# StanfordASL/pmpc

Measured on AMD Instinct MI355X. Metric: SCP iterations/sec (M particles x N horizon), higher is better.
Workload: dtype f64; 1 GPU; quadrotor x12 u4 M=4096 N=50 Nc=1 box-u, full SCP iteration (on-device linearise + c_lqp_solve-equivalent + residual), BASELINE config D; timed window = SCP iterations 6..2477 from the cold start X_prev = x0, U_prev = U_ref (the active-set round count falls as the SCP loop converges, so the rate depends on the window); particles_per_gpu=4096, parallelism=particle-shard x1, scp_loop=library (pmpc_scp_loop_device), ipm_warm_start=True

## Files before the change

include/pmpc_abi.h:

```cpp
#ifndef PMPC_ABI_H
#define PMPC_ABI_H

#include <stddef.h>

#ifdef __cplusplus
extern "C" {
#endif


void c_lqp_solve(double *X_out, double *U_out, size_t xdim, size_t udim, size_t N, size_t M, long long Nc,
                 double *x0, double *f, double *fx, double *fu, double *X_prev, double *U_prev, double *Q,
                 double *R, double *X_ref, double *U_ref, double *lx, double *ux, double *lu, double *uu,
                 double reg_x, double reg_u, double *slew_reg, double *slew_reg0, double *slew_um1,
                 long long verbose);

void c_lcone_solve(double *X_out, double *U_out, size_t xdim, size_t udim, size_t N, size_t M, long long Nc,
                   double *x0, double *f, double *fx, double *fu, double *X_prev, double *U_prev, double *Q,
                   double *R, double *X_ref, double *U_ref, double *lx, double *ux, double *lu, double *uu,
                   double reg_x, double reg_u, double *slew_reg, double *slew_reg0, double *slew_um1,
                   long long verbose, double smooth_alpha, char *solver);

void pmpc_lqp_solve_host(double *X_out, double *U_out, size_t xdim, size_t udim, size_t N, size_t M, long long Nc,
                         double *x0, double *f, double *fx, double *fu, double *X_prev, double *U_prev, double *Q,
                         double *R, double *X_ref, double *U_ref, double *lx, double *ux, double *lu, double *uu,
                         double reg_x, double reg_u, double *slew_reg, double *slew_reg0, double *slew_um1,
                         long long verbose, unsigned rowmajor);
void pmpc_lcone_solve_host(double *X_out, double *U_out, size_t xdim, size_t udim, size_t N, size_t M, long long Nc,
                           double *x0, double *f, double *fx, double *fu, double *X_prev, double *U_prev, double *Q,
                           double *R, double *X_ref, double *U_ref, double *lx, double *ux, double *lu, double *uu,
                           double reg_x, double reg_u, double *slew_reg, double *slew_reg0, double *slew_um1,
                           long long verbose, double smooth_alpha, unsigned rowmajor, long long cone_k);
void pmpc_lcone_solve_host_ex(double *X_out, double *U_out, size_t xdim, size_t udim, size_t N, size_t M, long long Nc, double *x0, double *f,
                              double *fx, double *fu, double *X_prev, double *U_prev, double *Q, double *R, double *X_ref, double *U_ref, double *lx,
                              double *ux, double *lu, double *uu, double reg_x, double reg_u, double *slew_reg, double *slew_reg0, double *slew_um1,
                              long long verbose, double smooth_alpha, unsigned rowmajor, long long cone_k, int smooth_cstr, double smooth_beta);


#define PMPC_HAS_XBOUNDS 1u
#define PMPC_HAS_UBOUNDS 2u
#define PMPC_HAS_SLEW 4u
#define PMPC_HAS_SLEW0 8u
#define PMPC_FORCE_GENERIC 16u
#define PMPC_SYMMETRIC_COST 32u

#define PMPC_COLD_START 64u
#define PMPC_STATIC_CONS_BOUNDS 128u
#define PMPC_PREV_IS_LAST_SOLUTION 256u

#define PMPC_CONE_OBJECTIVE 1024u
#define PMPC_F32_MATRICES 512u

typedef struct pmpc_problem {
  size_t xdim, udim, N, M;
  long long Nc;
  unsigned flags;
  double reg_x, reg_u;
  const double *x0, *f, *fx, *fu, *X_prev, *U_prev, *Q, *R, *X_ref, *U_ref;
  const double *lx, *ux, *lu, *uu;
  const double *slew_reg, *slew_reg0, *slew_um1;
  double *X_out, *U_out;
  const double *weights;
  double barrier_mu;
  size_t soc_q;
  const double *soc_W, *soc_w0, *soc_v;
  double soc_v0;
  const double *soc_u_interior;
  size_t cone_count;
  const int *cone_sizes;
  const double *cone_A, *cone_c;
  int cone_per_stage;
  long long cone_k;
  int smooth_cstr;
  double smooth_beta;
} pmpc_problem;

typedef struct pmpc_info {
  int status;
  int ipm_iters;
  int structured_solves;
  int fast_path;
  double mu;
  double slack_res;
  double max_violation;
  int outer_solves;
  int active_set_rounds;
} pmpc_info;

typedef struct pmpc_ctx pmpc_ctx;

int pmpc_create(pmpc_ctx **ctx, int device);
void pmpc_destroy(pmpc_ctx *ctx);
int pmpc_set_option(pmpc_ctx *ctx, const char *key, double value);
int pmpc_get_option(pmpc_ctx *ctx, const char *key, double *value);
void *pmpc_stream(pmpc_ctx *ctx);
void pmpc_sync(pmpc_ctx *ctx);

int pmpc_lqp_solve_device(pmpc_ctx *ctx, const pmpc_problem *prob, pmpc_info *info, int verbose);

int pmpc_lcone_solve_device(pmpc_ctx *ctx, const pmpc_problem *prob, double smooth_alpha, pmpc_info *info, int verbose);

int pmpc_lsoc_solve_device(pmpc_ctx *ctx, const pmpc_problem *prob, pmpc_info *info, int verbose);

int pmpc_particle_costs_device(pmpc_ctx *ctx, const pmpc_problem *prob, const double *X, const double *U, double *J_out);

int pmpc_comm_unique_id(void *unique_id_128);
int pmpc_comm_init(pmpc_ctx *ctx, int rank, int world, const void *unique_id_128);
int pmpc_comm_init_mock(pmpc_ctx *ctx, int rank, int world, int group);
int pmpc_comm_rank(pmpc_ctx *ctx);
int pmpc_comm_world(pmpc_ctx *ctx);

int pmpc_linearize_device(pmpc_ctx *ctx, int model, size_t N, size_t M, const double *x0, const double *X_prev,
                          const double *U_prev, const double *params, double *f, double *fx, double *fu);

#define PMPC_MODEL_CUSTOM0 1000
int pmpc_model_compile(const char *source, int xdim, int udim, int pdim, const char *arch, void **code, size_t *bytes, char *log,
                       size_t log_cap);
void pmpc_model_free_code(void *code);
int pmpc_model_load(pmpc_ctx *ctx, const void *code, size_t bytes, int xdim, int udim, int pdim);
int pmpc_model_unload(pmpc_ctx *ctx, int id);

int pmpc_linearize_device_f32(pmpc_ctx *ctx, int model, size_t N, size_t M, const double *x0, const double *X_prev,
                              const double *U_prev, const double *params, double *f, float *fx, float *fu);

int pmpc_rollout_device(pmpc_ctx *ctx, int model, size_t N, size_t M, const double *x0, const double *U, const double *params, double *X);

int pmpc_shift_plan_device(pmpc_ctx *ctx, int model, size_t N, size_t M, size_t s, const double *X, const double *U,
                           const double *params, const double *U_tail, double *X_new, double *U_new, double *um1_new);

int pmpc_shift_active_set_device(pmpc_ctx *ctx, size_t N, size_t M, size_t udim, long long Nc, size_t s, const double *U,
                                 const double *U_tail, const int *act, const double *lo, const double *hi, double *U_new, int *act_new);

int pmpc_warm_shift_device(pmpc_ctx *ctx, size_t N, size_t M, size_t udim, long long Nc, size_t s, const double *U, const double *U_tail,
                           const double *lo, const double *hi, double *U_new, int *shifted);

int pmpc_warm_set_read_device(pmpc_ctx *ctx, int *act_out, size_t n);

int pmpc_linearize_compact_device(pmpc_ctx *ctx, int model, size_t N, size_t M, const double *x0, const double *X_prev,
                                  const double *U_prev, const double *params, double *f, double *jc);
int pmpc_expand_jac_device(pmpc_ctx *ctx, int model, size_t N, size_t M, const double *jc, double *fx, double *fu, int orient);
long long pmpc_jac_compact_doubles(int model, size_t N, size_t M);
int pmpc_jac_live_mask(int model, unsigned char *fx_mask, unsigned char *fu_mask);

int pmpc_as_sweep_variant(int sweep, int xdim, int udim, int M, int Nc, unsigned flags, const int *knobs, int *out);

int pmpc_as_sweep_resources(int sweep, int xdim, int udim, const int *variant, int *out);

int pmpc_as_sweep_launches(int sweep, unsigned long long *out, int n, int reset);
void pmpc_as_sweep_knobs(int *out);

int pmpc_fast_launches(int kind, unsigned long long *out, int n, int reset);

int pmpc_scp_residual_device(pmpc_ctx *ctx, size_t xdim, size_t udim, size_t N, size_t M, const double *X, const double *X_prev,
                             const double *U, const double *U_prev, double *out);

int pmpc_scp_loop_device(pmpc_ctx *ctx, int model, const double *params, const pmpc_problem *p, double *f2, double *fx2, double *fu2,
                         int steps, int first_cold, double *res, pmpc_info *infos, int *last_in_out);

int pmpc_ref_shift_device(pmpc_ctx *ctx, size_t dim, size_t rows, const double *A, const double *c, const double *ref, double *out);
long long pmpc_ref_shift_bad_pivots(pmpc_ctx *ctx, int reset);

typedef struct pmpc_scp_cost {
  int kind;
  union { int K; int id; };
  union { int pos_dim; int uses_u; };
  int pos_idx[3];
  int per_stage;
  union { const double *centres; const double *cparams; };
  const double *sigma, *w;
} pmpc_scp_cost;
size_t pmpc_abi_scp_cost_size(void);

int pmpc_obstacle_cost_grad_device(pmpc_ctx *ctx, const pmpc_scp_cost *cost, size_t xdim, size_t N, size_t M, const double *X_prev,
                                   double *cx);
int pmpc_obstacle_ref_shift_device(pmpc_ctx *ctx, const pmpc_scp_cost *cost, size_t xdim, size_t N, size_t M, const double *X_prev,
                                   const double *Q, const double *X_ref, double *out);

int pmpc_scp_loop_device_cost(pmpc_ctx *ctx, int model, const double *params, const pmpc_problem *p, double *f2, double *fx2,
                              double *fu2, int steps, int first_cold, double *res, pmpc_info *infos, int *last_in_out,
                              const pmpc_scp_cost *cost);

#define PMPC_COST_CUSTOM0 1000
int pmpc_cost_compile(const char *source, int xdim, int udim, int cdim, int uses_u, const char *arch, void **code, size_t *bytes, char *log,
                      size_t log_cap);
int pmpc_cost_load(pmpc_ctx *ctx, const void *code, size_t bytes, int xdim, int udim, int cdim, int uses_u);
int pmpc_cost_unload(pmpc_ctx *ctx, int id);
int pmpc_custom_cost_grad_device(pmpc_ctx *ctx, int id, size_t N, size_t M, const double *X_prev, const double *U_prev, const double *cparams,
                                 double *cx, double *cu, double *val);

typedef struct pmpc_scp_cstr {
  int kind;
  int K;
  union { int pos_dim; int id; };
  int pos_idx[3];
  long long centre_stride_particle, centre_stride_stage;
  union { const double *centres; const double *gparams; };
  const double *radius;
} pmpc_scp_cstr;
size_t pmpc_abi_scp_cstr_size(void);

int pmpc_keepout_augment_device(pmpc_ctx *ctx, const pmpc_scp_cstr *cstr, size_t xdim, size_t udim, size_t N, size_t M,
                                const double *X_prev, const double *f, const double *fx, const double *fu, const double *X_ref,
                                double *f_aug, double *fx_aug, double *fu_aug, double *X_prev_aug, double *X_ref_aug, double *xu_aug);

int pmpc_keepout_strip_residual_device(pmpc_ctx *ctx, size_t xdim, int K, size_t udim, size_t N, size_t M, const double *X_aug, double *X,
                                       const double *X_prev, const double *U, const double *U_prev, double *out);

typedef struct pmpc_scp_aug {
  const double *Q, *x0, *lx;
  double *f[2], *fx[2], *fu[2], *X_prev[2], *X_ref[2], *xu[2];
  double *X_out;
} pmpc_scp_aug;
size_t pmpc_abi_scp_aug_size(void);

int pmpc_scp_loop_device_cstr(pmpc_ctx *ctx, int model, const double *params, const pmpc_problem *p, double *f2, double *fx2,
                              double *fu2, int steps, int first_cold, double *res, pmpc_info *infos, int *last_in_out,
                              const pmpc_scp_cost *cost, const pmpc_scp_cstr *cstr, const pmpc_scp_aug *aug);
#define PMPC_CSTR_CUSTOM0 1000
int pmpc_cstr_compile(const char *source, int xdim, int kdim, int pdim, const char *arch, void **code, size_t *bytes, char *log, size_t log_cap);
int pmpc_cstr_load(pmpc_ctx *ctx, const void *code, size_t bytes, int xdim, int kdim, int pdim);
int pmpc_cstr_unload(pmpc_ctx *ctx, int id);
int pmpc_custom_cstr_rows_device(pmpc_ctx *ctx, int id, size_t N, size_t M, const double *X_prev, const double *gparams, double *a, double *h,
                                 double *g);
int pmpc_rows_augment_device(pmpc_ctx *ctx, int K, size_t xdim, size_t udim, size_t N, size_t M, const double *a, const double *h,
                             const double *X_prev, const double *f, const double *fx, const double *fu, const double *X_ref, double *f_aug,
                             double *fx_aug, double *fu_aug, double *X_prev_aug, double *X_ref_aug, double *xu_aug);
long long pmpc_cstr_bad_rows(pmpc_ctx *ctx, int reset);

void pmpc_scp_loop_follow_ups(unsigned long long *out2, int reset);

void pmpc_profile_enable(pmpc_ctx *ctx, int level);
void pmpc_profile_read(pmpc_ctx *ctx, double *ms4, long long *n4);
void pmpc_profile_read_partial(pmpc_ctx *ctx, double *ms, long long *n);
void pmpc_profile_read_all(pmpc_ctx *ctx, double *ms, long long *launches, int count);

void pmpc_restart_stats(pmpc_ctx *ctx, unsigned long long *out4, int reset);

const char *pmpc_version(void);
void pmpc_abi_struct_sizes(size_t *problem, size_t *info);

#ifdef __cplusplus
}
#endif
#endif
```

pmpc_amd/_lib.py:

```python
from __future__ import annotations

import ctypes
import os
from pathlib import Path

import numpy as np

_HERE = Path(__file__).resolve().parent
LIB_PATH = Path(os.environ["PMPC_HIP_LIB"]) if os.environ.get("PMPC_HIP_LIB") else _HERE / "libpmpc_hip.so"
_lib = None

c_dp = ctypes.POINTER(ctypes.c_double)

HAS_XBOUNDS, HAS_UBOUNDS, HAS_SLEW, HAS_SLEW0, FORCE_GENERIC, SYMMETRIC_COST, COLD_START, STATIC_CONS_BOUNDS, PREV_IS_LAST_SOLUTION, F32_MATRICES, CONE_OBJECTIVE = 1, 2, 4, 8, 16, 32, 64, 128, 256, 512, 1024

ABI_SYMBOLS = [
    "c_lqp_solve", "c_lcone_solve", "pmpc_lqp_solve_host", "pmpc_lcone_solve_host", "pmpc_create", "pmpc_destroy", "pmpc_stream", "pmpc_sync", "pmpc_lqp_solve_device",
    "pmpc_comm_unique_id", "pmpc_comm_init", "pmpc_comm_rank", "pmpc_comm_world", "pmpc_linearize_device",
    "pmpc_profile_enable", "pmpc_profile_read", "pmpc_version", "pmpc_lcone_solve_device", "pmpc_particle_costs_device", "pmpc_lsoc_solve_device", "pmpc_comm_init_mock",
    "pmpc_scp_residual_device", "pmpc_profile_read_partial", "pmpc_profile_read_all", "pmpc_scp_loop_device", "pmpc_linearize_device_f32",
    "pmpc_set_option", "pmpc_get_option", "pmpc_abi_struct_sizes", "pmpc_lcone_solve_host_ex", "pmpc_restart_stats",
    "pmpc_linearize_compact_device", "pmpc_expand_jac_device", "pmpc_jac_compact_doubles", "pmpc_jac_live_mask",
    "pmpc_as_sweep_variant", "pmpc_as_sweep_launches", "pmpc_as_sweep_knobs", "pmpc_as_sweep_resources", "pmpc_fast_launches",
    "pmpc_ref_shift_device", "pmpc_ref_shift_bad_pivots", "pmpc_obstacle_cost_grad_device", "pmpc_obstacle_ref_shift_device",
    "pmpc_scp_loop_device_cost", "pmpc_abi_scp_cost_size",
    "pmpc_rollout_device", "pmpc_shift_plan_device",
    "pmpc_keepout_augment_device", "pmpc_abi_scp_cstr_size",
    "pmpc_keepout_strip_residual_device", "pmpc_scp_loop_device_cstr", "pmpc_abi_scp_aug_size", "pmpc_scp_loop_follow_ups",
    "pmpc_shift_active_set_device", "pmpc_warm_shift_device", "pmpc_warm_set_read_device",
    "pmpc_model_compile", "pmpc_model_free_code", "pmpc_model_load", "pmpc_model_unload",
    "pmpc_cost_compile", "pmpc_cost_load", "pmpc_cost_unload", "pmpc_custom_cost_grad_device",
    "pmpc_cstr_compile", "pmpc_cstr_load", "pmpc_cstr_unload", "pmpc_custom_cstr_rows_device", "pmpc_rows_augment_device", "pmpc_cstr_bad_rows",
]
MODEL_CUSTOM0 = 1000
COST_CUSTOM0 = 1000
CSTR_CUSTOM0 = 1000


class PmpcProblem(ctypes.Structure):
    _fields_ = (
        [(k, ctypes.c_size_t) for k in ("xdim", "udim", "N", "M")]
        + [("Nc", ctypes.c_longlong), ("flags", ctypes.c_uint), ("reg_x", ctypes.c_double), ("reg_u", ctypes.c_double)]
        + [(k, ctypes.c_void_p) for k in ("x0", "f", "fx", "fu", "X_prev", "U_prev", "Q", "R", "X_ref", "U_ref",
                                          "lx", "ux", "lu", "uu", "slew_reg", "slew_reg0", "slew_um1", "X_out", "U_out", "weights")]
        + [("barrier_mu", ctypes.c_double), ("soc_q", ctypes.c_size_t), ("soc_W", ctypes.c_void_p), ("soc_w0", ctypes.c_void_p),
           ("soc_v", ctypes.c_void_p), ("soc_v0", ctypes.c_double), ("soc_u_interior", ctypes.c_void_p),
           ("cone_count", ctypes.c_size_t), ("cone_sizes", ctypes.POINTER(ctypes.c_int)), ("cone_A", ctypes.c_void_p), ("cone_c", ctypes.c_void_p),
           ("cone_per_stage", ctypes.c_int), ("cone_k", ctypes.c_longlong), ("smooth_cstr", ctypes.c_int), ("smooth_beta", ctypes.c_double)]
    )


class PmpcInfo(ctypes.Structure):
    _fields_ = [("status", ctypes.c_int), ("ipm_iters", ctypes.c_int), ("structured_solves", ctypes.c_int),
                ("fast_path", ctypes.c_int), ("mu", ctypes.c_double), ("slack_res", ctypes.c_double),
                ("max_violation", ctypes.c_double), ("outer_solves", ctypes.c_int), ("active_set_rounds", ctypes.c_int)]


class _KOrId(ctypes.Union):
    _fields_ = [("K", ctypes.c_int), ("id", ctypes.c_int)]


class _PosDimOrUsesU(ctypes.Union):
    _fields_ = [("pos_dim", ctypes.c_int), ("uses_u", ctypes.c_int)]


class _CentresOrCparams(ctypes.Union):
    _fields_ = [("centres", ctypes.c_void_p), ("cparams", ctypes.c_void_p)]


class PmpcScpCost(ctypes.Structure):
    _anonymous_ = ("_a", "_b", "_c")
    _fields_ = [("kind", ctypes.c_int), ("_a", _KOrId), ("_b", _PosDimOrUsesU), ("pos_idx", ctypes.c_int * 3), ("per_stage", ctypes.c_int),
                ("_c", _CentresOrCparams), ("sigma", ctypes.c_void_p), ("w", ctypes.c_void_p)]


class _PosDimOrCstrId(ctypes.Union):
    _fields_ = [("pos_dim", ctypes.c_int), ("id", ctypes.c_int)]


class _CentresOrGparams(ctypes.Union):
    _fields_ = [("centres", ctypes.c_void_p), ("gparams", ctypes.c_void_p)]


class PmpcScpCstr(ctypes.Structure):
    _anonymous_ = ("_a", "_b")
    _fields_ = [("kind", ctypes.c_int), ("K", ctypes.c_int), ("_a", _PosDimOrCstrId), ("pos_idx", ctypes.c_int * 3),
                ("centre_stride_particle", ctypes.c_longlong), ("centre_stride_stage", ctypes.c_longlong),
                ("_b", _CentresOrGparams), ("radius", ctypes.c_void_p)]


class PmpcScpAug(ctypes.Structure):
    _fields_ = ([(k, ctypes.c_void_p) for k in ("Q", "x0", "lx")] + [(k, ctypes.c_void_p * 2) for k in ("f", "fx", "fu", "X_prev", "X_ref", "xu")]
                + [("X_out", ctypes.c_void_p)])


def load():
    global _lib
    if _lib is not None:
        return _lib
    if not LIB_PATH.exists():
        raise ImportError(
            f"{LIB_PATH} is missing: build the HIP extension first (python -c 'import __graft_entry__ as g; g.build()' "
            "or make -C pmpc_amd/csrc). pmpc_amd has no CPU fallback.")
    lib = ctypes.CDLL(str(LIB_PATH), mode=ctypes.RTLD_GLOBAL)
    sz, ll, dbl, vp = ctypes.c_size_t, ctypes.c_longlong, ctypes.c_double, ctypes.c_void_p
    common = [c_dp, c_dp, sz, sz, sz, sz, ll] + [c_dp] * 14 + [dbl, dbl] + [c_dp] * 3 + [ll]
    lib.c_lqp_solve.argtypes = common
    lib.c_lqp_solve.restype = None
    lib.c_lcone_solve.argtypes = common + [dbl, ctypes.c_char_p]
    lib.c_lcone_solve.restype = None
    lib.pmpc_lqp_solve_host.argtypes = common + [ctypes.c_uint]
    lib.pmpc_lqp_solve_host.restype = None
    lib.pmpc_lcone_solve_host.argtypes = common + [dbl, ctypes.c_uint, ll]
    lib.pmpc_lcone_solve_host.restype = None
    lib.pmpc_lcone_solve_host_ex.argtypes = common + [dbl, ctypes.c_uint, ll, ctypes.c_int, dbl]
    lib.pmpc_lcone_solve_host_ex.restype = None
    lib.pmpc_create.argtypes = [ctypes.POINTER(vp), ctypes.c_int]
    lib.pmpc_create.restype = ctypes.c_int
    lib.pmpc_destroy.argtypes = [vp]
    lib.pmpc_destroy.restype = None
    lib.pmpc_set_option.argtypes = [vp, ctypes.c_char_p, ctypes.c_double]
    lib.pmpc_set_option.restype = ctypes.c_int
    lib.pmpc_get_option.argtypes = [vp, ctypes.c_char_p, c_dp]
    lib.pmpc_get_option.restype = ctypes.c_int
    lib.pmpc_stream.argtypes = [vp]
    lib.pmpc_stream.restype = vp
    lib.pmpc_sync.argtypes = [vp]
    lib.pmpc_sync.restype = None
    lib.pmpc_lqp_solve_device.argtypes = [vp, ctypes.POINTER(PmpcProblem), ctypes.POINTER(PmpcInfo), ctypes.c_int]
    lib.pmpc_lqp_solve_device.restype = ctypes.c_int
    lib.pmpc_lcone_solve_device.argtypes = [vp, ctypes.POINTER(PmpcProblem), dbl, ctypes.POINTER(PmpcInfo), ctypes.c_int]
    lib.pmpc_lcone_solve_device.restype = ctypes.c_int
    lib.pmpc_lsoc_solve_device.argtypes = [vp, ctypes.POINTER(PmpcProblem), ctypes.POINTER(PmpcInfo), ctypes.c_int]
    lib.pmpc_lsoc_solve_device.restype = ctypes.c_int
    lib.pmpc_particle_costs_device.argtypes = [vp, ctypes.POINTER(PmpcProblem), vp, vp, vp]
    lib.pmpc_particle_costs_device.restype = ctypes.c_int
    lib.pmpc_comm_unique_id.argtypes = [vp]
    lib.pmpc_comm_unique_id.restype = ctypes.c_int
    lib.pmpc_comm_init.argtypes = [vp, ctypes.c_int, ctypes.c_int, vp]
    lib.pmpc_comm_init.restype = ctypes.c_int
    lib.pmpc_comm_init_mock.argtypes = [vp, ctypes.c_int, ctypes.c_int, ctypes.c_int]
    lib.pmpc_comm_init_mock.restype = ctypes.c_int
    lib.pmpc_comm_rank.argtypes = [vp]
    lib.pmpc_comm_rank.restype = ctypes.c_int
    lib.pmpc_comm_world.argtypes = [vp]
    lib.pmpc_comm_world.restype = ctypes.c_int
    lib.pmpc_linearize_device.argtypes = [vp, ctypes.c_int, sz, sz] + [vp] * 7
    lib.pmpc_linearize_device.restype = ctypes.c_int
    lib.pmpc_linearize_device_f32.argtypes = [vp, ctypes.c_int, sz, sz] + [vp] * 7
    lib.pmpc_linearize_device_f32.restype = ctypes.c_int
    if hasattr(lib, "pmpc_jac_live_mask"):
        lib.pmpc_linearize_compact_device.argtypes = [vp, ctypes.c_int, sz, sz] + [vp] * 6
        lib.pmpc_linearize_compact_device.restype = ctypes.c_int
        lib.pmpc_expand_jac_device.argtypes = [vp, ctypes.c_int, sz, sz, vp, vp, vp, ctypes.c_int]
        lib.pmpc_expand_jac_device.restype = ctypes.c_int
        lib.pmpc_jac_compact_doubles.argtypes = [ctypes.c_int, sz, sz]
        lib.pmpc_jac_compact_doubles.restype = ctypes.c_longlong
        lib.pmpc_jac_live_mask.argtypes = [ctypes.c_int, vp, vp]
        lib.pmpc_jac_live_mask.restype = ctypes.c_int
    if hasattr(lib, "pmpc_as_sweep_variant"):
        lib.pmpc_as_sweep_variant.argtypes = [ctypes.c_int] * 5 + [ctypes.c_uint, ctypes.POINTER(ctypes.c_int), ctypes.POINTER(ctypes.c_int)]
        lib.pmpc_as_sweep_variant.restype = ctypes.c_int
    if hasattr(lib, "pmpc_as_sweep_launches"):
        lib.pmpc_as_sweep_launches.argtypes = [ctypes.c_int, ctypes.POINTER(ctypes.c_ulonglong), ctypes.c_int, ctypes.c_int]
        lib.pmpc_as_sweep_launches.restype = ctypes.c_int
        lib.pmpc_as_sweep_knobs.argtypes = [ctypes.POINTER(ctypes.c_int)]
        lib.pmpc_as_sweep_knobs.restype = None
    if hasattr(lib, "pmpc_fast_launches"):
        lib.pmpc_fast_launches.argtypes = [ctypes.c_int, ctypes.POINTER(ctypes.c_ulonglong), ctypes.c_int, ctypes.c_int]
        lib.pmpc_fast_launches.restype = ctypes.c_int
    if hasattr(lib, "pmpc_as_sweep_resources"):
        lib.pmpc_as_sweep_resources.argtypes = [ctypes.c_int] * 3 + [ctypes.POINTER(ctypes.c_int), ctypes.POINTER(ctypes.c_int)]
        lib.pmpc_as_sweep_resources.restype = ctypes.c_int
    lib.pmpc_scp_residual_device.argtypes = [vp, sz, sz, sz, sz] + [vp] * 5
    lib.pmpc_scp_residual_device.restype = ctypes.c_int
    lib.pmpc_profile_enable.argtypes = [vp, ctypes.c_int]
    lib.pmpc_profile_enable.restype = None
    lib.pmpc_profile_read.argtypes = [vp, c_dp, ctypes.POINTER(ctypes.c_longlong)]
    lib.pmpc_profile_read.restype = None
    lib.pmpc_profile_read_partial.argtypes = [vp, ctypes.POINTER(ctypes.c_double), ctypes.POINTER(ctypes.c_longlong)]
    lib.pmpc_profile_read_partial.restype = None
    lib.pmpc_restart_stats.argtypes = [vp, ctypes.POINTER(ctypes.c_ulonglong), ctypes.c_int]
    lib.pmpc_restart_stats.restype = None
    lib.pmpc_profile_read_all.argtypes = [vp, c_dp, ctypes.POINTER(ctypes.c_longlong), ctypes.c_int]
    lib.pmpc_profile_read_all.restype = None
    lib.pmpc_scp_loop_device.argtypes = [vp, ctypes.c_int, vp, ctypes.POINTER(PmpcProblem), vp, vp, vp, ctypes.c_int, ctypes.c_int, vp,
                                         ctypes.POINTER(PmpcInfo), ctypes.POINTER(ctypes.c_int)]
    lib.pmpc_scp_loop_device.restype = ctypes.c_int
    if hasattr(lib, "pmpc_scp_loop_device_cost"):
        lib.pmpc_ref_shift_device.argtypes = [vp, sz, sz, vp, vp, vp, vp]
        lib.pmpc_ref_shift_device.restype = ctypes.c_int
        lib.pmpc_ref_shift_bad_pivots.argtypes = [vp, ctypes.c_int]
        lib.pmpc_ref_shift_bad_pivots.restype = ctypes.c_longlong
        lib.pmpc_obstacle_cost_grad_device.argtypes = [vp, ctypes.POINTER(PmpcScpCost), sz, sz, sz, vp, vp]
        lib.pmpc_obstacle_cost_grad_device.restype = ctypes.c_int
        lib.pmpc_obstacle_ref_shift_device.argtypes = [vp, ctypes.POINTER(PmpcScpCost), sz, sz, sz, vp, vp, vp, vp]
        lib.pmpc_obstacle_ref_shift_device.restype = ctypes.c_int
        lib.pmpc_scp_loop_device_cost.argtypes = lib.pmpc_scp_loop_device.argtypes + [ctypes.POINTER(PmpcScpCost)]
        lib.pmpc_scp_loop_device_cost.restype = ctypes.c_int
        lib.pmpc_abi_scp_cost_size.argtypes = []
        lib.pmpc_abi_scp_cost_size.restype = sz
        if lib.pmpc_abi_scp_cost_size() != ctypes.sizeof(PmpcScpCost):
            raise ImportError(f"{LIB_PATH} and pmpc_amd/_lib.py disagree on pmpc_scp_cost: library {lib.pmpc_abi_scp_cost_size()} bytes, "
                              f"binding {ctypes.sizeof(PmpcScpCost)}: rebuild the library")
    if hasattr(lib, "pmpc_shift_plan_device"):
        lib.pmpc_rollout_device.argtypes = [vp, ctypes.c_int, sz, sz, vp, vp, vp, vp]
        lib.pmpc_rollout_device.restype = ctypes.c_int
        lib.pmpc_shift_plan_device.argtypes = [vp, ctypes.c_int, sz, sz, sz] + [vp] * 7
        lib.pmpc_shift_plan_device.restype = ctypes.c_int
    if hasattr(lib, "pmpc_keepout_augment_device"):
        lib.pmpc_keepout_augment_device.argtypes = [vp, ctypes.POINTER(PmpcScpCstr), sz, sz, sz, sz] + [vp] * 11
        lib.pmpc_keepout_augment_device.restype = ctypes.c_int
        lib.pmpc_abi_scp_cstr_size.argtypes = []
        lib.pmpc_abi_scp_cstr_size.restype = sz
        if lib.pmpc_abi_scp_cstr_size() != ctypes.sizeof(PmpcScpCstr):
            raise ImportError(f"{LIB_PATH} and pmpc_amd/_lib.py disagree on pmpc_scp_cstr: library {lib.pmpc_abi_scp_cstr_size()} bytes, "
                              f"binding {ctypes.sizeof(PmpcScpCstr)}: rebuild the library")
    if hasattr(lib, "pmpc_scp_loop_device_cstr"):
        lib.pmpc_keepout_strip_residual_device.argtypes = [vp, sz, ctypes.c_int, sz, sz, sz] + [vp] * 6
        lib.pmpc_keepout_strip_residual_device.restype = ctypes.c_int
        lib.pmpc_scp_loop_device_cstr.argtypes = lib.pmpc_scp_loop_device_cost.argtypes + [ctypes.POINTER(PmpcScpCstr), ctypes.POINTER(PmpcScpAug)]
        lib.pmpc_scp_loop_device_cstr.restype = ctypes.c_int
        lib.pmpc_scp_loop_follow_ups.argtypes = [ctypes.POINTER(ctypes.c_ulonglong), ctypes.c_int]
        lib.pmpc_scp_loop_follow_ups.restype = None
        lib.pmpc_abi_scp_aug_size.argtypes = []
        lib.pmpc_abi_scp_aug_size.restype = sz
        if lib.pmpc_abi_scp_aug_size() != ctypes.sizeof(PmpcScpAug):
            raise ImportError(f"{LIB_PATH} and pmpc_amd/_lib.py disagree on pmpc_scp_aug: library {lib.pmpc_abi_scp_aug_size()} bytes, "
                              f"binding {ctypes.sizeof(PmpcScpAug)}: rebuild the library")
    if hasattr(lib, "pmpc_warm_shift_device"):
        lib.pmpc_shift_active_set_device.argtypes = [vp, sz, sz, sz, ll, sz] + [vp] * 7
        lib.pmpc_shift_active_set_device.restype = ctypes.c_int
        lib.pmpc_warm_shift_device.argtypes = [vp, sz, sz, sz, ll, sz] + [vp] * 5 + [ctypes.POINTER(ctypes.c_int)]
        lib.pmpc_warm_shift_device.restype = ctypes.c_int
        lib.pmpc_warm_set_read_device.argtypes = [vp, vp, sz]
        lib.pmpc_warm_set_read_device.restype = ctypes.c_int
    if hasattr(lib, "pmpc_model_compile"):
        lib.pmpc_model_compile.argtypes = [ctypes.c_char_p] + [ctypes.c_int] * 3 + [ctypes.c_char_p, ctypes.POINTER(vp), ctypes.POINTER(sz), ctypes.c_char_p, sz]
        lib.pmpc_model_compile.restype = ctypes.c_int
        lib.pmpc_model_free_code.argtypes = [vp]
        lib.pmpc_model_free_code.restype = None
        lib.pmpc_model_load.argtypes = [vp, ctypes.c_char_p, sz] + [ctypes.c_int] * 3
        lib.pmpc_model_load.restype = ctypes.c_int
        lib.pmpc_model_unload.argtypes = [vp, ctypes.c_int]
        lib.pmpc_model_unload.restype = ctypes.c_int
    if hasattr(lib, "pmpc_cost_compile"):
        lib.pmpc_cost_compile.argtypes = [ctypes.c_char_p] + [ctypes.c_int] * 4 + [ctypes.c_char_p, ctypes.POINTER(vp), ctypes.POINTER(sz), ctypes.c_char_p, sz]
        lib.pmpc_cost_compile.restype = ctypes.c_int
        lib.pmpc_cost_load.argtypes = [vp, ctypes.c_char_p, sz] + [ctypes.c_int] * 4
        lib.pmpc_cost_load.restype = ctypes.c_int
        lib.pmpc_cost_unload.argtypes = [vp, ctypes.c_int]
        lib.pmpc_cost_unload.restype = ctypes.c_int
        lib.pmpc_custom_cost_grad_device.argtypes = [vp, ctypes.c_int, sz, sz] + [vp] * 6
        lib.pmpc_custom_cost_grad_device.restype = ctypes.c_int
    if hasattr(lib, "pmpc_cstr_compile"):
        lib.pmpc_cstr_compile.argtypes = [ctypes.c_char_p] + [ctypes.c_int] * 3 + [ctypes.c_char_p, ctypes.POINTER(vp), ctypes.POINTER(sz), ctypes.c_char_p, sz]
        lib.pmpc_cstr_compile.restype = ctypes.c_int
        lib.pmpc_cstr_load.argtypes = [vp, ctypes.c_char_p, sz] + [ctypes.c_int] * 3
        lib.pmpc_cstr_load.restype = ctypes.c_int
        lib.pmpc_cstr_unload.argtypes = [vp, ctypes.c_int]
        lib.pmpc_cstr_unload.restype = ctypes.c_int
        lib.pmpc_custom_cstr_rows_device.argtypes = [vp, ctypes.c_int, sz, sz] + [vp] * 5
        lib.pmpc_custom_cstr_rows_device.restype = ctypes.c_int
        lib.pmpc_rows_augment_device.argtypes = [vp, ctypes.c_int, sz, sz, sz, sz] + [vp] * 13
        lib.pmpc_rows_augment_device.restype = ctypes.c_int
        lib.pmpc_cstr_bad_rows.argtypes = [vp, ctypes.c_int]
        lib.pmpc_cstr_bad_rows.restype = ctypes.c_longlong
    lib.pmpc_version.argtypes = []
    lib.pmpc_version.restype = ctypes.c_char_p
    if not hasattr(lib, "pmpc_abi_struct_sizes"):
        raise ImportError(f"{LIB_PATH} predates this binding (no pmpc_abi_struct_sizes): rebuild it (make -C pmpc_amd/csrc)")
    lib.pmpc_abi_struct_sizes.argtypes = [ctypes.POINTER(sz), ctypes.POINTER(sz)]
    lib.pmpc_abi_struct_sizes.restype = None
    sp, si = sz(0), sz(0)
    lib.pmpc_abi_struct_sizes(ctypes.byref(sp), ctypes.byref(si))
    if (sp.value, si.value) != (ctypes.sizeof(PmpcProblem), ctypes.sizeof(PmpcInfo)):
        raise ImportError(f"{LIB_PATH} ({lib.pmpc_version().decode()}) and pmpc_amd/_lib.py disagree on the ABI structs: library "
                          f"{sp.value}/{si.value} bytes, binding {ctypes.sizeof(PmpcProblem)}/{ctypes.sizeof(PmpcInfo)}: rebuild the library")
    _lib = lib
    return lib


def jac_live_mask(model: int, x: int, u: int):
    lib = load()
    mx, mu = np.zeros(x * x, dtype=np.uint8), np.zeros(x * u, dtype=np.uint8)
    got = lib.pmpc_jac_live_mask(int(model), mx.ctypes.data, mu.ctypes.data)
    if got < 0:
        raise ValueError(f"model {model} is not a built-in model")
    if got != 100 * x + u:
        raise ValueError(f"model {model}: compact records are for dims {got // 100} x {got % 100}, not {x} x {u}")
    return mx.reshape(x, x).T.astype(bool), mu.reshape(u, x).T.astype(bool)


AS_SWEEP_FLAGS = ("defect", "as_settled_in", "mat32", "cone_H", "xb_D", "as_uraw", "as_T")


def as_sweep_variant(sweep: str, x: int, u: int, M: int, Nc: int, flags: int, knobs=None):
    lib = load()
    out = (ctypes.c_int * 8)()
    kn = (ctypes.c_int * 3)(*knobs) if knobs is not None else None
    got = lib.pmpc_as_sweep_variant({"bwd": 0, "fwd": 1}[sweep], x, u, M, Nc, flags, kn, out)
    if got < 0:
        raise ValueError(f"({x}, {u}) is not a compiled pair of the active-set sweeps")
    return tuple(out[:5]), bool(got), tuple(bool(v) for v in out[5:8])


def as_sweep_resources(sweep: str, x: int, u: int, variant):
    out = (ctypes.c_int * 4)()
    got = load().pmpc_as_sweep_resources({"bwd": 0, "fwd": 1}[sweep], x, u, (ctypes.c_int * 5)(*(int(v) for v in variant)), out)
    if got == -2:
        return None
    if got == -1:
        raise ValueError(f"({x}, {u}) is not a compiled pair of the active-set sweeps")
    if got != 0:
        raise RuntimeError(f"pmpc_as_sweep_resources: HIP error {got}")
    return dict(zip(("regs", "scratch_bytes", "lds_bytes", "max_threads"), (int(v) for v in out)))


def as_sweep_code(sweep: str, variant) -> int:
    a, b, c, d, e = (int(v) for v in variant)
    if sweep == "bwd":
        return a + 3 * (b + 2 * (c + 2 * (d + 3 * e)))
    return a + 2 * b + 4 * c + 8 * d + 16 * e


def as_sweep_launches(sweep: str, reset: bool = False):
    lib = load()
    sw = {"bwd": 0, "fwd": 1}[sweep]
    n = lib.pmpc_as_sweep_launches(sw, None, 0, 0)
    out = (ctypes.c_ulonglong * n)()
    lib.pmpc_as_sweep_launches(sw, out, n, int(reset))
    return [int(v) for v in out]


FAST_LAUNCH_KINDS = {"sweep": 0, "cond": 1, "cons": 2}
CONS_SOLVE_VARIANTS = ("plain", "blocked", "lds", "reg12", "reg17")


def fast_sweep_code(factor, hxb, hub, deep) -> int:
    return int(bool(factor)) + 2 * int(bool(hxb)) + 4 * int(bool(hub)) + 8 * int(bool(deep))


def cons_solve_code(variant: str, factor) -> int:
    return CONS_SOLVE_VARIANTS.index(variant) + 5 * int(bool(factor))


def fast_launches(kind: str, reset: bool = False):
    lib = load()
    kd = FAST_LAUNCH_KINDS[kind]
    n = lib.pmpc_fast_launches(kd, None, 0, 0)
    out = (ctypes.c_ulonglong * n)()
    lib.pmpc_fast_launches(kd, out, n, int(reset))
    return [int(v) for v in out]


def scp_loop_follow_ups(reset: bool = False):
    out = (ctypes.c_ulonglong * 2)()
    load().pmpc_scp_loop_follow_ups(out, int(reset))
    return int(out[0]), int(out[1])


def as_sweep_knobs():
    out = (ctypes.c_int * 3)()
    load().pmpc_as_sweep_knobs(out)
    return tuple(out)


def dptr(a: np.ndarray):
    assert a.dtype == np.float64 and a.flags["C_CONTIGUOUS"]
    return a.ctypes.data_as(c_dp)
```

pmpc_amd/csrc/as_ctl_dev.h:

```cpp
#pragma once
#include "pmpc_dev.h"

namespace {

__device__ inline void as_ctl_block(AsCtl *ctl, const int *cnt_part, int M, const int *fail, int reduce, int decide, int last_of_batch,
                                                 AsCtl *mirror, unsigned long long *mirror_seq, unsigned long long seq, double *tail, const double *viol,
                                                 const int *open_part = nullptr) {
  __shared__ int sh[4][1024];
  __shared__ double shv[1024];
  if (ctl->done) {
    if (threadIdx.x == 0 && decide && last_of_batch && mirror) {
      *mirror = *ctl;
      __threadfence_system();
      *(volatile unsigned long long *)mirror_seq = seq;
    }
    return;
  }
  if (reduce) {
    int r = 0, d = 0, b = 0, op = 0;
    double vw = 0.0;
    for (int i = threadIdx.x; i < M; i += 1024) {
      r += cnt_part[3 * i]; d += cnt_part[3 * i + 1]; b |= cnt_part[3 * i + 2];
      if (viol) vw = fmax(vw, viol[i]);
      if (open_part) op += open_part[i];
    }
    sh[0][threadIdx.x] = r; sh[1][threadIdx.x] = d; sh[2][threadIdx.x] = b; sh[3][threadIdx.x] = op; shv[threadIdx.x] = vw;
    __syncthreads();
    for (int o = 512; o > 0; o >>= 1) {
      if (threadIdx.x < o) {
        sh[0][threadIdx.x] += sh[0][threadIdx.x + o];
        sh[1][threadIdx.x] += sh[1][threadIdx.x + o];
        sh[2][threadIdx.x] |= sh[2][threadIdx.x + o];
        sh[3][threadIdx.x] += sh[3][threadIdx.x + o];
        shv[threadIdx.x] = fmax(shv[threadIdx.x], shv[threadIdx.x + o]);
      }
      __syncthreads();
    }
    if (threadIdx.x == 0 && viol && ctl->round < 16) ctl->worst[ctl->round] = shv[0];
    if (threadIdx.x == 0) {
      if (tail) { tail[0] = sh[0][0]; tail[1] = sh[1][0]; tail[2] = sh[2][0]; tail[3] = *fail; tail[4] = sh[3][0]; }
      else { ctl->cnt[0] = sh[0][0]; ctl->cnt[1] = sh[1][0]; ctl->cnt[2] = sh[2][0]; ctl->cnt[3] = *fail; ctl->open = sh[3][0]; }
    }
  }
  if (threadIdx.x == 0 && decide) {
    if (tail) {
      for (int k = 0; k < 4; k++) ctl->cnt[k] = (int)(tail[k] < 2e9 ? tail[k] : 2e9);
      ctl->open = (int)(tail[4] < 2e9 ? tail[4] : 2e9);
    }
    const int rel = ctl->cnt[0], add = ctl->cnt[1], bad = ctl->cnt[2], fl = ctl->cnt[3];
    const int round = ctl->round;
    if (round < 16) { ctl->hist[round][0] = rel; ctl->hist[round][1] = add; }
    const int changes = rel + add;
    int done = 0, status = 1;
    if (bad || fl) { done = 1; status = 2; }
    else if (changes == 0 && ctl->open == 0) { done = 1; status = 0; }
    else if (changes == 0) {
      if (round + 1 >= ctl->max_rounds) done = 1;
    } else {
      if (changes * 2 > ctl->last_changes && ++ctl->stalls >= ctl->stall_limit) done = 1;
      ctl->last_changes = changes;
      if (round + 1 >= ctl->max_rounds) done = 1;
    }
    ctl->round = round + 1;
    ctl->status = status;
    const int e = ctl->round - 3 > 0 ? ctl->round - 3 : 0;
    double tl = 1e-11;
    for (int k = 0; k < e && tl < 1e-8; k++) tl *= 10.0;
    ctl->tol_l = ctl->dual_scale * (tl < 1e-8 ? tl : 1e-8);
    __threadfence();
    ctl->done = done;
    if ((done || last_of_batch) && mirror) {
      *mirror = *ctl;
      __threadfence_system();
      *(volatile unsigned long long *)mirror_seq = seq;
    }
  }
}

__device__ inline void as_perm_block(const int *settled, int M, int *perm) {
  __shared__ int cnt[1024];
  const int t = threadIdx.x, per = (M + 1023) / 1024, lo = t * per, hi = min(M, lo + per);
  int n = 0;
  for (int i = lo; i < hi; i++) n += settled[i] ? 0 : 1;
  cnt[t] = n;
  __syncthreads();
  for (int o = 1; o < 1024; o <<= 1) {
    const int v = t >= o ? cnt[t - o] : 0;
    __syncthreads();
    cnt[t] += v;
    __syncthreads();
  }
  const int total = cnt[1023];
  int pu = cnt[t] - n, ps = total + lo - pu;
  for (int i = lo; i < hi; i++) {
    if (settled[i]) perm[ps++] = i;
    else perm[pu++] = i;
  }
}

}
```

pmpc_amd/csrc/dynamics.hip:

```cpp
#include "pmpc_dev.h"
#include "jac_compact.h"
#include "model_jit.h"
#include <cstring>
#include <cstdlib>

namespace {

struct Unicycle {
  static constexpr int X = 4, U = 2, P = 3, UNITS = 64;
  typedef jacc::UnicycleSpec Spec;
  static __device__ __forceinline__ void step(const double *xs, const double *us, const double *p, double *fo);
  static __device__ __forceinline__ void eval(long long idx, int N, const double *x0, const double *X_prev, const double *U_prev,
                                              const double *params, double *fo, double *A, double *B);
};
struct Quadrotor {
  static constexpr int X = 12, U = 4, P = 4, UNITS = 32;
  typedef jacc::QuadrotorSpec Spec;
  static __device__ __forceinline__ void step(const double *xs, const double *us, const double *p, double *fo);
  static __device__ __forceinline__ void eval(long long idx, int N, const double *x0, const double *X_prev, const double *U_prev,
                                              const double *params, double *fo, double *A, double *B);
};

struct Bicycle {
  static constexpr int X = 4, U = 2, P = 2, UNITS = 64;
  typedef jacc::BicycleSpec Spec;
  static __device__ __forceinline__ void step(const double *xs, const double *us, const double *p, double *fo);
  static __device__ __forceinline__ void eval(long long idx, int N, const double *x0, const double *X_prev, const double *U_prev,
                                              const double *params, double *fo, double *A, double *B);
};

template <class F>
void with_model(int model, F &&fn) {
  if (model == 0) fn(Unicycle{});
  else if (model == 1) fn(Quadrotor{});
  else if (model == 2) fn(Bicycle{});
  else throw PmpcHipError{(int)hipErrorInvalidValue, "unknown built-in model", __FILE__, __LINE__};
}

__device__ __forceinline__ void Unicycle::step(const double *xs, const double *us, const double *p, double *fo) {
  const double vs = p[0], ws = p[1], T = p[2], eps = 1e-6;
  double u1 = vs * us[0], u2 = -ws * us[1];
  u1 += (u1 >= 0.0 ? eps : -eps);
  u2 += (u2 >= 0.0 ? eps : -eps);
  const double px = xs[0], py = xs[1], v0 = xs[2], th0 = xs[3];
  const double a = T * u2 + th0;
  double sa, ca, s0, c0;
  sincos(a, &sa, &ca);
  sincos(th0, &s0, &c0);
  const double iu2 = 1.0 / u2, iu22 = iu2 * iu2;
  const double n1 = u2 * sa * v0 + T * u1 * u2 * sa + u1 * ca - s0 * u2 * v0 - c0 * u1;
  const double n2 = -(u2 * ca * v0 - u1 * sa + T * u1 * u2 * ca) + c0 * u2 * v0 - s0 * u1;
  fo[0] = px + n1 * iu22; fo[1] = py + n2 * iu22; fo[2] = v0 + T * u1; fo[3] = a;
}
__device__ __forceinline__ void Unicycle::eval(long long idx, int N, const double *x0, const double *X_prev, const double *U_prev,
                                               const double *params, double *fo, double *A, double *B) {
  const int i = (int)(idx / N), j = (int)(idx % N);
  const double *xs = j == 0 ? x0 + 4 * (size_t)i : X_prev + (idx - 1) * 4;
  const double *us = U_prev + idx * 2, *p = params + 3 * (size_t)i;
  const double vs = p[0], ws = p[1], T = p[2], eps = 1e-6;
  double u1 = vs * us[0], u2 = -ws * us[1];
  u1 += (u1 >= 0.0 ? eps : -eps);
  u2 += (u2 >= 0.0 ? eps : -eps);
  const double px = xs[0], py = xs[1], v0 = xs[2], th0 = xs[3];
  const double a = T * u2 + th0;
  double sa, ca, s0, c0;
  sincos(a, &sa, &ca);
  sincos(th0, &s0, &c0);
  const double iu2 = 1.0 / u2, iu22 = iu2 * iu2;
  const double n1 = u2 * sa * v0 + T * u1 * u2 * sa + u1 * ca - s0 * u2 * v0 - c0 * u1;
  const double n2 = -(u2 * ca * v0 - u1 * sa + T * u1 * u2 * ca) + c0 * u2 * v0 - s0 * u1;
  fo[0] = px + n1 * iu22; fo[1] = py + n2 * iu22; fo[2] = v0 + T * u1; fo[3] = a;
  A[0 + 4 * 0] = 1.0; A[1 + 4 * 1] = 1.0; A[2 + 4 * 2] = 1.0; A[3 + 4 * 3] = 1.0;
  A[0 + 4 * 2] = (u2 * sa - s0 * u2) * iu22;
  A[0 + 4 * 3] = (u2 * ca * v0 + T * u1 * u2 * ca - u1 * sa - c0 * u2 * v0 + s0 * u1) * iu22;
  A[1 + 4 * 2] = (-u2 * ca + c0 * u2) * iu22;
  A[1 + 4 * 3] = (-(-u2 * sa * v0 - u1 * ca - T * u1 * u2 * sa) - s0 * u2 * v0 - c0 * u1) * iu22;
  const double dn1_du1 = T * u2 * sa + ca - c0, dn2_du1 = sa - T * u2 * ca - s0;
  const double dn1_du2 = sa * v0 + u2 * ca * T * v0 + T * u1 * sa + T * u1 * u2 * ca * T - u1 * sa * T - s0 * v0;
  const double dn2_du2 = -(ca * v0 - u2 * sa * T * v0 - u1 * ca * T + T * u1 * ca - T * T * u1 * u2 * sa) + c0 * v0;
  B[0 + 4 * 0] = dn1_du1 * iu22 * vs;
  B[1 + 4 * 0] = dn2_du1 * iu22 * vs;
  B[2 + 4 * 0] = T * vs;
  B[0 + 4 * 1] = (dn1_du2 * iu22 - 2.0 * n1 * iu22 * iu2) * (-ws);
  B[1 + 4 * 1] = (dn2_du2 * iu22 - 2.0 * n2 * iu22 * iu2) * (-ws);
  B[3 + 4 * 1] = T * (-ws);
}

__device__ __forceinline__ void Bicycle::step(const double *xs, const double *us, const double *p, double *fo) {
  const double Lw = p[0], dt = p[1];
  const double px = xs[0], py = xs[1], th = xs[2], v = xs[3], acc = us[0];
  double s, c;
  sincos(th, &s, &c);
  const double td = tan(us[1]), dtv = dt * v;
  fo[0] = px + dtv * c; fo[1] = py + dtv * s; fo[2] = th + dtv * td / Lw; fo[3] = v + dt * acc;
}
__device__ __forceinline__ void Bicycle::eval(long long idx, int N, const double *x0, const double *X_prev, const double *U_prev,
                                              const double *params, double *fo, double *A, double *B) {
  const int i = (int)(idx / N), j = (int)(idx % N);
  const double *xs = j == 0 ? x0 + 4 * (size_t)i : X_prev + (idx - 1) * 4;
  const double *us = U_prev + idx * 2, *p = params + 2 * (size_t)i;
  const double Lw = p[0], dt = p[1];
  const double px = xs[0], py = xs[1], th = xs[2], v = xs[3], acc = us[0];
  double s, c;
  sincos(th, &s, &c);
  const double td = tan(us[1]), dtv = dt * v;
  fo[0] = px + dtv * c; fo[1] = py + dtv * s; fo[2] = th + dtv * td / Lw; fo[3] = v + dt * acc;
  A[0 + 4 * 0] = 1.0; A[1 + 4 * 1] = 1.0; A[2 + 4 * 2] = 1.0; A[3 + 4 * 3] = 1.0;
  A[0 + 4 * 2] = -dtv * s;
  A[0 + 4 * 3] = dt * c;
  A[1 + 4 * 2] = dtv * c;
  A[1 + 4 * 3] = dt * s;
  A[2 + 4 * 3] = dt * td / Lw;
  B[3 + 4 * 0] = dt;
  B[2 + 4 * 1] = dtv * (1.0 + td * td) / Lw;
}

__device__ __forceinline__ void Quadrotor::step(const double *xs, const double *us, const double *p, double *fo) {
  const double m = p[0], Jx = p[1], Jy = p[2], Jz = p[3], dt = 0.05, g = 9.81;
  const double ph = xs[6], th = xs[7], ps = xs[8], wx = xs[9], wy = xs[10], wz = xs[11];
  const double T = us[0], tx = us[1], ty = us[2], tz = us[3];
  double sph, cph, sth, cth, sps, cps;
  sincos(ph, &sph, &cph);
  sincos(th, &sth, &cth);
  sincos(ps, &sps, &cps);
  const double icth = 1.0 / cth, tth = sth * icth;
  const double bx = cps * sth * cph + sps * sph, by = sps * sth * cph - cps * sph, bz = cth * cph;
  const double a = T / m;
  fo[0] = xs[0] + dt * xs[3]; fo[1] = xs[1] + dt * xs[4]; fo[2] = xs[2] + dt * xs[5];
  fo[3] = xs[3] + dt * a * bx; fo[4] = xs[4] + dt * a * by; fo[5] = xs[5] + dt * (a * bz - g);
  fo[6] = ph + dt * (wx + sph * tth * wy + cph * tth * wz);
  fo[7] = th + dt * (cph * wy - sph * wz);
  fo[8] = ps + dt * (sph * icth * wy + cph * icth * wz);
  fo[9] = wx + dt * (tx - (Jz - Jy) * wy * wz) / Jx;
  fo[10] = wy + dt * (ty - (Jx - Jz) * wz * wx) / Jy;
  fo[11] = wz + dt * (tz - (Jy - Jx) * wx * wy) / Jz;
}
__device__ __forceinline__ void Quadrotor::eval(long long idx, int N, const double *x0, const double *X_prev, const double *U_prev,
                                                const double *params, double *fo, double *A, double *B) {
  const int i = (int)(idx / N), j = (int)(idx % N);
  const double *xs = j == 0 ? x0 + 12 * (size_t)i : X_prev + (idx - 1) * 12;
  const double *us = U_prev + idx * 4, *p = params + 4 * (size_t)i;
  const double m = p[0], Jx = p[1], Jy = p[2], Jz = p[3], dt = 0.05, g = 9.81;
  const double ph = xs[6], th = xs[7], ps = xs[8], wx = xs[9], wy = xs[10], wz = xs[11];
  const double T = us[0], tx = us[1], ty = us[2], tz = us[3];
  double sph, cph, sth, cth, sps, cps;
  sincos(ph, &sph, &cph);
  sincos(th, &sth, &cth);
  sincos(ps, &sps, &cps);
  const double icth = 1.0 / cth, tth = sth * icth, sec2 = icth * icth;
  const double bx = cps * sth * cph + sps * sph, by = sps * sth * cph - cps * sph, bz = cth * cph;
  const double a = T / m;
  fo[0] = xs[0] + dt * xs[3]; fo[1] = xs[1] + dt * xs[4]; fo[2] = xs[2] + dt * xs[5];
  fo[3] = xs[3] + dt * a * bx; fo[4] = xs[4] + dt * a * by; fo[5] = xs[5] + dt * (a * bz - g);
  fo[6] = ph + dt * (wx + sph * tth * wy + cph * tth * wz);
  fo[7] = th + dt * (cph * wy - sph * wz);
  fo[8] = ps + dt * (sph * icth * wy + cph * icth * wz);
  fo[9] = wx + dt * (tx - (Jz - Jy) * wy * wz) / Jx;
  fo[10] = wy + dt * (ty - (Jx - Jz) * wz * wx) / Jy;
  fo[11] = wz + dt * (tz - (Jy - Jx) * wx * wy) / Jz;
#define AE(r, t) A[(r) + 12 * (t)]
#define BE(r, t) B[(r) + 12 * (t)]
  for (int k = 0; k < 12; k++) AE(k, k) = 1.0;
  for (int k = 0; k < 3; k++) AE(k, 3 + k) = dt;
  AE(3, 6) = dt * a * (-cps * sth * sph + sps * cph); AE(3, 7) = dt * a * (cps * cth * cph); AE(3, 8) = dt * a * (-sps * sth * cph + cps * sph);
  AE(4, 6) = dt * a * (-sps * sth * sph - cps * cph); AE(4, 7) = dt * a * (sps * cth * cph); AE(4, 8) = dt * a * (cps * sth * cph + sps * sph);
  AE(5, 6) = dt * a * (-cth * sph); AE(5, 7) = dt * a * (-sth * cph);
  AE(6, 6) += dt * (cph * tth * wy - sph * tth * wz);
  AE(6, 7) = dt * (sph * sec2 * wy + cph * sec2 * wz);
  AE(6, 9) = dt; AE(6, 10) = dt * sph * tth; AE(6, 11) = dt * cph * tth;
  AE(7, 6) = dt * (-sph * wy - cph * wz);
  AE(7, 10) = dt * cph; AE(7, 11) = -dt * sph;
  AE(8, 6) = dt * (cph * icth * wy - sph * icth * wz);
  AE(8, 7) = dt * (sph * wy + cph * wz) * sth * sec2;
  AE(8, 10) = dt * sph * icth; AE(8, 11) = dt * cph * icth;
  AE(9, 10) = -dt * (Jz - Jy) * wz / Jx; AE(9, 11) = -dt * (Jz - Jy) * wy / Jx;
  AE(10, 9) = -dt * (Jx - Jz) * wz / Jy; AE(10, 11) = -dt * (Jx - Jz) * wx / Jy;
  AE(11, 9) = -dt * (Jy - Jx) * wy / Jz; AE(11, 10) = -dt * (Jy - Jx) * wx / Jz;
  BE(3, 0) = dt * bx / m; BE(4, 0) = dt * by / m; BE(5, 0) = dt * bz / m;
  BE(9, 1) = dt / Jx; BE(10, 2) = dt / Jy; BE(11, 3) = dt / Jz;
#undef AE
#undef BE
}

__device__ __forceinline__ void residual_block(int bid, int nblk, const double *X, const double *Xp, long long rows_x, int x, const double *U,
                                               const double *Up, long long rows_u, int u, unsigned long long *out_bits) {
  __shared__ double sh[256];
  const int sub = threadIdx.x & 3;
  const long long grp = (bid * 256LL + threadIdx.x) >> 2, ngrp = ((long long)nblk * 256) >> 2;
  const int qx = (x + 3) / 4, qu = (u + 3) / 4;
  double m = 0.0;
  for (long long r = grp; r < rows_x + rows_u; r += ngrp) {
    const bool isx = r < rows_x;
    const long long rr = isx ? r : r - rows_x;
    const int d = isx ? x : u, q = isx ? qx : qu;
    const double *a = (isx ? X : U) + rr * d, *b = (isx ? Xp : Up) + rr * d;
    const int k1 = min(d, (sub + 1) * q);
    double acc = 0.0;
    for (int k = sub * q; k < k1; k++) { const double t = a[k] - b[k]; acc = fma(t, t, acc); }
    acc += __shfl_xor(acc, 1, 64);
    acc += __shfl_xor(acc, 2, 64);
    m = (acc == acc) ? fmax(m, acc) : INFINITY;
  }
  sh[threadIdx.x] = sqrt(m);
  __syncthreads();
  for (int o = 128; o > 0; o >>= 1) {
    if (threadIdx.x < o) sh[threadIdx.x] = fmax(sh[threadIdx.x], sh[threadIdx.x + o]);
    __syncthreads();
  }
  if (threadIdx.x == 0) atomicMax(out_bits, (unsigned long long)__double_as_longlong(sh[0]));
}
struct ResArgs {
  const double *X, *Xp, *U, *Up;
  long long rows;
  int x, u, nblk;
  unsigned long long *out_bits;
};
#ifndef PMPC_LIN_THREADS
#define PMPC_LIN_THREADS 256
#endif
template <class Model, class JT>
__global__ void __launch_bounds__(PMPC_LIN_THREADS) k_linearize(int N, long long tot, const double *x0, const double *X_prev, const double *U_prev,
                                                  const double *params, double *f, JT *fx, JT *fu, ResArgs res) {
  constexpr int X = Model::X, U = Model::U, UNITS = Model::UNITS;
  {
    const int glin = (int)gridDim.x - res.nblk;
    if ((int)blockIdx.x >= glin) {
      residual_block((int)blockIdx.x - glin, res.nblk, res.X, res.Xp, res.rows, res.x, res.U, res.Up, res.rows, res.u, res.out_bits);
      return;
    }
  }
  constexpr int REC = X + X * X + X * U, LD = REC | 1;
  extern __shared__ double rec[];
  const int t = threadIdx.x;
  const long long first = (long long)blockIdx.x * UNITS;
  for (int e = t; e < UNITS * LD; e += PMPC_LIN_THREADS) rec[e] = 0.0;
  __syncthreads();
  if (t < UNITS && first + t < tot) {
    double *mine = rec + t * LD;
    Model::eval(first + t, N, x0, X_prev, U_prev, params, mine, mine + X, mine + X + X * X);
  }
  __syncthreads();
  const int n = (int)((tot - first) < UNITS ? (tot - first) : UNITS);
  for (int e = t; e < n * X; e += PMPC_LIN_THREADS) f[first * X + e] = rec[(e / X) * LD + e % X];
  for (int e = t; e < n * X * X; e += PMPC_LIN_THREADS) fx[first * (X * X) + e] = (JT)rec[(e / (X * X)) * LD + X + e % (X * X)];
  for (int e = t; e < n * X * U; e += PMPC_LIN_THREADS) fu[first * (X * U) + e] = (JT)rec[(e / (X * U)) * LD + X + X * X + e % (X * U)];
}

template <class Model>
void launch_model(int N, int M, const double *x0, const double *X_prev, const double *U_prev, const double *params, double *f,
                  double *fx, double *fu, const ResArgs &res, hipStream_t s, int jac32) {
  const long long tot = (long long)M * N;
  constexpr int REC = Model::X + Model::X * Model::X + Model::X * Model::U, LD = REC | 1;
  const unsigned grid = (unsigned)((tot + Model::UNITS - 1) / Model::UNITS);
  if (jac32)
    hipLaunchKernelGGL((k_linearize<Model, float>), dim3(grid + (unsigned)res.nblk), dim3(PMPC_LIN_THREADS), Model::UNITS * LD * sizeof(double), s, N, tot, x0,
                       X_prev, U_prev, params, f, (float *)fx, (float *)fu, res);
  else
    hipLaunchKernelGGL((k_linearize<Model, double>), dim3(grid + (unsigned)res.nblk), dim3(PMPC_LIN_THREADS), Model::UNITS * LD * sizeof(double), s, N, tot, x0,
                       X_prev, U_prev, params, f, fx, fu, res);
}
constexpr int LIN_CUNITS = 64;
template <class Model>
__global__ void __launch_bounds__(PMPC_LIN_THREADS) k_linearize_compact(int N, long long tot, const double *x0, const double *X_prev, const double *U_prev,
                                                                         const double *params, double *f, double *jc, ResArgs res) {
  typedef jacc::Compact<typename Model::Spec> C;
  constexpr int X = Model::X, U = Model::U, UNITS = LIN_CUNITS, REC = C::REC, POOL = C::POOL;
  {
    const int glin = (int)gridDim.x - res.nblk;
    if ((int)blockIdx.x >= glin) {
      residual_block((int)blockIdx.x - glin, res.nblk, res.X, res.Xp, res.rows, res.x, res.U, res.Up, res.rows, res.u, res.out_bits);
      return;
    }
  }
  constexpr int LD = (X + REC) | 1;
  extern __shared__ double rec[];
  const int t = threadIdx.x;
  const long long first = (long long)blockIdx.x * UNITS;
  if (t < UNITS && first + t < tot) {
    double J[X * X + X * U] = {};
    double *mine = rec + t * LD;
    Model::eval(first + t, N, x0, X_prev, U_prev, params, mine, J, J + X * X);
#pragma unroll
    for (int k = 0; k < REC; k++) mine[X + k] = J[C::tab.rec_src[k]];
    if ((first + t) % N == 0) {
      double *pool = jc + tot * REC + ((first + t) / N) * POOL;
#pragma unroll
      for (int k = 0; k < POOL; k++) pool[k] = C::tab.pool_src[k] < 0 ? 0.0 : J[C::tab.pool_src[k] < 0 ? 0 : C::tab.pool_src[k]];
    }
  }
  __syncthreads();
  const int n = (int)((tot - first) < UNITS ? (tot - first) : UNITS);
  for (int e = t; e < n * X; e += PMPC_LIN_THREADS) f[first * X + e] = rec[(e / X) * LD + e % X];
  for (int e = t; e < n * REC; e += PMPC_LIN_THREADS) jc[first * REC + e] = rec[(e / REC) * LD + X + e % REC];
}

template <class Model>
__global__ void __launch_bounds__(256) k_expand_jac(int N, long long tot, const double *jc, double *fx, double *fu, int orient) {
  typedef jacc::Compact<typename Model::Spec> C;
  constexpr int X = Model::X, U = Model::U, XX = X * X, XU = X * U, D = XX + XU;
  const long long n = tot * D;
  for (long long k = (long long)blockIdx.x * 256 + threadIdx.x; k < n; k += (long long)gridDim.x * 256) {
    const long long unit = k / D;
    const int e = (int)(k % D);
    const int m = C::tab.expand[orient ? 1 : 0][e];
    const double v = m >= 0 ? jc[unit * C::REC + m] : jc[tot * C::REC + (unit / N) * C::POOL + (-1 - m)];
    if (e < XX) fx[unit * XX + e] = v;
    else fu[unit * XU + (e - XX)] = v;
  }
}

template <class Model>
void launch_model_compact(int N, int M, const double *x0, const double *X_prev, const double *U_prev, const double *params, double *f,
                          double *jc, const ResArgs &res, hipStream_t s) {
  typedef jacc::Compact<typename Model::Spec> C;
  const long long tot = (long long)M * N;
  constexpr int LD = (Model::X + C::REC) | 1;
  const unsigned grid = (unsigned)((tot + LIN_CUNITS - 1) / LIN_CUNITS);
  hipLaunchKernelGGL((k_linearize_compact<Model>), dim3(grid + (unsigned)res.nblk), dim3(PMPC_LIN_THREADS), LIN_CUNITS * LD * sizeof(double), s, N, tot,
                     x0, X_prev, U_prev, params, f, jc, res);
}
__global__ void __launch_bounds__(256) k_widen_f32(const float *src, double *dst, long long n) {
  for (long long k = (long long)blockIdx.x * 256 + threadIdx.x; k < n; k += (long long)gridDim.x * 256) dst[k] = (double)src[k];
}


constexpr int ROLL_LANES = 64;
template <class Model>
__global__ void __launch_bounds__(ROLL_LANES) k_rollout(int N, int M, const double *x0, const double *U, const double *params, double *X) {
  constexpr int XD = Model::X, UD = Model::U, PD = Model::P;
  const int i = (int)blockIdx.x * ROLL_LANES + (int)threadIdx.x;
  if (i >= M) return;
  double x[XD], xn[XD], u[UD], p[PD];
#pragma unroll
  for (int k = 0; k < PD; k++) p[k] = params[(size_t)i * PD + k];
#pragma unroll
  for (int k = 0; k < XD; k++) x[k] = x0[(size_t)i * XD + k];
  const double *Ui = U + (size_t)i * N * UD;
  double *Xi = X + (size_t)i * N * XD;
  for (int j = 0; j < N; j++) {
#pragma unroll
    for (int k = 0; k < UD; k++) u[k] = Ui[(size_t)j * UD + k];
    Model::step(x, u, p, xn);
#pragma unroll
    for (int k = 0; k < XD; k++) Xi[(size_t)j * XD + k] = x[k] = xn[k];
  }
}

template <class Model>
__global__ void __launch_bounds__(ROLL_LANES) k_shift_plan(int N, int M, int s, int tail_blocks, const double *X, const double *U, const double *params,
                                                           const double *U_tail, double *Xn, double *Un, double *um1n) {
  constexpr int XD = Model::X, UD = Model::U, PD = Model::P;
  const int keep = N - s;
  if ((int)blockIdx.x < tail_blocks) {
    const int i = (int)blockIdx.x * ROLL_LANES + (int)threadIdx.x;
    if (i >= M) return;
    double x[XD], xn[XD], u[UD], p[PD];
#pragma unroll
    for (int k = 0; k < PD; k++) p[k] = params[(size_t)i * PD + k];
#pragma unroll
    for (int k = 0; k < XD; k++) x[k] = X[((size_t)i * N + (N - 1)) * XD + k];
    for (int t = 0; t < s; t++) {
      const double *us = U_tail ? U_tail + ((size_t)i * s + t) * UD : U + ((size_t)i * N + (N - 1)) * UD;
#pragma unroll
      for (int k = 0; k < UD; k++) u[k] = us[k];
      Model::step(x, u, p, xn);
#pragma unroll
      for (int k = 0; k < XD; k++) x[k] = xn[k];
      const size_t row = (size_t)i * N + keep + t;
#pragma unroll
      for (int k = 0; k < UD; k++) Un[row * UD + k] = u[k];
#pragma unroll
      for (int k = 0; k < XD; k++) Xn[row * XD + k] = x[k];
    }
    return;
  }
  const long long nx = (long long)M * keep * XD, nu = (long long)M * keep * UD, nm = um1n ? (long long)M * UD : 0;
  const long long stride = (long long)((int)gridDim.x - tail_blocks) * ROLL_LANES;
  for (long long e = (long long)((int)blockIdx.x - tail_blocks) * ROLL_LANES + threadIdx.x; e < nx + nu + nm; e += stride) {
    if (e < nx) {
      const long long i = e / (keep * XD), r = e % (keep * XD);
      Xn[i * N * XD + r] = X[i * N * XD + (long long)s * XD + r];
    } else if (e < nx + nu) {
      const long long q = e - nx, i = q / (keep * UD), r = q % (keep * UD);
      Un[i * N * UD + r] = U[i * N * UD + (long long)s * UD + r];
    } else {
      const long long q = e - nx - nu, i = q / UD, k = q % UD;
      um1n[q] = U[(i * N + (s - 1)) * UD + k];
    }
  }
}

__global__ void __launch_bounds__(256) k_shift_active_set(int N, int UD, int Nc, int s, long long n, const double *U, const double *U_tail, const int *act,
                                                          const double *lo, const double *hi, double *Un, int *actn) {
  const int keep = N - s, row = N * UD;
  const long long stride = (long long)gridDim.x * 256;
  for (long long e = (long long)blockIdx.x * 256 + threadIdx.x; e < n; e += stride) {
    const long long i = e / row;
    const int q = (int)(e - i * row), j = q / UD, r = q - j * UD;
    const long long is = j < Nc ? 0 : i;
    double z;
    int a;
    if (j >= keep && U_tail) {
      z = U_tail[(is * s + (j - keep)) * UD + r];
      a = 0;
    } else {
      const long long src = (is * N + (j < keep ? j + s : N - 1)) * UD + r;
      z = U[src];
      a = act[src];
    }
    const long long b = (is * N + j) * UD + r;
    const double l = lo ? lo[b] : -INFINITY, h = hi ? hi[b] : INFINITY;
    double zc = z;
    int an = 0;
    if (!(l > h) && !(z != z)) {
      zc = z < l ? l : (z > h ? h : z);
      if (zc == l && (a == 1 || z < l)) an = 1;
      else if (zc == h && (a == 2 || z > h)) an = 2;
    }
    Un[e] = zc;
    actn[e] = an;
  }
}

}

static long long residual_blocks(long long rows) {
  long long nb = (2 * rows * 4 + 255) / 256;
  const long long cap = rows >= 200000 ? 1024 : 256;
  return nb > cap ? cap : nb;
}

void launch_linearize(int model, int N, int M, const double *x0, const double *X_prev, const double *U_prev,
                      const double *params, double *f, double *fx, double *fu, hipStream_t s, int jac32) {
  if (model_custom(model)) return custom_launch_linearize(model, N, M, x0, X_prev, U_prev, params, f, fx, fu, s);
  ResArgs none;
  memset(&none, 0, sizeof(none));
  with_model(model, [&](auto m) { launch_model<decltype(m)>(N, M, x0, X_prev, U_prev, params, f, fx, fu, none, s, jac32); });
}
void launch_linearize_compact(int model, int N, int M, const double *x0, const double *X_prev, const double *U_prev, const double *params,
                              double *f, double *jc, const double *Xr, const double *Xrp, const double *Ur, const double *Urp, int x, int u,
                              double *res_out, hipStream_t s) {
  ResArgs r;
  memset(&r, 0, sizeof(r));
  if (res_out) {
    r.X = Xr; r.Xp = Xrp; r.U = Ur; r.Up = Urp; r.rows = (long long)M * N; r.x = x; r.u = u;
    r.nblk = (int)residual_blocks(r.rows);
    r.out_bits = (unsigned long long *)res_out;
  }
  with_model(model, [&](auto m) { launch_model_compact<decltype(m)>(N, M, x0, X_prev, U_prev, params, f, jc, r, s); });
}
void launch_rollout(int model, int N, int M, const double *x0, const double *U, const double *params, double *X, hipStream_t s) {
  if (model_custom(model)) return custom_launch_rollout(model, N, M, x0, U, params, X, s);
  const unsigned grid = (unsigned)((M + ROLL_LANES - 1) / ROLL_LANES);
  with_model(model, [&](auto m) { hipLaunchKernelGGL((k_rollout<decltype(m)>), dim3(grid), dim3(ROLL_LANES), 0, s, N, M, x0, U, params, X); });
}
void launch_shift_plan(int model, int N, int M, int sh, const double *X, const double *U, const double *params, const double *U_tail, double *Xn,
                       double *Un, double *um1n, hipStream_t s) {
  if (model_custom(model)) return custom_launch_shift_plan(model, N, M, sh, X, U, params, U_tail, Xn, Un, um1n, s);
  const int tail_blocks = (M + ROLL_LANES - 1) / ROLL_LANES;
  with_model(model, [&](auto m) {
    typedef decltype(m) Model;
    const long long n = (long long)M * (N - sh) * (Model::X + Model::U) + (long long)M * Model::U;
    long long cb = (n + 4 * ROLL_LANES - 1) / (4 * ROLL_LANES);
    if (cb > 8192) cb = 8192;
    hipLaunchKernelGGL((k_shift_plan<Model>), dim3((unsigned)(tail_blocks + cb)), dim3(ROLL_LANES), 0, s, N, M, sh, tail_blocks, X, U, params, U_tail,
                       Xn, Un, um1n);
  });
}
void launch_shift_active_set(int N, int M, int u, int Nc, int sh, const double *U, const double *U_tail, const int *act, const double *lo,
                             const double *hi, double *Un, int *actn, hipStream_t s) {
  const long long n = (long long)M * N * u;
  long long b = (n + 255) / 256;
  if (b > 8192) b = 8192;
  hipLaunchKernelGGL(k_shift_active_set, dim3((unsigned)b), dim3(256), 0, s, N, u, Nc < 0 || Nc > N ? N : Nc, sh, n, U, U_tail, act, lo, hi, Un, actn);
}
bool model_known(int model) { return model >= 0 && model <= 2; }
bool jac_compact_dims(int model, int x, int u) {
  bool ok = false;
  if (model_known(model)) with_model(model, [&](auto m) { ok = x == decltype(m)::X && u == decltype(m)::U; });
  return ok;
}
long long jac_compact_doubles(int model, int N, int M) {
  const long long tot = (long long)M * N;
  long long n = -1;
  if (model_known(model))
    with_model(model, [&](auto m) {
      typedef jacc::Compact<typename decltype(m)::Spec> C;
      n = tot * C::REC + (long long)M * C::POOL;
    });
  return n;
}
void launch_expand_jac(int model, int N, int M, const double *jc, double *fx, double *fu, int orient, hipStream_t s) {
  const long long tot = (long long)M * N;
  with_model(model, [&](auto m) {
    typedef decltype(m) Model;
    long long b = (tot * (Model::X * Model::X + Model::X * Model::U) + 255) / 256;
    if (b > 8192) b = 8192;
    hipLaunchKernelGGL((k_expand_jac<Model>), dim3((unsigned)b), dim3(256), 0, s, N, tot, jc, fx, fu, orient);
  });
}
int jac_live_mask(int model, unsigned char *fx_mask, unsigned char *fu_mask) {
  auto fill = [&](auto spec) {
    typedef jacc::Compact<decltype(spec)> C;
    for (int c = 0; c < C::X + C::U; c++)
      for (int r = 0; r < C::X; r++) (c < C::X ? fx_mask[r + C::X * c] : fu_mask[r + C::X * (c - C::X)]) = C::cls(r, c) == -1;
    return C::X * 100 + C::U;
  };
  int dims = -1;
  if (model_known(model)) with_model(model, [&](auto m) { dims = fill(typename decltype(m)::Spec{}); });
  return dims;
}
void launch_widen_f32(const float *src, double *dst, long long n, hipStream_t s) {
  long long b = (n + 255) / 256;
  if (b > 4096) b = 4096;
  hipLaunchKernelGGL(k_widen_f32, dim3((unsigned)b), dim3(256), 0, s, src, dst, n);
}

void launch_linearize_with_residual(int model, int N, int M, const double *x0, const double *X_prev, const double *U_prev,
                                    const double *params, double *f, double *fx, double *fu, const double *Xr, const double *Xrp,
                                    const double *Ur, const double *Urp, int x, int u, double *res_out, hipStream_t s, int jac32) {
  if (model_custom(model)) {
    custom_launch_linearize(model, N, M, x0, X_prev, U_prev, params, f, fx, fu, s);
    return launch_scp_residual(Xr, Xrp, Ur, Urp, (long long)M * N, x, u, res_out, s, false);
  }
  ResArgs r;
  r.X = Xr; r.Xp = Xrp; r.U = Ur; r.Up = Urp; r.rows = (long long)M * N; r.x = x; r.u = u;
  r.nblk = (int)residual_blocks(r.rows);
  r.out_bits = (unsigned long long *)res_out;
  with_model(model, [&](auto m) { launch_model<decltype(m)>(N, M, x0, X_prev, U_prev, params, f, fx, fu, r, s, jac32); });
}

namespace {
__global__ void __launch_bounds__(256) k_scp_residual(const double *X, const double *Xp, long long rows_x, int x, const double *U,
                                                      const double *Up, long long rows_u, int u, unsigned long long *out_bits) {
  residual_block((int)blockIdx.x, (int)gridDim.x, X, Xp, rows_x, x, U, Up, rows_u, u, out_bits);
}
}

void launch_scp_residual(const double *X, const double *Xp, const double *U, const double *Up, long long rows, int x, int u,
                         double *out, hipStream_t s, bool zero_out) {
  if (zero_out) HIP_CHECK(hipMemsetAsync(out, 0, sizeof(double), s));
  const long long nb = residual_blocks(rows);
  hipLaunchKernelGGL(k_scp_residual, dim3((unsigned)nb), dim3(256), 0, s, X, Xp, rows, x, U, Up, rows, u, (unsigned long long *)out);
}
```

pmpc_amd/csrc/kernels_as.hip:

```cpp
#include <atomic>
#include <type_traits>

#include "fast_common.h"
#include "as_ctl_dev.h"
#include "as_variant.h"
#include "../../include/pmpc_abi.h"
#include "jac_compact.h"

#ifdef PMPC_STAGE_TIMELINE
#define PMPC_TL_STAMPS 10
__device__ unsigned long long pmpc_tl[3][128][PMPC_TL_STAMPS];
#define TL_DECL(kind) unsigned long long tl_[PMPC_TL_STAMPS] = {}; const int tl_kind = (kind); const bool tl_on = blockIdx.x == gridDim.x / 2
#define TL(k) do { __builtin_amdgcn_sched_barrier(0); tl_[k] = __builtin_amdgcn_s_memtime(); __builtin_amdgcn_sched_barrier(0); } while (0)
#define TL_FLUSH(j) do { if (tl_on && threadIdx.x == 0 && (j) < 128) { for (int k_ = 0; k_ < PMPC_TL_STAMPS; k_++) pmpc_tl[tl_kind][j][k_] = tl_[k_]; } } while (0)
#else
#define TL_DECL(kind)
#define TL(k)
#define TL_FLUSH(j)
#endif

#ifndef PMPC_AS_LEAN_WAVES
#define PMPC_AS_LEAN_WAVES 4
#endif
#ifndef PMPC_AS_DEEP_WAVES
// ... 548 lines not shown
      for (int p = 0; p < UD; p++) {
        if (act0[p] == 0) ym = fmax(ym, fabs(y[p]) / fmax(1.0, fabs(ub0[p])));
        else asks_release |= (act0[p] == 1 ? -a.as_big * y[p] : a.as_big * y[p]) < -tol_l;
      }
      frozen = ym <= a.as_freeze_tol && !asks_release;
      if (frozen) {
#pragma unroll
        for (int p = 0; p < UD; p++)
          if (act0[p] == 0) y[p] = 0.0;
      }
    }
    dcons = gu ? pick<UD>(y, g) : 0.0;
    if (cbad && i == 0 && lane == 0) *a.fail = 2;
  }
  if (CONE && frozen && a.as_settled_in && a.as_settled_in[i]) {
    if (lane == 0) {
      a.as_cnt[3 * i + 0] = 0; a.as_cnt[3 * i + 1] = 0; a.as_cnt[3 * i + 2] = 0;
      if (a.as_settled_out) a.as_settled_out[i] = 1;
      if (a.as_jhi) a.as_jhi[i] = -1;
      a.as_open[i] = 0;
      if (a.as_viol) a.as_viol[i] = 0.0;
    }
    if (i == 0 && lane < UD) a.as_delta[lane] = 0.0;
    return;
  }
  const double inv_dual = 1.0 / ((a.as_ctl ? a.as_ctl->dual_scale : 1.0) * pwi);
  auto stage = [&](auto main_tag, const int j, const Pipe &cur) {
    constexpr bool MAIN = decltype(main_tag)::value;
    TL(0);
    v4d D = {0.0, 0.0, 0.0, 0.0};
    if (MAIN || j > 0) {
#pragma unroll
      for (int r = 0; r < KS; r++) D = mfma(cur.T[r], V[r], D);
    }
    TL(1);
    const double raw = D[KS];
    const double ubc = cur.grp;
    const double kc = dpp_d<0x55>(cur.grp);
    const double loc = dpp_d<0xAA>(cur.grp);
    const double hic = dpp_d<0xFF>(cur.grp);
    const int actc = __builtin_amdgcn_mov_dpp(__double2loint(cur.grp), 0x141, 0xF, 0xF, true);
    TL(2);
    if (DEFECT) {
      const double snapped = actc == 1 ? loc : (actc == 2 ? hic : fmin(fmax(ubc, loc), hic));
      nbad |= (store_u && !(snapped == ubc)) ? 1 : 0;
      if (!MAIN && j < Nc) nbad |= (store_u && !(ubc == Ub[(size_t)j * UD + g])) ? 1 : 0;
    } else {
      nbad |= (store_u && !(loc <= hic)) ? 1 : 0;
    }
    double draw;
    if (!MAIN && j < Nc) draw = a.cons_G ? dcons : (gu ? a.duc[j * UD + g] : 0.0);
    else draw = -raw - kc;
    const bool cnt_here = store_u && (MAIN || j >= Nc || i == 0);
    const bool held = store_u && actc != 0;
    const double lam = actc == 1 ? -a.as_big * draw : a.as_big * draw;
    const bool release = held && lam < -tol_l;
    const double zt = ubc + draw;
    const bool vlo = store_u && !held && zt < loc - a.as_tol_p * fmax(1.0, fabs(loc));
    const bool vhi = store_u && !held && !vlo && zt > hic + a.as_tol_p * fmax(1.0, fabs(hic));
    const int anew = release ? 0 : (vlo ? 1 : (vhi ? 2 : actc));
    const double unew = held ? ubc : (vlo ? loc : (vhi ? hic : zt));
    const double dug = unew - ubc;
    nbad |= (store_u && !(draw == draw)) ? 1 : 0;
    nrel += (cnt_here && release) ? 1 : 0;
    nadd += (cnt_here && (vlo || vhi)) ? 1 : 0;
    jh = (cnt_here && (release || vlo || vhi)) ? j : jh;
    {
      const double pv = (vlo ? loc - zt : (vhi ? zt - hic : 0.0)) * __builtin_amdgcn_rcp(fmax(1.0, fabs(vlo ? loc : hic)));
      const double dv = release ? -lam * inv_dual : 0.0;
      vworst = fmax(vworst, cnt_here ? fmax(pv, dv) : 0.0);
    }
    TL(3);
    const double du_q = dpp_d<0x00>(dug);
    if (SENS && !MAIN && j < Nc) dcap = dug;
    const double knew = actc ? -draw : 0.0;
    if (MAIN || j >= Nc) {
      const double k1 = dpp_d<0x00>(knew);
      const double z1 = CONE ? dpp_d<0x00>(zt) : 0.0;
      if (st_lane) gst(pS, (c == 0) ? unew : ((CONE && c == 2) ? z1 : k1));
    } else {
      const double z1 = CONE ? dpp_d<0x00>(zt) : 0.0;
      if (store_u || (CONE && gu && c == 2)) gst(pS, (c == 0) ? unew : z1);
      if (store_u && i == 0) a.as_delta[j * UD + g] = dug;
    }
    pS += UD * (int)D8;
    if (store_u) gsto_i(ubase(act_, uoff(j) >> 1), lug >> 1, anew);
    TL(4);
    D[KS] = 0.0;
    double bop = (c < 4 && gu) ? du_q : 0.0;
    if (SENS) {
      const bool sc = c >= 4 && c < 4 + UD && gu;
      const double bs = (!MAIN && j < Nc) ? ((g == c - 4) ? 1.0 : 0.0) : -raw;
      bop = sc ? bs : bop;
    }
    D = mfma(cur.T[KS], bop, D);
    if (SENS) {
      if (c >= 4 && c < 4 + UD) {
        typedef double v2dd __attribute__((ext_vector_type(2)));
        const v2dd lo2 = {D[0], KS > 1 ? D[KS > 1 ? 1 : 0] : 0.0}, hi2 = {KS > 2 ? D[KS > 2 ? 2 : 0] : 0.0, gu ? bop : 0.0};
        __attribute__((address_space(1))) char *t = (__attribute__((address_space(1))) char *)(unsigned long long)ubase(T_, (long long)(j * (int)(64 * D8))) + lT;
        *(v2dd __attribute__((address_space(1))) *)t = lo2;
        *(v2dd __attribute__((address_space(1))) *)(t + 16) = hi2;
      }
    }
    if (DEFECT) {
      const double dfo = own_x ? cur.f - cur.xb : 0.0;
      D[0] += dpp_d<0x00>(dfo);
      if (KS > 1) D[1] += dpp_d<0x55>(dfo);
      if (KS > 2) D[2] += dpp_d<0xAA>(dfo);
    }
    if (own_x) {
      double mine = D[0];
#pragma unroll
      for (int r = 1; r < KS; r++) mine = (c == r) ? D[r] : mine;
      gsto(ubase(Xo_, xoff(j)), lx1, cur.xb + mine);
    }
#pragma unroll
    for (int r = 0; r < KS; r++) V[r] = D[r];
    TL(5);
    TL_FLUSH(j);
  };

  int nrel_e = 0, nadd_e = 0, nbad_e = 0, jh_e = -1;
  auto settled_update = [&](int j0) {
    double dl[UD];
#pragma unroll
    for (int k = 0; k < UD; k++) dl[k] = readlane_d(dcap, 16 * k);
    const int s16 = lane & 15, q4 = lane >> 4, gs = s16 >> 2, rs = s16 & 3;
    const bool is_x = rs < KS && KS * gs + rs < XD, is_u = rs == 3 && gs < UD;
    const size_t xo = (size_t)(is_x ? KS * gs + rs : 0), uo = (size_t)(is_u ? gs : 0);
    constexpr int SB = 4;
    for (int j4 = j0; j4 < N; j4 += 4 * SB) {
      double dv[SB], xv[SB], ub[SB], kf[SB], lo[SB], hi[SB];
      int act[SB];
#pragma unroll
      for (int q = 0; q < SB; q++) {
        const int jj = j4 + 4 * q + q4, jc = jj < N ? jj : N - 1;
        const double *t = a.as_T + (pbase + jc) * 64 + s16;
        double acc = 0.0;
#pragma unroll
        for (int k = 0; k < UD; k++) acc = fma(gld(t + 16 * k), dl[k], acc);
        dv[q] = acc;
        xv[q] = is_x ? gld(Xb + (pbase + jc) * XD + xo) : 0.0;
        const size_t e = (pbase + jc) * UD + uo;
        ub[q] = is_u ? gld(Ub + e) : 0.0;
        kf[q] = is_u ? gld(a.kff + e) : 0.0;
        lo[q] = is_u ? gld(a.as_lo + e) : 0.0;
        hi[q] = is_u ? gld(a.as_hi + e) : 0.0;
        act[q] = is_u ? a.as_act[e] : 0;
      }
#pragma unroll
      for (int q = 0; q < SB; q++) {
        const int jj = j4 + 4 * q + q4;
        const bool live = jj < N;
        if (is_x && live) gst(a.Xo + (pbase + jj) * XD + xo, xv[q] + dv[q]);
        if (is_u && live) {
          const size_t e = (pbase + jj) * UD + uo;
          if (act[q] == 0) {
            const double zt = ub[q] + dv[q];
            const bool vlo = zt < lo[q] - a.as_tol_p * fmax(1.0, fabs(lo[q])), vhi = !vlo && zt > hi[q] + a.as_tol_p * fmax(1.0, fabs(hi[q]));
            nadd_e += (vlo || vhi) ? 1 : 0;
            nbad_e |= !(zt == zt) ? 1 : 0;
            gst(a.Uo + e, zt);
            if (CONE) gst(a.as_uraw + e, zt);
          } else {
            const double kn = kf[q] - dv[q];
            const double lam = act[q] == 1 ? a.as_big * kn : -a.as_big * kn;
            const bool release = lam < -tol_l;
            nrel_e += release ? 1 : 0;
            jh_e = (release && jj > jh_e) ? jj : jh_e;
            nbad_e |= !(kn == kn) ? 1 : 0;
            gst(a.kff + e, kn);
            if (release) a.as_act[e] = 0;
            if (a.Uo != Ub) gst(a.Uo + e, ub[q]);
            if (CONE) gst(a.as_uraw + e, ub[q] + dv[q]);
          }
        }
      }
    }
  };

  auto finish = [&]() {
    double r = grp_allsum((double)nrel), d = grp_allsum((double)nadd), b = grp_allsum((double)nbad);
    if (SENS && elem) {
      r += grp_allsum(row_allsum((double)nrel_e)); d += grp_allsum(row_allsum((double)nadd_e)); b += grp_allsum(row_allsum((double)nbad_e));
      int m = jh_e;
#pragma unroll
      for (int o = 32; o > 0; o >>= 1) { const int v = __shfl_xor(m, o, 64); m = v > m ? v : m; }
      jh = m > jh ? m : jh;
    }
    if (a.as_viol) {
      double p01, p23, q0, q1;
      swap32_d(vworst, p01, p23);
      const double m = fmax(p01, p23);
      swap16_d(m, q0, q1);
      if (lane == 0) a.as_viol[i] = fmax(q0, q1);
    }
    if (a.as_jhi) {
      int m = jh;
#pragma unroll
      for (int k = 1; k < 4; k++) { const int o = __builtin_amdgcn_readlane(jh, 16 * k); m = o > m ? o : m; }
      if (lane == 0) a.as_jhi[i] = m;
    }
    if (lane == 0) {
      a.as_cnt[3 * i + 0] = (int)r;
      a.as_cnt[3 * i + 1] = (int)d;
      a.as_cnt[3 * i + 2] = b > 0.0 ? 1 : 0;
      if (a.as_settled_out) a.as_settled_out[i] = (r == 0.0 && d == 0.0 && !(b > 0.0)) ? 1 : 0;
      if (CONE) a.as_open[i] = 0;
    }
  };

  const int jmin = Nc > 1 ? Nc : 1;
  auto clampN = [&](int jj) { return jj < N ? jj : N - 1; };
  int j = 0;
  if constexpr (SENS && !DEFECT) if (elem) {
    Pipe P;
    fetch(0, P);
    stage(std::false_type{}, 0, P);
    settled_update(1);
    finish();
    return;
  }
  if (PF2) {
    Pipe P0, P1, P2;
    fetch(0, P0);
    fetch(clampN(1), P1);
    for (; j < jmin && j < N; j++) {
      fetch(clampN(j + 2), P2);
      stage(std::false_type{}, j, P0);
      P0 = P1;
      P1 = P2;
    }
    for (; j + 2 < N; j += 3) {
      fetch(clampN(j + 2), P2);
      stage(std::true_type{}, j, P0);
      fetch(clampN(j + 3), P0);
      stage(std::true_type{}, j + 1, P1);
      fetch(clampN(j + 4), P1);
      stage(std::true_type{}, j + 2, P2);
    }
    if (j < N) { stage(std::true_type{}, j, P0); j++; }
    if (j < N) { stage(std::true_type{}, j, P1); j++; }
  } else {
    Pipe A, B;
    fetch(0, A);
    for (; j < jmin && j < N; j++) {
      fetch(clampN(j + 1), B);
      stage(std::false_type{}, j, A);
      A = B;
    }
    for (; j < N; j++) {
      fetch(clampN(j + 1), B);
      stage(std::true_type{}, j, A);
      A = B;
    }
  }
  finish();
}

__global__ void k_as_begin(AsCtl *ctl, int *fail, int max_rounds, double dual_scale, int stall_limit) {
  if (threadIdx.x == 0) {
    *fail = 0;
    AsCtl h = {};
    h.max_rounds = max_rounds;
    h.stall_limit = stall_limit;
    h.last_changes = 0x7fffffff;
    h.dual_scale = dual_scale;
    h.tol_l = dual_scale * 1e-11;
    *ctl = h;
  }
}

__global__ void __launch_bounds__(1024) k_as_ctl(AsCtl *ctl, const int *cnt_part, int M, const int *fail, int reduce, int decide, int last_of_batch,
                                                 AsCtl *mirror, unsigned long long *mirror_seq, unsigned long long seq, double *tail, const double *viol,
                                                 const int *open_part) {
  as_ctl_block(ctl, cnt_part, M, fail, reduce, decide, last_of_batch, mirror, mirror_seq, seq, tail, viol, open_part);
}

__global__ void __launch_bounds__(1024) k_as_perm(const int *settled, int M, int *perm, const int *done) {
  if (done && *done) return;
  as_perm_block(settled, M, perm);
}

template <class F>
void lift(bool v, F &&f) {
  if (v) f(std::true_type{}); else f(std::false_type{});
}
template <class F>
void lift3(int v, F &&f) {
  if (v == 0) f(std::integral_constant<int, 0>{}); else if (v == 1) f(std::integral_constant<int, 1>{}); else f(std::integral_constant<int, 2>{});
}
[[noreturn]] void no_such_variant(const char *sweep, int x, int u) {
  fprintf(stderr, "pmpc_hip: %s: the selected variant is not compiled for xdim %d, udim %d (as_variant.h)\n", sweep, x, u);
  throw PmpcHipError{-1, sweep, __FILE__, __LINE__};
}
const AsSweepKnobs &as_sweep_knobs() {
  static const AsSweepKnobs k = {getenv("PMPC_AS_DEEP2_MAXM") ? atoi(getenv("PMPC_AS_DEEP2_MAXM")) : PMPC_AS_DEEP2_MAXM,
                                 getenv("PMPC_AS_DEEP_MAXM") ? atoi(getenv("PMPC_AS_DEEP_MAXM")) : PMPC_AS_DEEP_WAVES * 1024,
                                 getenv("PMPC_AS_FWD_PF2_MAXM") ? atoi(getenv("PMPC_AS_FWD_PF2_MAXM")) : (1 << 30)};
  return k;
}
std::atomic<unsigned long long> as_bwd_launches[AS_BWD_CODES], as_fwd_launches[AS_FWD_CODES];

template <int XD, int UD>
void launch_bwd_as_t(const LQArgs &a, hipStream_t s) {
  const BwdAsVariant v = select_bwd_as(a.M, a.defect, a.as_settled_in, a.mat32, a.cone_H, a.xb_D, as_sweep_knobs());
  bool launched = false;
  lift3(v.mode, [&](auto MODE) { lift(v.skip, [&](auto SKIP) { lift(v.defect, [&](auto DEFECT) { lift3(v.ex, [&](auto EX) { lift(v.f32, [&](auto F32) {
    if constexpr (bwd_as_compiled(BwdAsVariant{MODE, SKIP, DEFECT, EX, F32}, XD, UD)) {
      hipLaunchKernelGGL((k_bwd_as<XD, UD, MODE, SKIP, DEFECT, EX, std::conditional_t<F32, float, double>>), dim3(a.M), dim3(64), 0, s, a);
      as_bwd_launches[bwd_as_code(v)].fetch_add(1, std::memory_order_relaxed);
      launched = true;
    }
  }); }); }); }); });
  if (!launched) no_such_variant("factor sweep of an active-set round", XD, UD);
}
template <int XD, int UD>
void launch_fwd_as_t(const LQArgs &a, hipStream_t s) {
  const FwdAsVariant v = select_fwd_as(a.M, a.Nc, a.defect, a.mat32, a.as_uraw, a.as_T, as_sweep_knobs());
  bool launched = false;
  lift(v.defect, [&](auto DEFECT) { lift(v.pf2, [&](auto PF2) { lift(v.cone, [&](auto CONE) { lift(v.f32, [&](auto F32) { lift(v.sens, [&](auto SENS) {
    if constexpr (fwd_as_compiled(FwdAsVariant{DEFECT, PF2, CONE, F32, SENS}, XD, UD)) {
      hipLaunchKernelGGL((k_fwd_as<XD, UD, DEFECT, PF2, CONE, std::conditional_t<F32, float, double>, SENS>), dim3(a.M), dim3(64), 0, s, a);
      as_fwd_launches[fwd_as_code(v)].fetch_add(1, std::memory_order_relaxed);
      launched = true;
    }
  }); }); }); }); });
  if (!launched) no_such_variant("forward sweep of an active-set round", XD, UD);
}

}

#ifdef PMPC_STAGE_TIMELINE
extern "C" int pmpc_debug_timeline_read(unsigned long long *out) {
  return (int)hipMemcpyFromSymbol(out, HIP_SYMBOL(pmpc_tl), sizeof(unsigned long long) * 3 * 128 * PMPC_TL_STAMPS);
}
#endif
static bool as_dims_compiled(int x, int u) {
#define X(xd, ud) if (x == xd && u == ud) return true;
  PMPC_FAST_DIMS(X)
#undef X
  return false;
}
bool f32_as_dims_supported(int x, int u) { return as_dims_compiled(x, u) && as_f32_dims(x, u); }
bool xbox_as_dims_supported(int x, int u) { return as_dims_compiled(x, u) && as_xbox_dims(x, u); }
bool cone_as_dims_supported(int x, int u) { return as_dims_compiled(x, u) && as_cone_dims(x, u); }
int pmpc_as_sweep_variant(int sweep, int xdim, int udim, int M, int Nc, unsigned flags, const int *knobs, int *out) {
  if ((sweep != 0 && sweep != 1) || !as_dims_compiled(xdim, udim) || !out) return -1;
  const AsSweepKnobs k = knobs ? AsSweepKnobs{knobs[0], knobs[1], knobs[2]} : AsSweepKnobs{PMPC_AS_DEEP2_MAXM, PMPC_AS_DEEP_WAVES * 1024, 1 << 30};
  const bool defect = flags & 1, settled_in = flags & 2, mat32 = flags & 4, cone_H = flags & 8, xb_D = flags & 16, as_uraw = flags & 32, as_T = flags & 64;
  out[5] = f32_as_dims_supported(xdim, udim); out[6] = cone_as_dims_supported(xdim, udim); out[7] = xbox_as_dims_supported(xdim, udim);
  if (sweep == 0) {
    const BwdAsVariant v = select_bwd_as(M, defect, settled_in, mat32, cone_H, xb_D, k);
    out[0] = v.mode; out[1] = v.skip; out[2] = v.defect; out[3] = v.ex; out[4] = v.f32;
    return bwd_as_compiled(v, xdim, udim);
  }
  const FwdAsVariant v = select_fwd_as(M, Nc, defect, mat32, as_uraw, as_T, k);
  out[0] = v.defect; out[1] = v.pf2; out[2] = v.cone; out[3] = v.f32; out[4] = v.sens;
  return fwd_as_compiled(v, xdim, udim);
}
namespace {
template <int XD, int UD>
int as_sweep_attr_t(int sweep, const int *f, hipFuncAttributes *attr) {
  int got = -2;
  if (sweep == 0) {
    if (f[0] < 0 || f[0] > 2 || f[3] < 0 || f[3] > 2) return -2;
    lift3(f[0], [&](auto MODE) { lift(f[1] != 0, [&](auto SKIP) { lift(f[2] != 0, [&](auto DEFECT) { lift3(f[3], [&](auto EX) { lift(f[4] != 0, [&](auto F32) {
      if constexpr (bwd_as_compiled(BwdAsVariant{MODE, SKIP, DEFECT, EX, F32}, XD, UD))
        got = (int)hipFuncGetAttributes(attr, (const void *)&k_bwd_as<XD, UD, MODE, SKIP, DEFECT, EX, std::conditional_t<F32, float, double>>);
    }); }); }); }); });
  } else {
    lift(f[0] != 0, [&](auto DEFECT) { lift(f[1] != 0, [&](auto PF2) { lift(f[2] != 0, [&](auto CONE) { lift(f[3] != 0, [&](auto F32) { lift(f[4] != 0, [&](auto SENS) {
      if constexpr (fwd_as_compiled(FwdAsVariant{DEFECT, PF2, CONE, F32, SENS}, XD, UD))
        got = (int)hipFuncGetAttributes(attr, (const void *)&k_fwd_as<XD, UD, DEFECT, PF2, CONE, std::conditional_t<F32, float, double>, SENS>);
    }); }); }); }); });
  }
  return got;
}
}
int pmpc_as_sweep_resources(int sweep, int xdim, int udim, const int *variant, int *out) {
  if ((sweep != 0 && sweep != 1) || !as_dims_compiled(xdim, udim) || !variant || !out) return -1;
  hipFuncAttributes attr = {};
  int got = -1;
#define X(xd, ud) if (xdim == xd && udim == ud) got = as_sweep_attr_t<xd, ud>(sweep, variant, &attr);
  PMPC_FAST_DIMS(X)
#undef X
  if (got != 0) return got;
  out[0] = attr.numRegs; out[1] = (int)attr.localSizeBytes; out[2] = (int)attr.sharedSizeBytes; out[3] = attr.maxThreadsPerBlock;
  return 0;
}
int pmpc_as_sweep_launches(int sweep, unsigned long long *out, int n, int reset) {
  if (sweep != 0 && sweep != 1) return -1;
  std::atomic<unsigned long long> *t = sweep == 0 ? as_bwd_launches : as_fwd_launches;
  const int codes = sweep == 0 ? AS_BWD_CODES : AS_FWD_CODES;
  for (int c = 0; c < codes; c++) {
    const unsigned long long v = reset ? t[c].exchange(0, std::memory_order_relaxed) : t[c].load(std::memory_order_relaxed);
    if (out && c < n) out[c] = v;
  }
  return codes;
}
void pmpc_as_sweep_knobs(int *out) {
  const AsSweepKnobs &k = as_sweep_knobs();
  out[0] = k.deep2_maxm; out[1] = k.deep_maxm; out[2] = k.fwd_pf2_maxm;
}
void launch_bwd_as(const LQArgs &a, hipStream_t s) {
#define X(xd, ud) if (a.x == xd && a.u == ud) { launch_bwd_as_t<xd, ud>(a, s); return; }
  PMPC_FAST_DIMS(X)
#undef X
  no_such_variant("factor sweep of an active-set round", a.x, a.u);
}
void launch_fwd_as(const LQArgs &a, hipStream_t s) {
#define X(xd, ud) if (a.x == xd && a.u == ud) { launch_fwd_as_t<xd, ud>(a, s); return; }
  PMPC_FAST_DIMS(X)
#undef X
  no_such_variant("forward sweep of an active-set round", a.x, a.u);
}
void launch_as_ctl(AsCtl *ctl, const int *cnt_part, int M, const int *fail, int reduce, int decide, int last_of_batch, AsCtl *mirror,
                   unsigned long long *mirror_seq, unsigned long long seq, hipStream_t s, double *tail, const double *viol, const int *open_part) {
  hipLaunchKernelGGL(k_as_ctl, dim3(1), dim3(1024), 0, s, ctl, cnt_part, M, fail, reduce, decide, last_of_batch, mirror, mirror_seq, seq, tail, viol,
                     open_part);
}
void launch_as_perm(const int *settled, int M, int *perm, const int *done, hipStream_t s) {
  hipLaunchKernelGGL(k_as_perm, dim3(1), dim3(1024), 0, s, settled, M, perm, done);
}
void launch_as_begin(AsCtl *ctl, int *fail, int max_rounds, double dual_scale, hipStream_t s, int stall_limit) {
  hipLaunchKernelGGL(k_as_begin, dim3(1), dim3(64), 0, s, ctl, fail, max_rounds, dual_scale, stall_limit);
}
```

pmpc_amd/csrc/pmpc_dev.h:

```cpp
#pragma once
#include <hip/hip_runtime.h>
#include <cstdint>
#include <cstdio>
#include <cstdlib>

struct PmpcHipError {
  int code;
  const char *what, *file;
  int line;
};
#define HIP_CHECK(expr)                                                                       \
  do {                                                                                        \
    hipError_t _e = (expr);                                                                   \
    if (_e != hipSuccess) {                                                                   \
      fprintf(stderr, "pmpc_hip: HIP error %s at %s:%d (%s)\n", hipGetErrorString(_e), __FILE__, \
              __LINE__, #expr);                                                               \
      throw PmpcHipError{(int)_e, #expr, __FILE__, __LINE__};                                 \
    }                                                                                         \
  } while (0)
#define HIP_WARN(expr)                                                                        \
  do {                                                                                        \
    hipError_t _e = (expr);                                                                   \
    if (_e != hipSuccess)                                                                     \
      fprintf(stderr, "pmpc_hip: HIP error %s at %s:%d (%s)\n", hipGetErrorString(_e), __FILE__, __LINE__, #expr); \
  } while (0)

struct AsCtl {
  int done;
  int status;
  int round;
  int max_rounds, last_changes, stalls;
  int stall_limit;
  int open;
  int cnt[4];
  int hist[16][2];
  double tol_l;
  double dual_scale;
  double worst[16];
};

#ifndef PMPC_AS_CK_LOG
#define PMPC_AS_CK_LOG 2
#endif
#define PMPC_AS_CK_FIRST (1 << PMPC_AS_CK_LOG)

struct LQArgs {
  int x, u, N, M, Nc;
  int w;
  int n;
  double reg_x, reg_u;
  const double *pw;
  const double *cons_w;
  const double *f, *fx, *fu, *Q, *R, *X_prev, *U_prev, *X_ref, *U_ref;
  const double *slew, *slew0, *um1;
  const double *X, *U;
  const double *Dx, *Du, *wx, *wu;
  int du_full;
  double *xm, *xd, *um, *ud;
  const double *zeros;
  double *K;
  double *Hinv;
  double *kff;
  double *gc_part;
  double *Hc_part;
  int cost_lds;
  double *Hc_grp;
  double *scratch;
  const double *duc;
  double *dX, *dU;
  int *as_act;
  const double *as_lo, *as_hi;
  int *as_cnt;
  double *as_viol;
  const double *defect;
  const int *as_settled_in;
  int *as_settled_out;
  const int *as_perm;
  double *as_ck;
  int *as_jhi;
  int ck_slots;
  unsigned long long *ck_stat;
  double as_big, as_tol_p, as_tol_l;
  double as_freeze_tol;
  const double *Xb, *Ub;
  double *Xo, *Uo;
  double *as_delta;
  const AsCtl *as_ctl;
  const int *done;
  int as_merge;
  const double *cons_tH, *cons_tg;
  int cons_G;
  const double *cone_H, *cone_g;
  double *as_uraw;
  int *as_open;
  double *as_T;
  const double *xb_D, *xb_g;
  int mat32;
  int jac_compact;
  int owner;
  int any_slew;
  int sym_cost;
  int *fail;
};

struct Slab {
  long long count;
  int d, N, Nc;
  int is_u;
  int owner;
  const double *lo, *hi;
  double *z, *dz;
  const double *dz2;
  double *tl, *tu, *ll, *lu, *cl, *cu, *D, *w;
};

struct SlabEx {
  Slab s;
  int bounded;
  const double *ref, *prev;
  double *gm, *gd;
  double reg;
  const double *pw;
  long long per;
};

struct IpmScal {
  double comp_sum;
  double cnt;
  double muaff_sum;
  double pad0;
  double res_max;
  double viol_max;
  unsigned long long amin_bits;
  unsigned long long pad1;
  double mu, sigma, sigmu, alpha_aff, alpha, nu;
  int iter, status;
  double mu_target;
  double dev_max;
  double *part_dev;
};

#define PMPC_RED_BLOCKS 1024

size_t lq_generic_lds_bytes(const LQArgs &a);
void launch_rollout(const LQArgs &a, const double *U, double *X, hipStream_t s);
void launch_bwd_generic(const LQArgs &a, bool factor, hipStream_t s);
void launch_fwd_generic(const LQArgs &a, hipStream_t s);
void launch_reduce_particles_hg(const double *Hc_part, const double *gc_part, double *tmp, double *Hg, int M, int nc, hipStream_t s, int MH = -1);
void launch_reduce_particles(const double *src, double *tmp, double *dst, int M, int E, hipStream_t s);
struct AsCtlCall {
  AsCtl *ctl;
  const int *cnt_part;
  int M;
  const int *fail;
  AsCtl *mirror;
  unsigned long long *mirror_seq;
  unsigned long long seq;
  const double *viol;
  const int *open_part;
  const int *settled;
  int *perm;
};
int launch_cons_partials(const double *Hc_part, const double *gc_part, int M, int nc, double *tmp, const AsCtlCall &pend,
                         hipStream_t s);
void launch_cons_small(const double *Hc_part, const double *gc_part, int M, int nc, bool with_H, double *Hg, double *tmp, bool solve_now,
                       double *Lc, double *duc, int *fail, hipStream_t s);
void launch_cons_solve(double *Hc, double *Lc, const double *gc, double *duc, int nc, bool factor, int *fail,
                       hipStream_t s);
void launch_epi_check(const double *lam, const double *J, const double *user, int M, double cap, double *out, hipStream_t s, double *mirror = nullptr,
                      unsigned long long *mirror_seq = nullptr, unsigned long long seq = 0);
void launch_cons_scale(const double *Hc_part, const double *gc_part, const double *w, int M, int nc, bool with_H, double *outH, double *outg,
                       const int *as_act, double as_big, const double *Du, const double *wu, int u, int owner, hipStream_t s);

bool lq_fast_supported(const LQArgs &a);
void launch_bwd_fast(const LQArgs &a, bool factor, hipStream_t s);
void launch_fwd_fast(const LQArgs &a, hipStream_t s);
int cond_fast_groups(int M);
void launch_cond_fast(const LQArgs &a, hipStream_t s);
void launch_rollout_fast(const LQArgs &a, const double *U, double *X, hipStream_t s);
void launch_grad_prep(const LQArgs &a, hipStream_t s);
void count_fast_launch(int kind, int code);
void launch_as_publish(int *counters, const int *fail, int *mirror_cnt, unsigned long long *mirror_seq, unsigned long long seq, hipStream_t s);
void launch_particle_cost(const LQArgs &a, const double *X, const double *U, double *J, hipStream_t s);

void launch_bwd_as(const LQArgs &a, hipStream_t s);
void launch_fwd_as(const LQArgs &a, hipStream_t s);
void launch_as_perm(const int *settled, int M, int *perm, const int *done, hipStream_t s);
void launch_as_begin(AsCtl *ctl, int *fail, int max_rounds, double dual_scale, hipStream_t s, int stall_limit = 2);
void launch_as_ctl(AsCtl *ctl, const int *cnt_part, int M, const int *fail, int reduce, int decide, int last_of_batch, AsCtl *mirror,
                   unsigned long long *mirror_seq, unsigned long long seq, hipStream_t s, double *tail = nullptr, const double *viol = nullptr,
                   const int *open_part = nullptr);

struct ConeArgs {
  int M, N, u, q, Nc, owner;
  const double *U, *Uraw;
  const double *A, *c;
  int ncones, qs[4], rows, per_stage;
  const double *R;
  int r32;
  double reg_u, rho_scale;
  double *z, *rec;
  double *H, *g;
  int *cnt, *settled, *open;
  int *jhi;
  const int *done;
  const AsCtl *ctl;
  int finish;
  double tol_step, tol_phi, dual_scale;
};
#define PMPC_CONE_REC 12
bool cone_as_supported(int u, int q);
bool cone_as_dims_supported(int x, int u);
void launch_cone_step(const ConeArgs &a, hipStream_t s);
void launch_cone_drop_redundant_lo(double *lo, const double *A, const double *c, int q, long long rows, int u, hipStream_t s);

struct XboxArgs {
  int M, N, x;
  const double *X;
  const double *lo, *hi;
  const double *Q, *pw;
  double reg_x, rho_scale;
  double *qmax;
  double *z;
  int *st;
  double *D, *g;
  int *cnt, *settled, *open;
  int *jhi;
  const int *done;
  const AsCtl *ctl;
  int finish;
  double tol, dual_scale;
  double z_tol;
  int keep_on_clamp;
  double act_frac;
  int ctrl_from;
};
bool xbox_as_dims_supported(int x, int u);
void launch_xbox_step(const XboxArgs &a, hipStream_t s);
void launch_xbox_from_ipm(const struct Slab &sx, int *st, double *z, hipStream_t s);

void launch_block_transpose(const double *in, double *out, int rows, int cols, long long n, hipStream_t s);
void launch_host_checks(const double *lx, const double *ux, long long nx, const double *lu, const double *uu, long long nu,
                        const double *Q, long long nq, int x, const double *R, long long nr, int u, int *flags, hipStream_t s);
void launch_axpy(double *y, const double *xv, double alpha, long long n, hipStream_t s);
void launch_fill(double *y, double v, long long n, hipStream_t s);
void launch_cons_bounds(double *lo, double *hi, int M, int N, int u, int Nc, hipStream_t s);
void launch_init_base(double *U, const double *U_prev, int M, int N, int u, int Nc, hipStream_t s);
void launch_violation(const Slab &sl, double *part_max, hipStream_t s);
void launch_violation_sum(const Slab &sl, const double *za, const double *zb, double *part_max, hipStream_t s);
void launch_ipm_clip(const Slab &sl, hipStream_t s);
void launch_as_setup(const Slab &sl, int from_ipm, int keep_base, int *act, double *ztry, double big, hipStream_t s);
void launch_as_check(const Slab &sl, int *act, const double *ztry, double big, double tol_p, double tol_l, int *counters,
                     unsigned long long *worst_bits, hipStream_t s);
void launch_as_accept_all(const Slab &sl, const int *act, const double *ztry, double *Uout, const double *xtry, const double *dx,
                          long long nx, double *Xws, double *Xout, hipStream_t s);
void launch_ipm_init_slack(const Slab &sl, double mu0, hipStream_t s, double thr_frac = 1e-2);
void launch_ipm_prepare(const Slab &sl, int corrector, const IpmScal *sc, double *part_sum, double *part_cnt,
                        double *part_max, hipStream_t s);
void launch_ipm_step(const Slab &sl, int corrector, IpmScal *sc, double *part_s1, double *part_s2, hipStream_t s);
void launch_ipm_advance(const SlabEx &X, const SlabEx &U, int do_update, const IpmScal *sc, double *part_sum, double *part_cnt,
                        double *part_max, hipStream_t s);
void launch_ipm_exchange(int phase, bool pack, bool unpack, IpmScal *sc, const int *fail, double *xch, int rank, int world,
                         const double *part_sum, const double *part_cnt, const double *part_max, int nblocks, hipStream_t s,
                         double mu_target = 0.0, double *part_dev = nullptr,
                         IpmScal *mirror = nullptr, unsigned long long *mirror_seq = nullptr, unsigned long long seq = 0);

struct SocArgs {
  int M, N, u, Nc, q, owner;
  const double *U, *dU, *dU2;
  int corr;
  double *cl, *cu, *cc;
  const double *lo, *hi;
  const double *W, *w0, *v;
  double v0, mu, sigmu;
  double *sl, *su, *sc;
  double *zl, *zu, *zc;
  double *dsl, *dsu, *dsc, *dzl, *dzu, *dzc;
  double *Hadd, *wu;
  int *fail;
};
int launch_soc_prepare(const SocArgs &a, int mode, double *part_sum, double *part_cnt, hipStream_t s);
int launch_soc_step(const SocArgs &a, unsigned long long *amin_bits, double *part_s1, double *part_s2, hipStream_t s);
void launch_soc_update(const SocArgs &a, double alpha, double *X, const double *dX, const double *dX2, double *U, long long nx,
                       long long nu, long long ncz, hipStream_t s);
void launch_soc_fill_u(double *U, const double *u0, long long tot, int u, hipStream_t s);

void launch_bar_prep(const double *X, const double *U, const double *lx, const double *ux, const double *lu, const double *uu, double *Dx, double *wx,
                     double *Du, double *wu, double mu, long long nx, long long nu, int u, int N, int Nc, int owner, double *part_val, double *part_min,
                     double *out2, hipStream_t s, int mode = 0, double beta = 1.0);
void launch_cost_dots(const LQArgs &a, const double *X, const double *U, const double *dX1, const double *dU1, const double *dX2, const double *dU2,
                      double *out, hipStream_t s, const double *bx = nullptr, const double *bu = nullptr);
int launch_epi_newton(const double *Hc_part, const double *gb, const double *ga, const double *dots, const double *sig, int M, int nc, double k_minus_summu,
                      double *coef, double *duc, int *fail, hipStream_t s, int mode = 0, double *xch = nullptr);
void launch_axpy_particle(const double *a_, const double *b_, const double *coef, double *y, long long per, long long tot, hipStream_t s);
void launch_step_to(const double *a_, const double *b_, double alpha, double *y, long long tot, hipStream_t s);
void launch_interior(double *U, const double *lo, const double *hi, long long tot, double frac, hipStream_t s);
void launch_share_cons(double *U, int M, int N, int u, int Nc, hipStream_t s);

struct SlewAug {
  int x, u, N, M, Nc, has_xb, has_ub, has_um1;
  double dx, du;
  const double *f, *fx, *fu, *Xp, *Up, *Q, *R, *Xr, *Ur, *lx, *ux, *lu, *uu, *cons_lo, *cons_hi, *slew, *slew0, *um1;
  double *af, *afx, *afu, *aXp, *aUp, *aQ, *aR, *aXr, *aUr, *alo, *ahi;
};
void launch_slew_augment(const SlewAug &g, hipStream_t s);
void launch_slew_split(const double *Z, const double *W, double *X, double *U, long long rows, int x, int u, int N, int Nc,
                       const double *cons_lo, const double *cons_hi, hipStream_t s);
void launch_linearize(int model, int N, int M, const double *x0, const double *X_prev, const double *U_prev,
                      const double *params, double *f, double *fx, double *fu, hipStream_t s, int jac32 = 0);
void launch_linearize_compact(int model, int N, int M, const double *x0, const double *X_prev, const double *U_prev, const double *params,
                              double *f, double *jc, const double *Xr, const double *Xrp, const double *Ur, const double *Urp, int x, int u,
                              double *res_out, hipStream_t s);
void launch_rollout(int model, int N, int M, const double *x0, const double *U, const double *params, double *X, hipStream_t s);
void launch_shift_plan(int model, int N, int M, int sh, const double *X, const double *U, const double *params, const double *U_tail, double *Xn,
                       double *Un, double *um1n, hipStream_t s);
void launch_shift_active_set(int N, int M, int u, int Nc, int sh, const double *U, const double *U_tail, const int *act, const double *lo,
                             const double *hi, double *Un, int *actn, hipStream_t s);
bool model_known(int model);
bool jac_compact_dims(int model, int x, int u);
long long jac_compact_doubles(int model, int N, int M);
void launch_expand_jac(int model, int N, int M, const double *jc, double *fx, double *fu, int orient, hipStream_t s);
int jac_live_mask(int model, unsigned char *fx_mask, unsigned char *fu_mask);
void launch_linearize_with_residual(int model, int N, int M, const double *x0, const double *X_prev, const double *U_prev,
                                    const double *params, double *f, double *fx, double *fu, const double *Xr, const double *Xrp,
                                    const double *Ur, const double *Urp, int x, int u, double *res_out, hipStream_t s, int jac32 = 0);
void launch_widen_f32(const float *src, double *dst, long long n, hipStream_t s);
bool f32_as_dims_supported(int x, int u);
void launch_scp_residual(const double *X, const double *Xp, const double *U, const double *Up, long long rows, int x, int u,
                         double *out, hipStream_t s, bool zero_out = true);
```

pmpc_amd/csrc/solver_internal.h:

```cpp
#pragma once
#include <dlfcn.h>
#include <rccl/rccl.h>

#include <algorithm>
#include <chrono>
#include <cmath>
#include <condition_variable>
#include <cstring>
#include <functional>
#include <optional>
#include <map>
#include <atomic>
#include <mutex>
#include <thread>
#include <limits>
#include <vector>

#include "../../include/pmpc_abi.h"
#include "pmpc_dev.h"

namespace pmpc_impl {

struct DevBuf {
  void *p = nullptr;
  size_t bytes = 0;
  bool ensure(size_t b) {
    if (b <= bytes) return false;
    if (p) HIP_WARN(hipFree(p));
    p = nullptr;
    bytes = 0;
    HIP_CHECK(hipMalloc(&p, b ? b : 8));
    bytes = b;
    return true;
  }
  void release() {
    if (p) (void)hipFree(p);
    p = nullptr;
    bytes = 0;
  }
  double *d() const { return (double *)p; }
};

struct SlabBufs {
  DevBuf lo, hi, tl, tu, ll, lu, cl, cu, D, w;
};

struct Workspace {
  DevBuf X, U, dX, dU, dX2, dU2, xm, xd, um, ud, K, Hinv, kff, gc_part, Hc_part, scratch, red_tmp, Hg , Lc, duc;
  DevBuf Hc_w, gc_w, cons_w, epi_lam, epi_out, epi_gath;
  DevBuf Hc_grp;
  DevBuf es_Dx, es_wx, es_Du, es_wu, es_xm, es_xd, es_um, es_ud, es_kff2, es_kff3, es_gc2, es_dots, es_coef, es_out2, es_Xt, es_Ut, es_U, es_zero;
  long long es_key = -1;
  DevBuf xch, zeros, zslew, zslew0, zum1, part_sum, part_cnt, part_max, sc, fail;
  DevBuf pw, Jc, Jg;
  DevBuf soc_zl, soc_zu, soc_zc, soc_dzl, soc_dzu, soc_dzc, soc_sl, soc_su, soc_sc, soc_dsl, soc_dsu, soc_dsc;
  DevBuf soc_cl, soc_cu, soc_cc;
  DevBuf soc_wU, soc_wzl, soc_wzu, soc_wzc;
  long long soc_key = -1;
  DevBuf Hadd, wu_soc;
  DevBuf cone_A, cone_c, cone_z, cone_rec, cone_uraw, as_open;
  DevBuf xb_qmax;
  DevBuf xb_z, xb_st, xb_D, xb_g;
  DevBuf jac_tmp;
  DevBuf cost_ref[2];
  DevBuf cost_uref[2], cost_grad;
  DevBuf cstr_rows, cstr_bad;
  DevBuf cost_bad;
  DevBuf m64[4];
  DevBuf warmU, warm_llu, warm_luu, warm_llx, warm_lux;
  DevBuf lateX, lateU;
  long long warm_key = -1;
  double warm_mu = 0.0;
  DevBuf as_perm;
  int as_perm_m = -1;
  DevBuf as_T;
  DevBuf as_ck, as_jhi, ck_stat;
  DevBuf as_act, as_cnt, as_cntp, as_settled, as_ctl, as_delta, as_viol;
  long long su_key = -1;
  const double *su_src_lo = nullptr, *su_src_hi = nullptr;
  bool as_U_valid = false;
  int as_pred_rounds = 3;
  DevBuf cons_lo, cons_hi;
  long long cons_key = -1;
  long long xb_block_key = -1;
  int xb_warm_backoff = 0, xb_warm_fails = 0;
  long long as_key = -1;
  double as_scale = 1.0;
  size_t as_count = 0;
  DevBuf as_act2;
  DevBuf part_dev;
  DevBuf sa_f, sa_fx, sa_fu, sa_Xp, sa_Up, sa_Q, sa_R, sa_Xr, sa_Ur, sa_lo, sa_hi, sa_Xo, sa_Uo, sa_cl, sa_ch;
  SlabBufs sx, su;
};


enum PmpcOpt {
  OPT_AS_WARM, OPT_AS_SKIP, OPT_AS_DEFECT, OPT_AS_COLD_ROUNDS, OPT_POLISH_MU, OPT_WARM_START, OPT_CONE_AS, OPT_CONE_COLD_ROUNDS, OPT_XBOX_AS,
  OPT_SLEW_INCREMENT_BOXES, OPT_AS_FUSE_CTL, OPT_AS_WAVE_CONS, OPT_HOST_REUSE, OPT_WARN_SLOW_PATH, OPT_CONE_RANK_MEMORY, OPT_CONE_EPIGRAPH, OPT_COND_GROUPED, OPT_AS_FREEZE_TOL, OPT_AS_CKPT, OPT_AS_SENS_MIN_M, OPT_AS_PERM_MIN_M, OPT_CONE_PATH, OPT_COUNT
};
}
using namespace pmpc_impl;

struct ProfCat {
  std::vector<std::pair<hipEvent_t, hipEvent_t>> pending, pool;
  double ms = 0.0;
  long long n = 0;
};

struct pmpc_ctx {
  double opt[OPT_COUNT];
  bool warned_slow_path = false;
  std::vector<double> cone_rw;
  long long cone_rw_key = -1;
  long long fp_key = -1;
  int fp_ok = -1;
  std::vector<double> cone_lam;
  long long cone_lam_key = -1;
  double cone_rho = 0.0;
  std::vector<double> cons_w_host, epi_lam_host;
  const double *cons_w_active = nullptr;
  int xb_ctrl_from = -1;
  AsCtlCall as_pend{};
  int prof = 0;
  double partial_ms = 0.0;
  long long partial_n = 0;
  double last_ms[8] = {0};
  long long last_n[8] = {0};
  ProfCat cat[8];
  int device = 0;
  hipStream_t stream = nullptr;
  Workspace ws;
  IpmScal *sc_host = nullptr;
  int *fail_host = nullptr;
  struct ScMirror { IpmScal sc; unsigned long long seq; int as_cnt[4]; unsigned long long as_seq; AsCtl ctl; double epi[4]; unsigned long long epi_seq; };
  ScMirror *mirror = nullptr, *mirror_dev = nullptr;
  unsigned long long seq = 0, as_seq = 0, epi_seq = 0;
  ncclComm_t comm = nullptr;
  bool mock_comm = false;
  int rank = 0, world = 1;
  bool single_rank_comm = false;
  bool multi() const { return world > 1 || single_rank_comm; }
  DevBuf stage[19], stage_t[4];
  void *pinned = nullptr;
  void *sm_pinned = nullptr;
  size_t sm_pinned_bytes = 0;
  size_t pinned_bytes = 0;
  struct StagedChunk { void *dst; size_t bytes, off; };
  std::vector<StagedChunk> staged;
  DevBuf host_flags;
  struct ScpHook {
    std::function<void()> post_batch;
    bool fired = false, ok = false;
    const double *compact_fx = nullptr;
    int compact_model = 0;
  } scp;
};

namespace pmpc_impl {

void allreduce(pmpc_ctx *c, void *buf, size_t n, ncclDataType_t dt, ncclRedOp_t op);
void broadcast(pmpc_ctx *c, void *buf, size_t n, ncclDataType_t dt, int root);
void comm_release(pmpc_ctx *c);
unsigned *cost_bad_counter(pmpc_ctx *c);

struct ScpHookGuard {
  pmpc_ctx *const c;
  ~ScpHookGuard() { c->scp = pmpc_ctx::ScpHook{}; }
};

struct ProfScope {
  pmpc_ctx *c;
  int k;
  std::pair<hipEvent_t, hipEvent_t> ev;
  bool on;
  ProfScope(pmpc_ctx *c_, int k_) : c(c_), k(k_), on(c_->prof >= 2 || (c_->prof == 1 && k_ == 0)) {
    if (!on) return;
    ProfCat &pc = c->cat[k];
    if (pc.pool.empty()) {
      HIP_CHECK(hipEventCreate(&ev.first));
      HIP_CHECK(hipEventCreate(&ev.second));
    } else {
      ev = pc.pool.back();
      pc.pool.pop_back();
    }
    HIP_CHECK(hipEventRecord(ev.first, c->stream));
  }
  ~ProfScope() {
    if (!on) return;
    HIP_WARN(hipEventRecord(ev.second, c->stream));
    c->cat[k].pending.push_back(ev);
  }
};

template <class Pred>
bool spin_until(Pred ready, double limit_s = 2.0) {
  const auto t0 = std::chrono::steady_clock::now();
  for (;;) {
    for (int k = 0; k < 1024; k++) {
      if (ready()) return true;
      __builtin_ia32_pause();
    }
    if (std::chrono::duration<double>(std::chrono::steady_clock::now() - t0).count() > limit_s) return ready();
  }
}
void wait_published(pmpc_ctx *c, volatile unsigned long long *seq, unsigned long long want);
void read_scalars(pmpc_ctx *c);
void exchange(pmpc_ctx *c, int phase);
void structured_solve(pmpc_ctx *c, LQArgs &a, bool factor, bool fast, bool prep_done = false);
int fail_after_error(pmpc_ctx *c, const pmpc_problem *p, pmpc_info *info);
void fill_nan_outputs(pmpc_ctx *c, const pmpc_problem *p);

}

constexpr int PMPC_NEEDS_F64 = -7;

extern "C" {
pmpc_problem widened_f32_problem(pmpc_ctx *c, const pmpc_problem *p, bool jacobians = true);
void build_slew_increment_problem(pmpc_ctx *c, const pmpc_problem *p, pmpc_problem &q, SlewAug &g);
int lcone_body(pmpc_ctx *c, const pmpc_problem *p, double smooth_alpha, pmpc_info *info, int verbose);
__attribute__((visibility("hidden"))) int lcone_smooth_body(pmpc_ctx *c, const pmpc_problem *p, double mu_b, pmpc_info *info, int verbose, int smode = 0, double sbeta = 1.0,
                                                            bool phase1_start = false);
int pmpc_epigraph_solve_host(int M, int nc, const double *J, const double *H, const double *g, const unsigned char *held, double K, double cap, double *lam_io, double *delta,
                             double *t_out, int verbose);
int solve_impl_body(pmpc_ctx *c, const pmpc_problem *p, pmpc_info *info, int verbose, bool soc);
bool slew_increment_form_applies(const pmpc_ctx *c, const pmpc_problem *p, bool soc);
int solve_slew_increment_form(pmpc_ctx *c, const pmpc_problem *p, pmpc_info *info, int verbose);
}
```

pmpc_amd/csrc/solver_qp.hip:

```cpp
#include "solver_internal.h"

namespace {

constexpr int GO_ON = -1000;

struct AsAttempt {
  double dual_scale;
  int mode, max_rounds;
  LQArgs b;
  ConeArgs ca;
  XboxArgs xa;
  int *act;
  AsCtl *ctl;
  bool cone, xbox;
  bool refused;
  bool use_defect;
  AsCtl h;
  int round;
  int n_batches_at_hook;
};

class QpSolve {
 public:
  QpSolve(pmpc_ctx *c_, const pmpc_problem *p_, pmpc_info *info_, int verbose_, bool soc_)
// ... 388 lines not shown
  double mu = 1.0;
  int status = 1, newton = 0;
  const bool soc_warm_off = c->opt[OPT_WARM_START] == 0.0;
  const long long skey = shape_key(x, q * 2 + (has_ub ? 1 : 0), 16);
  bool warm = !soc_warm_off && !(p->flags & PMPC_COLD_START) && w.soc_key == skey, remembered = false;
  int nblk, fl;
soc_restart:
  sa.mu = 1.0; sa.sigmu = 0.0;
  if (warm) {
    HIP_CHECK(hipMemcpyAsync(w.U.p, w.soc_wU.p, nu * D8, hipMemcpyDeviceToDevice, s));
    HIP_CHECK(hipMemcpyAsync(sa.zl, w.soc_wzl.p, nu * D8, hipMemcpyDeviceToDevice, s));
    HIP_CHECK(hipMemcpyAsync(sa.zu, w.soc_wzu.p, nu * D8, hipMemcpyDeviceToDevice, s));
    HIP_CHECK(hipMemcpyAsync(sa.zc, w.soc_wzc.p, ncz * D8, hipMemcpyDeviceToDevice, s));
  } else {
    launch_soc_fill_u(w.U.d(), p->soc_u_interior, (long long)nu, u, s);
  }
  if (fast) launch_rollout_fast(a, w.U.d(), w.X.d(), s);
  else launch_rollout(a, w.U.d(), w.X.d(), s);
  nblk = launch_soc_prepare(sa, warm ? 2 : 0, w.part_sum.d(), w.part_cnt.d(), s);
  fl = measure(nblk, mu);
  if (fl && warm) {
    if (verbose) printf("pmpc_hip: stage cones: remembered iterate rejected, cold start\n");
    warm = false;
    w.soc_key = -1;
    HIP_CHECK(hipMemsetAsync(w.fail.p, 0, sizeof(int), s));
    goto soc_restart;
  }
  if (fl) return finish(fl == 3 ? 3 : 2);
  sa.corr = 0; sa.sigmu = 0.0;
  nblk = launch_soc_prepare(sa, 1, w.part_sum.d(), w.part_cnt.d(), s);
  fl = measure(nblk, mu);
  if (fl) { status = fl == 3 ? 3 : 2; }
  auto read_step = [&](double &amax) -> int {
    if (c->multi()) allreduce(c, &sc->amin_bits, 1, ncclFloat64, ncclMin);
    HIP_CHECK(hipMemcpyAsync(&host_rd.amin, &sc->amin_bits, sizeof(unsigned long long), hipMemcpyDeviceToHost, s));
    HIP_CHECK(hipMemcpyAsync(&host_rd.fail, w.fail.p, sizeof(int), hipMemcpyDeviceToHost, s));
    HIP_CHECK(hipStreamSynchronize(s));
    memcpy(&amax, &host_rd.amin, sizeof(double));
    return host_rd.fail;
  };
  int centre_left = finish_now ? 5 : 0;
  bool centring = false;
  for (int it = 0; it < 100 && status == 1; it++) {
    a.dX = w.dX.d(); a.dU = w.dU.d();
    structured_solve(c, a, true, fast);
    inf.structured_solves++;
    HIP_CHECK(hipMemcpyAsync(&sc->amin_bits, &one_bits, sizeof(one_bits), hipMemcpyHostToDevice, s));
    sa.corr = 0; sa.sigmu = 0.0;
    nblk = launch_soc_step(sa, &sc->amin_bits, w.part_sum.d(), w.part_cnt.d(), s);
    HIP_CHECK(hipMemcpyAsync(hs.data(), w.part_sum.p, nblk * D8, hipMemcpyDeviceToHost, s));
    HIP_CHECK(hipMemcpyAsync(hc.data(), w.part_cnt.p, nblk * D8, hipMemcpyDeviceToHost, s));
    double a_aff;
    if (read_step(a_aff)) { status = centring ? 0 : 2; break; }
    if (centring) {
      HIP_CHECK(hipMemsetAsync(sa.cl, 0, nu * D8, s));
      HIP_CHECK(hipMemsetAsync(sa.cu, 0, nu * D8, s));
      HIP_CHECK(hipMemsetAsync(sa.cc, 0, ncz * D8, s));
    }
    double s1 = 0.0, s2 = 0.0;
    for (int k = 0; k < nblk; k++) { s1 += hs[k]; s2 += hc[k]; }
    if (c->multi()) {
      double pair[2] = {s1, s2};
      HIP_CHECK(hipMemcpyAsync(w.xch.p, pair, 2 * D8, hipMemcpyHostToDevice, s));
      allreduce(c, w.xch.p, 2, ncclFloat64, ncclSum);
      HIP_CHECK(hipMemcpyAsync(pair, w.xch.p, 2 * D8, hipMemcpyDeviceToHost, s));
      HIP_CHECK(hipStreamSynchronize(s));
      s1 = pair[0]; s2 = pair[1];
    }
    a_aff = std::min(1.0, a_aff);
    const double mu_aff = mu + a_aff * (s1 + a_aff * s2) / cone_cnt;
    double sigma = mu_aff / mu;
    sigma = centring ? 1.0 : std::min(1.0, std::max(0.0, sigma * sigma * sigma));
    sa.corr = 1; sa.sigmu = sigma * mu;
    launch_soc_prepare(sa, 1, w.part_sum.d(), w.part_cnt.d(), s);
    a.dX = w.dX2.d(); a.dU = w.dU2.d();
    structured_solve(c, a, false, fast);
    a.dX = w.dX.d(); a.dU = w.dU.d();
    HIP_CHECK(hipMemcpyAsync(&sc->amin_bits, &one_bits, sizeof(one_bits), hipMemcpyHostToDevice, s));
    launch_soc_step(sa, &sc->amin_bits, w.part_sum.d(), w.part_cnt.d(), s);
    double amax;
    if (read_step(amax)) { status = centring ? 0 : 2; break; }
    const double alpha = std::min(1.0, 0.99 * amax);
    if (!(alpha > 0.0)) { status = centring ? 0 : 2; break; }
    launch_soc_update(sa, alpha, w.X.d(), w.dX.d(), w.dX2.d(), w.U.d(), (long long)nx, (long long)nu, (long long)ncz, s);
    newton++;
    sa.corr = 0; sa.sigmu = 0.0;
    nblk = launch_soc_prepare(sa, 1, w.part_sum.d(), w.part_cnt.d(), s);
    double mu_new;
    fl = measure(nblk, mu_new);
    if (fl) {
      status = (mu <= 1e2 * mu_tol) ? 0 : (fl == 3 ? 3 : 2);
      break;
    }
    if (verbose) printf("pmpc_hip: soc it %3d  mu %9.3e -> %9.3e  alpha_aff %6.4f  sigma %8.2e  alpha %6.4f\n", newton, mu, mu_new, a_aff, sigma, alpha);
    const bool stalled = alpha < 1e-3 && mu <= 1e2 * mu_tol;
    mu = mu_new;
    if (!remembered && !soc_warm_off && mu <= 0.5) {
      for (DevBuf *b : {&w.soc_wU, &w.soc_wzl, &w.soc_wzu}) b->ensure(nu * D8);
      w.soc_wzc.ensure(ncz * D8);
      HIP_CHECK(hipMemcpyAsync(w.soc_wU.p, w.U.p, nu * D8, hipMemcpyDeviceToDevice, s));
      HIP_CHECK(hipMemcpyAsync(w.soc_wzl.p, sa.zl, nu * D8, hipMemcpyDeviceToDevice, s));
      HIP_CHECK(hipMemcpyAsync(w.soc_wzu.p, sa.zu, nu * D8, hipMemcpyDeviceToDevice, s));
      HIP_CHECK(hipMemcpyAsync(w.soc_wzc.p, sa.zc, ncz * D8, hipMemcpyDeviceToDevice, s));
      w.soc_key = skey;
      remembered = true;
    }
    if (centring) {
      if (--centre_left <= 0 || stalled) { status = 0; break; }
    } else if (stalled || (mu <= mu_tol && centre_left <= 0)) {
      status = 0;
      break;
    } else if (mu <= mu_tol) {
      centring = true;
    }
  }
  if (status != 0 && warm) {
    if (verbose) printf("pmpc_hip: stage cones: warm-started run failed (status %d), cold start\n", status);
    warm = false; remembered = false; status = 1; newton = 0;
    w.soc_key = -1;
    HIP_CHECK(hipMemsetAsync(w.fail.p, 0, sizeof(int), s));
    goto soc_restart;
  }
  inf.ipm_iters = newton;
  inf.mu = mu;
  if (verbose) printf("pmpc_hip: stage cones: status %d after %d Newton steps\n", status, newton);
  return (finish_now || status != 0) ? finish(status) : 0;
}

int QpSolve::equality_phase() {
  reset_scalars();
  equality_solve();
  if (has_xb) launch_violation(sx, w.part_max.d(), s);
  if (has_ub) launch_violation(su, w.part_max.d() + B, s);
  exchange(c, 1);
  read_scalars(c);
  inf.max_violation = c->sc_host->viol_max;
  if (*c->fail_host || !(c->sc_host->viol_max == c->sc_host->viol_max)) return 2;
  if (verbose) printf("pmpc_hip: equality-only optimum, max bound violation %.3e\n", c->sc_host->viol_max);
  if (!has_xb && !has_ub) return 0;
  if (c->sc_host->viol_max <= 0.0 && mu_target == 0.0) return 0;
  return 1;
}

int QpSolve::active_set_fast(double dual_scale, int mode, int max_rounds, int xb) {
  if (!(mode == 0 && as_defect_on && (p->flags & PMPC_PREV_IS_LAST_SOLUTION) && Nc <= 1)) densify();
  AsAttempt t = as_blocks(dual_scale, mode, max_rounds, xb);
  if (t.refused || !as_start(t)) return 1;
  as_rounds(t);
  return as_accept(t);
}

AsAttempt QpSolve::as_blocks(double dual_scale, int mode, int max_rounds, int xb) {
  AsAttempt t;
  memset(&t, 0, sizeof(t));
  t.dual_scale = dual_scale; t.mode = mode; t.max_rounds = max_rounds;
  LQArgs &b = t.b;
  ConeArgs &ca = t.ca;
  XboxArgs &xa = t.xa;
  const double big = 1e30, tol_p = 1e-13;
  w.as_act.ensure(nu * sizeof(int) + 8); w.as_cntp.ensure((size_t)M * 3 * sizeof(int)); w.as_settled.ensure((size_t)M * sizeof(int));
  w.as_ctl.ensure(sizeof(AsCtl)); w.as_delta.ensure((size_t)std::max(nc, 1) * D8);
  int *act = t.act = (int *)w.as_act.p;
  AsCtl *ctl = t.ctl = (AsCtl *)w.as_ctl.p;
  b = a;
  b.Dx = b.wx = b.Du = b.wu = nullptr; b.du_full = 0;
  b.as_act = act; b.as_lo = su.lo; b.as_hi = su.hi; b.as_cnt = (int *)w.as_cntp.p; b.as_big = big; b.as_tol_p = tol_p;
  b.as_settled_out = (int *)w.as_settled.p; b.as_delta = w.as_delta.d(); b.as_ctl = ctl; b.done = &ctl->done;
  w.as_viol.ensure((size_t)M * D8);
  b.as_viol = w.as_viol.d();
  b.Xb = p->X_out; b.Ub = p->U_out; b.Xo = p->X_out; b.Uo = p->U_out;
  {
    int slots = 0;
    if (c->opt[OPT_AS_CKPT] != 0.0 && as_skip_on && nc <= 32)
      while ((PMPC_AS_CK_FIRST << slots) <= N - 1) slots++;
    if (slots > 0) {
      const int ks = (x + 3) / 4;
      w.as_ck.ensure((size_t)M * slots * (64 * ks + 32) * D8);
      w.as_jhi.ensure((size_t)M * sizeof(int));
      if (w.ck_stat.ensure(4 * sizeof(unsigned long long))) HIP_CHECK(hipMemsetAsync(w.ck_stat.p, 0, 4 * sizeof(unsigned long long), s));
      b.as_ck = w.as_ck.d(); b.as_jhi = (int *)w.as_jhi.p; b.ck_slots = slots; b.ck_stat = (unsigned long long *)w.ck_stat.p;
    }
  }
  w.as_key = -1;
  const bool cone = t.cone = cone_as && (mode == 0 || mode == 3 || mode == 5);
  b.as_freeze_tol = (cone && Nc == 1) ? c->opt[OPT_AS_FREEZE_TOL] : 0.0;
  if (cone) {
    const int q = (int)p->soc_q;
    const size_t rows = (size_t)M * N;
    w.Hadd.ensure(nu * u * D8); w.wu_soc.ensure(nu * D8); w.cone_uraw.ensure(nu * D8); w.as_open.ensure((size_t)M * sizeof(int));
    const bool z_new = w.cone_z.ensure(rows * cone_rows * D8), rec_new = w.cone_rec.ensure(rows * std::max(ncones, 1) * PMPC_CONE_REC * D8);
    if (z_new || rec_new) w.as_key = -1;
    b.cone_H = w.Hadd.d(); b.cone_g = w.wu_soc.d(); b.as_uraw = w.cone_uraw.d(); b.as_open = (int *)w.as_open.p;
    ca.M = M; ca.N = N; ca.u = u; ca.q = q; ca.Nc = Nc; ca.owner = a.owner;
    ca.rows = cone_rows;
    if (ncones > 0) {
      ca.ncones = ncones; ca.per_stage = p->cone_per_stage ? 1 : 0;
      for (int k = 0; k < ncones; k++) ca.qs[k] = p->cone_sizes[k];
      ca.A = p->cone_A; ca.c = p->cone_c;
    } else {
      ca.ncones = 1; ca.qs[0] = q; ca.per_stage = 0;
      ca.A = w.cone_A.d(); ca.c = w.cone_c.d();
    }
    ca.R = p->R; ca.r32 = a.mat32; ca.reg_u = p->reg_u; ca.rho_scale = 1e7;
    ca.z = w.cone_z.d(); ca.rec = w.cone_rec.d(); ca.H = w.Hadd.d(); ca.g = w.wu_soc.d();
    ca.cnt = (int *)w.as_cntp.p; ca.settled = (int *)w.as_settled.p; ca.open = (int *)w.as_open.p; ca.done = &ctl->done; ca.ctl = ctl;
    ca.jhi = b.as_jhi;
    ca.tol_step = 1e-6; ca.tol_phi = 1e-9;
    ca.dual_scale = dual_scale;
  }
  const bool xbox = t.xbox = xbox_as && xb != 0;
  {
    const int min_m = (int)c->opt[OPT_AS_SENS_MIN_M];
    if (min_m > 0 && M >= min_m && as_skip_on && Nc == 1 && (mode != 0 || w.as_pred_rounds >= 2)) {
      w.as_T.ensure((size_t)M * N * 64 * D8);
      b.as_T = w.as_T.d();
    }
  }
  if (xbox) {
    w.as_open.ensure((size_t)M * sizeof(int)); w.xb_D.ensure(nx * D8); w.xb_g.ensure(nx * D8);
    const bool z_new = w.xb_z.ensure(nx * D8), st_new = w.xb_st.ensure(nx * sizeof(int));
    if ((z_new || st_new) && mode == 0) { t.refused = true; return t; }
    if (mode == 2 || xb == 2) {
      HIP_CHECK(hipMemsetAsync(w.xb_z.p, 0, nx * D8, s));
      HIP_CHECK(hipMemsetAsync(w.xb_st.p, 0, nx * sizeof(int), s));
    } else if (mode == 1) {
      launch_xbox_from_ipm(sx, (int *)w.xb_st.p, w.xb_z.d(), s);
    }
    b.xb_D = w.xb_D.d(); b.xb_g = w.xb_g.d(); b.as_open = (int *)w.as_open.p;
    xa.M = M; xa.N = N; xa.x = x; xa.lo = p->lx; xa.hi = p->ux; xa.Q = p->Q; xa.pw = p->weights; xa.reg_x = p->reg_x; xa.rho_scale = 1e7;
    w.xb_qmax.ensure((size_t)M * D8);
    xa.qmax = w.xb_qmax.d();
    xa.z = w.xb_z.d(); xa.st = (int *)w.xb_st.p; xa.D = w.xb_D.d(); xa.g = w.xb_g.d();
    xa.cnt = (int *)w.as_cntp.p; xa.settled = (int *)w.as_settled.p; xa.open = (int *)w.as_open.p; xa.done = &ctl->done; xa.ctl = ctl;
    xa.jhi = b.as_jhi;
    xa.tol = 1e-9; xa.dual_scale = dual_scale;
    xa.z_tol = 1e-3;
    xa.keep_on_clamp = 1;
    xa.act_frac = 0.5;
    xa.ctrl_from = c->xb_ctrl_from >= 0 ? c->xb_ctrl_from : x;
  }
  return t;
}

bool QpSolve::as_start(AsAttempt &t) {
  LQArgs &b = t.b;
  ConeArgs &ca = t.ca;
  XboxArgs &xa = t.xa;
  const int mode = t.mode, max_rounds = t.max_rounds;
  const double dual_scale = t.dual_scale, big = b.as_big;
  const bool cone = t.cone, xbox = t.xbox;
  int *act = t.act;
  AsCtl *ctl = t.ctl;
  launch_as_begin(ctl, (int *)w.fail.p, max_rounds, dual_scale, s, cone ? 8 : (xbox ? (c->xb_ctrl_from >= 0 ? 8 : (mode == 0 ? 6 : 3)) : 2));
  const bool use_defect = t.use_defect = mode == 0 && as_defect_on && (p->flags & PMPC_PREV_IS_LAST_SOLUTION);
  if (a.mat32 && !use_defect) return false;
  if (mode == 3) {
    ProfScope ps(c, 5);
    HIP_CHECK(hipMemsetAsync(act, 0, nu * sizeof(int) + 8, s));
    HIP_CHECK(hipMemsetAsync(w.cone_z.p, 0, (size_t)M * N * cone_rows * D8, s));
    if (p->soc_u_interior) launch_soc_fill_u(p->U_out, p->soc_u_interior, (long long)nu, u, s);
    else launch_init_base(p->U_out, p->U_prev, M, N, u, Nc, s);
    launch_rollout_fast(b, p->U_out, p->X_out, s);
  } else if (mode == 4) {
  } else if (!use_defect) {
    ProfScope ps(c, 5);
    Slab st = su;
    st.z = (mode == 0 && !w.as_U_valid) ? const_cast<double *>(p->U_prev) : w.U.d();
    st.D = nullptr; st.w = nullptr;
    if (mode == 5) {
      st.ll = w.soc_zl.d(); st.lu = w.soc_zu.d();
      HIP_CHECK(hipMemcpyAsync(w.cone_z.p, w.soc_zc.p, (size_t)M * N * cone_rows * D8, hipMemcpyDeviceToDevice, s));
    }
    launch_as_setup(st, mode == 5 ? 1 : mode, 0, act, p->U_out, big, s);
    launch_rollout_fast(b, p->U_out, p->X_out, s);
  }
  c->as_pend.ctl = nullptr;
  if (xbox) {
    ProfScope ps(c, 5);
    xa.finish = 0;
    xa.X = use_defect ? p->X_prev : p->X_out;
    launch_xbox_step(xa, s);
  }
  if (cone) {
    ProfScope ps(c, 5);
    ca.finish = 0;
    ca.U = use_defect ? p->U_prev : p->U_out;
    launch_cone_step(ca, s);
  }
  return true;
}

void QpSolve::as_rounds(AsAttempt &t) {
  LQArgs &b = t.b;
  ConeArgs &ca = t.ca;
  XboxArgs &xa = t.xa;
  const int mode = t.mode, max_rounds = t.max_rounds;
  const bool cone = t.cone, xbox = t.xbox, use_defect = t.use_defect;
  AsCtl *ctl = t.ctl;
  AsCtl &h = t.h;
  int &round = t.round, &n_batches_at_hook = t.n_batches_at_hook;
  const bool fuse_env = c->opt[OPT_AS_FUSE_CTL] != 0.0 && c->opt[OPT_AS_WAVE_CONS] != 0.0;
  const bool fuse_ctl = fuse_env && !c->multi() && Nc == 1;
  const int *open_part = (cone || xbox) ? (const int *)w.as_open.p : nullptr;
  const int perm_min_m = (int)c->opt[OPT_AS_PERM_MIN_M];
  round = 0;
  int depth = mode == 0 ? std::max(1, std::min(w.as_pred_rounds, max_rounds)) : std::min(3, max_rounds);
  if (verbose > 1 && xbox) depth = 1;
  static const bool duc_trace = getenv("PMPC_DUC_TRACE") != nullptr;
  if (duc_trace) depth = 1;
  n_batches_at_hook = -1000;
  memset(&h, 0, sizeof(h));
  while (true) {
    const int batch = std::min(depth, max_rounds - round);
    for (int k = 0; k < batch; k++) {
      const int r = round + k;
      b.defect = (use_defect && r == 0) ? p->f : nullptr;
      const bool skip = as_skip_on && r > 0 && nc <= 32;
      b.as_settled_in = skip ? (const int *)w.as_settled.p : nullptr;
      b.as_perm = nullptr;
      if (skip && perm_min_m > 0 && M >= perm_min_m && b.as_T) {
        ProfScope pp(c, 5);
        if (w.as_perm.ensure((size_t)M * sizeof(int)) || w.as_perm_m != M) {
          std::vector<int> id(M);
          for (int q_ = 0; q_ < M; q_++) id[q_] = q_;
          HIP_CHECK(hipMemcpyAsync(w.as_perm.p, id.data(), (size_t)M * sizeof(int), hipMemcpyHostToDevice, s));
          HIP_CHECK(hipStreamSynchronize(s));
          w.as_perm_m = M;
        }
        static const bool perm_fused = !(getenv("PMPC_AS_PERM_FUSED") && atoi(getenv("PMPC_AS_PERM_FUSED")) == 0);
        if (c->as_pend.ctl && perm_fused) {
          c->as_pend.settled = (const int *)w.as_settled.p;
          c->as_pend.perm = (int *)w.as_perm.p;
        } else {
          launch_as_perm((const int *)w.as_settled.p, M, (int *)w.as_perm.p, &ctl->done, s);
        }
        b.as_perm = (const int *)w.as_perm.p;
      }
      const bool last = k == batch - 1;
      const bool merge = c->multi() && nc > 0;
      b.as_merge = merge ? (k == 0 ? 1 : 2) : 0;
      c->as_seq++;
      structured_solve(c, b, true, true, true);
      ProfScope ps(c, 5);
      if (cone) {
        ca.finish = 1;
        ca.U = p->U_out; ca.Uraw = w.cone_uraw.d();
        launch_cone_step(ca, s);
      }
      if (xbox) {
        xa.finish = 1;
        xa.X = p->X_out;
        launch_xbox_step(xa, s);
      }
      if (merge) {
        if (last) {
          double *tl = w.Hg.d() + (size_t)nc * nc + nc;
          launch_as_ctl(ctl, (const int *)w.as_cntp.p, M, (const int *)w.fail.p, 1, 0, 0, nullptr, nullptr, 0, s, tl, nullptr, open_part);
          allreduce(c, tl, 5, ncclFloat64, ncclSum);
          launch_as_ctl(ctl, nullptr, M, (const int *)w.fail.p, 0, 1, 1, &c->mirror_dev->ctl, &c->mirror_dev->as_seq, c->as_seq, s, tl);
        }
      } else if (c->multi()) {
        launch_as_ctl(ctl, (const int *)w.as_cntp.p, M, (const int *)w.fail.p, 1, 0, 0, nullptr, nullptr, 0, s, nullptr, nullptr, open_part);
        allreduce(c, &ctl->open, 5, ncclInt32, ncclSum);
        launch_as_ctl(ctl, nullptr, M, (const int *)w.fail.p, 0, 1, last ? 1 : 0, &c->mirror_dev->ctl, &c->mirror_dev->as_seq, c->as_seq, s);
      } else if (!last && fuse_ctl) {
        c->as_pend = AsCtlCall{ctl, (const int *)w.as_cntp.p, M, (const int *)w.fail.p, &c->mirror_dev->ctl, &c->mirror_dev->as_seq, c->as_seq,
                               b.as_viol, open_part, nullptr, nullptr};
      } else {
        launch_as_ctl(ctl, (const int *)w.as_cntp.p, M, (const int *)w.fail.p, 1, 1, last ? 1 : 0, &c->mirror_dev->ctl, &c->mirror_dev->as_seq, c->as_seq, s,
                      nullptr, b.as_viol, open_part);
      }
    }
    if (round == 0 && c->scp.post_batch) {
      std::function<void()> hook;
      hook.swap(c->scp.post_batch);
      c->scp.fired = true;
      n_batches_at_hook = 0;
      hook();
    }
    n_batches_at_hook++;
    {
      const unsigned long long lo_seq = c->as_seq - (unsigned long long)batch + 1, hi_seq = c->as_seq;
      const bool seen = spin_until([&] {
        const unsigned long long v = *(volatile unsigned long long *)&c->mirror->as_seq;
        return v >= lo_seq && v <= hi_seq;
      });
      if (!seen) {
        HIP_CHECK(hipStreamSynchronize(s));
        const unsigned long long v = *(volatile unsigned long long *)&c->mirror->as_seq;
        if (!(v >= lo_seq && v <= hi_seq)) throw PmpcHipError{-1, "active-set control block never published", __FILE__, __LINE__};
      }
      __atomic_thread_fence(__ATOMIC_ACQUIRE);
      memcpy(&h, (const void *)&c->mirror->ctl, sizeof(h));
    }
    if (verbose)
      for (int r = round; r < h.round && r < 16; r++)
        printf("pmpc_hip: active set (%s) round %d: %d released, %d activated (largest violation behind a change %.2e)\n",
               mode == 5 ? "finish" : (mode == 4 ? "state rows" : (mode >= 2 ? "cold" : (mode ? "finish" : "warm"))), r + 1, h.hist[r][0], h.hist[r][1], h.worst[r]);
    if (verbose && cone) printf("pmpc_hip: active set: %d stage cones still open after round %d\n", h.open, h.round);
    if (duc_trace && nc > 0 && !a.cons_G) {
      std::vector<double> hd(nc);
      HIP_CHECK(hipMemcpy(hd.data(), w.as_delta.p, nc * D8, hipMemcpyDeviceToHost));
      double m = 0.0;
      for (double v : hd) m = std::max(m, std::fabs(v));
      int nset = 0;
      { std::vector<int> hs(M); HIP_CHECK(hipMemcpy(hs.data(), w.as_settled.p, M * sizeof(int), hipMemcpyDeviceToHost)); for (int v : hs) nset += v; }
      printf("pmpc_hip: trace: round %d max |du_c| %.3e, %d of %d particles settled\n", h.round, m, nset, M);
      if (b.as_jhi) {
        std::vector<int> hj(M), hs(M), hist(N + 1, 0);
        HIP_CHECK(hipMemcpy(hj.data(), w.as_jhi.p, M * sizeof(int), hipMemcpyDeviceToHost));
        HIP_CHECK(hipMemcpy(hs.data(), w.as_settled.p, M * sizeof(int), hipMemcpyDeviceToHost));
        for (int q = 0; q < M; q++) if (!hs[q]) hist[hj[q] < 0 ? N : hj[q]]++;
        printf("pmpc_hip: trace:   highest changed stage:");
        for (int q = 0; q <= N; q++) if (hist[q]) printf(" %d:%d", q == N ? -1 : q, hist[q]);
        printf("\n");
      }
    }
  if (verbose > 1 && xbox) dump_state_rows(h.round);
  if (verbose > 1 && cone) dump_cone_records();
    inf.structured_solves += h.round - round;
    inf.active_set_rounds += h.round - round;
    round = h.round;
    if (h.done || round >= max_rounds) break;
    depth = 1;
  }
}

void QpSolve::dump_state_rows(int round) {
    HIP_CHECK(hipStreamSynchronize(s));
    std::vector<double> hz(nx), hX(nx), hU(nu);
    std::vector<int> hs(nx), hact(nu);
    HIP_CHECK(hipMemcpy(hz.data(), w.xb_z.p, nx * D8, hipMemcpyDeviceToHost));
    HIP_CHECK(hipMemcpy(hs.data(), w.xb_st.p, nx * sizeof(int), hipMemcpyDeviceToHost));
    HIP_CHECK(hipMemcpy(hX.data(), p->X_out, nx * D8, hipMemcpyDeviceToHost));
    HIP_CHECK(hipMemcpy(hU.data(), p->U_out, nu * D8, hipMemcpyDeviceToHost));
    HIP_CHECK(hipMemcpy(hact.data(), w.as_act.p, nu * sizeof(int), hipMemcpyDeviceToHost));
    int held = 0, uheld = 0, wi = 0;
    double zmax = 0.0, xmax = 0.0;
    for (size_t k = 0; k < nx; k++) {
      held += hs[k] != 0;
      if (hz[k] > zmax) { zmax = hz[k]; wi = (int)(k / ((size_t)N * x)); }
      xmax = std::max(xmax, std::fabs(hX[k]));
    }
    for (size_t k = 0; k < nu; k++) uheld += hact[k] != 0;
    printf("   state rows after round %d: %d held, %d controls held, largest multiplier %.3e (particle %d), largest |x| %.3e\n", round, held, uheld, zmax, wi, xmax);
    if (getenv("PMPC_XB_DUMP")) {
      const int pi = atoi(getenv("PMPC_XB_DUMP"));
      for (int j = 0; j < N; j++) {
        printf("     p%d j%2d st", pi, j);
        for (int r = 0; r < x; r++) printf(" %d", hs[((size_t)pi * N + j) * x + r]);
        printf(" | act");
        for (int r = 0; r < u; r++) printf(" %d", hact[((size_t)pi * N + j) * u + r]);
        printf(" | v");
        for (int r = 3; r < 6 && r < x; r++) printf(" %+.4f", hX[((size_t)pi * N + j) * x + r]);
        printf(" | z");
        for (int r = 3; r < 6 && r < x; r++) printf(" %.3e", hz[((size_t)pi * N + j) * x + r]);
        printf(" | u");
        for (int r = 0; r < u; r++) printf(" %+.4f", hU[((size_t)pi * N + j) * u + r]);
        printf("\n");
      }
    }
}

void QpSolve::dump_cone_records() {
    HIP_CHECK(hipStreamSynchronize(s));
    const int q1 = cone_rows;
    std::vector<double> hz((size_t)M * N * q1), hr((size_t)M * N * std::max(ncones, 1) * PMPC_CONE_REC), hu(nu), hraw(nu), hg(nu);
    HIP_CHECK(hipMemcpy(hz.data(), w.cone_z.p, hz.size() * D8, hipMemcpyDeviceToHost));
    HIP_CHECK(hipMemcpy(hr.data(), w.cone_rec.p, hr.size() * D8, hipMemcpyDeviceToHost));
    HIP_CHECK(hipMemcpy(hu.data(), p->U_out, nu * D8, hipMemcpyDeviceToHost));
    HIP_CHECK(hipMemcpy(hraw.data(), w.cone_uraw.p, nu * D8, hipMemcpyDeviceToHost));
    HIP_CHECK(hipMemcpy(hg.data(), w.wu_soc.p, nu * D8, hipMemcpyDeviceToHost));
    {
      std::vector<int> hcnt((size_t)M * 3);
      HIP_CHECK(hipMemcpy(hcnt.data(), w.as_cntp.p, hcnt.size() * sizeof(int), hipMemcpyDeviceToHost));
      std::vector<int> hact(nu);
      HIP_CHECK(hipMemcpy(hact.data(), w.as_act.p, nu * sizeof(int), hipMemcpyDeviceToHost));
      printf("   act:");
      for (size_t k = 0; k < nu && k < 24; k++) printf(" %d", hact[k]);
      printf("\n   as_cnt:");
      for (int v : hcnt) printf(" %d", v);
      printf(" | U of particle 0:");
      for (int k = 0; k < N * u && k < 12; k++) printf(" %.6e", hu[k]);
      printf(" | uraw:");
      for (int k = 0; k < N * u && k < 12; k++) printf(" %.6e", hraw[k]);
      printf(" | cone_g:");
      for (int k = 0; k < N * u && k < 12; k++) printf(" %.3e", hg[k]);
      printf("\n");
    }
    int shown = 0;
    for (size_t k = 0; k < (size_t)M * N && shown < 6; k++) {
      if (M > 64 ? hr[k * PMPC_CONE_REC + 11] < 3.0 : hr[k * PMPC_CONE_REC] == 0.0) continue;
      printf("   [flips %g]", hr[k * PMPC_CONE_REC + 11]);
      shown++;
      printf("   cone (%zu,%zu) case %g rho %.3e curv %.3e nu %.6e | s_b", k / N, k % N, hr[k * PMPC_CONE_REC], hr[k * PMPC_CONE_REC + 1], hr[k * PMPC_CONE_REC + 2], hr[k * PMPC_CONE_REC + 3]);
      for (int r = 0; r < q1; r++) printf(" %.9e", hr[k * PMPC_CONE_REC + 4 + (q1 - 1) + r]);
      printf(" | z");
      for (int r = 0; r < q1; r++) printf(" %.9e", hz[k * q1 + r]);
      printf(" | u");
      for (int r = 0; r < u; r++) printf(" %.9e", hu[k * u + r]);
      printf(" | uraw");
      for (int r = 0; r < u; r++) printf(" %.9e", hraw[k * u + r]);
      printf(" | g");
      for (int r = 0; r < u; r++) printf(" %.3e", hg[k * u + r]);
      {
        std::vector<double> hk(u), hH((size_t)u * u);
        std::vector<int> ha(u);
        HIP_CHECK(hipMemcpy(hk.data(), w.kff.d() + k * u, u * D8, hipMemcpyDeviceToHost));
        HIP_CHECK(hipMemcpy(ha.data(), (int *)w.as_act.p + k * u, u * sizeof(int), hipMemcpyDeviceToHost));
        HIP_CHECK(hipMemcpy(hH.data(), w.Hadd.d() + k * u * u, (size_t)u * u * D8, hipMemcpyDeviceToHost));
        printf(" | kff");
        for (int r = 0; r < u; r++) printf(" %.3e", hk[r]);
        printf(" | act");
        for (int r = 0; r < u; r++) printf(" %d", ha[r]);
        printf(" | Hdiag");
        for (int r = 0; r < u; r++) printf(" %.3e", hH[r * (u + 1)]);
      }
      printf("\n");
    }
}

int QpSolve::as_accept(AsAttempt &t) {
  const AsCtl &h = t.h;
  const int mode = t.mode, round = t.round, n_batches_at_hook = t.n_batches_at_hook;
  const double dual_scale = t.dual_scale;
  const bool xbox = t.xbox;
  if (verbose && (h.cnt[2] || h.cnt[3])) printf("pmpc_hip: active set: numerical failure / broken promise (bad %d, fail %d)\n", h.cnt[2], h.cnt[3]);
  if (!h.done) return 1;
  if (h.status != 0) return h.status;
  if (has_xb && !xbox_as) {
    reset_scalars();
    HIP_CHECK(hipMemsetAsync(w.part_max.p, 0, 2 * PMPC_RED_BLOCKS * D8, s));
    Slab sc2 = sx;
    sc2.z = p->X_out;
    launch_violation(sc2, w.part_max.d(), s);
    exchange(c, 1);
    read_scalars(c);
    if (*c->fail_host || !(c->sc_host->viol_max <= 1e-13)) {
      if (verbose) printf("pmpc_hip: active set settled but a state box is violated by %.3e: interior-point path\n", c->sc_host->viol_max);
      w.xb_block_key = as_key;
      return 1;
    }
  }
  w.as_U_valid = !(p->flags & PMPC_PREV_IS_LAST_SOLUTION) || (c->multi() && Nc > 1);
  if (w.as_U_valid) HIP_CHECK(hipMemcpyAsync(w.U.p, p->U_out, nu * D8, hipMemcpyDeviceToDevice, s));
  outputs_written = true;
  w.as_key = as_key;
  w.as_scale = dual_scale;
  w.as_count = nu;
  if (mode == 0) w.as_pred_rounds = round;
  c->scp.ok = n_batches_at_hook == 1 && !(has_xb && !xbox);
  return 0;
}

int QpSolve::active_set_solve(double dual_scale, int mode, int max_rounds, int xb) {
  if (fast) return active_set_fast(dual_scale, mode, max_rounds, xb);
  reset_scalars();
  const double big = 1e30, tol_p = 1e-13;
  w.as_act.ensure(nu * sizeof(int) + 8); w.as_cnt.ensure(4 * sizeof(int) + 8);
  int *act = (int *)w.as_act.p, *cnt = (int *)w.as_cnt.p;
  unsigned long long *worst_dev = (unsigned long long *)(cnt + 4);
  double *Xtry = w.dX2.d(), *Utry = w.dU2.d();
  LQArgs b = a;
  b.X = Xtry; b.U = Utry; b.Dx = b.wx = nullptr; b.Du = su.D; b.wu = su.w; b.dX = w.dX.d(); b.dU = w.dU.d();
  Slab st = su;
  st.z = w.U.d(); st.dz = w.dU.d(); st.dz2 = nullptr;
  int last_add = 1, last_changes = 0x7fffffff, stalls = 0;
  w.as_key = -1;
  for (int round = 0; round < max_rounds; round++) {
    const double tol_l = dual_scale * std::min(1e-8, 1e-11 * std::pow(10.0, std::max(0, round - 3)));
    {
      const bool same_base = round > 0 && last_add == 0;
      launch_as_setup(st, round == 0 ? mode : 0, same_base, act, Utry, big, s);
      if (!same_base) launch_rollout(b, Utry, Xtry, s);
      structured_solve(c, b, true, false);
      HIP_CHECK(hipMemsetAsync(cnt, 0, 4 * sizeof(int) + 8, s));
      launch_as_check(st, act, Utry, big, tol_p, tol_l, cnt, worst_dev, s);
      launch_as_publish(cnt, (const int *)w.fail.p, c->multi() ? nullptr : c->mirror_dev->as_cnt, &c->mirror_dev->as_seq, ++c->as_seq, s);
    }
    inf.structured_solves++;
    inf.active_set_rounds++;
    if (c->multi()) {
      allreduce(c, cnt, 4, ncclInt32, ncclSum);
      launch_as_publish(cnt, nullptr, c->mirror_dev->as_cnt, &c->mirror_dev->as_seq, c->as_seq, s);
    }
    wait_published(c, &c->mirror->as_seq, c->as_seq);
    struct { int rel, add, bad, fail; unsigned long long worst; } hc;
    memcpy(&hc, (const void *)c->mirror->as_cnt, 4 * sizeof(int));
    hc.worst = 0;
    if (verbose) {
      HIP_CHECK(hipMemcpyAsync(&hc.worst, worst_dev, 8, hipMemcpyDeviceToHost, s));
      HIP_CHECK(hipStreamSynchronize(s));
    }
    double worst;
    memcpy(&worst, &hc.worst, sizeof(double));
    if (verbose)
      printf("pmpc_hip: active set (%s) round %d: %d released, %d activated (largest %.2e)%s\n", mode == 2 ? "cold" : (mode ? "finish" : "warm"), round + 1,
             hc.rel, hc.add, worst, (hc.bad || hc.fail) ? " (numerical failure)" : "");
    if (hc.bad || hc.fail) return 2;
    last_add = hc.add;
    const int changes = hc.rel + hc.add;
    if (changes == 0) {
      if (has_xb) {
        HIP_CHECK(hipMemsetAsync(w.part_max.p, 0, 2 * PMPC_RED_BLOCKS * D8, s));
        launch_violation_sum(sx, Xtry, w.dX.d(), w.part_max.d(), s);
        exchange(c, 1);
        read_scalars(c);
        if (*c->fail_host || !(c->sc_host->viol_max <= 1e-13)) {
          if (verbose) printf("pmpc_hip: active set settled but a state box is violated by %.3e: interior-point path\n", c->sc_host->viol_max);
          w.xb_block_key = as_key;
          return 1;
        }
      }
      launch_as_accept_all(st, act, Utry, p->U_out, Xtry, w.dX.d(), (long long)nx, w.X.d(), p->X_out, s);
      w.as_U_valid = true;
      outputs_written = true;
      w.as_key = as_key;
      w.as_scale = dual_scale;
      w.as_count = nu;
      return 0;
    }
    if (changes * 2 > last_changes && ++stalls >= 2) return 1;
    last_changes = changes;
  }
  return 1;
}

int QpSolve::interior_point(const bool warm) {
  const double tol = (has_xb && !xbox_as) ? 1e-14 : 1e-12;
  const int max_iter = 80;
  SlabEx ex, eu;
  memset(&ex, 0, sizeof(ex));
  memset(&eu, 0, sizeof(eu));
  ex.s = sx; eu.s = su;
  if (!has_xb) { ex.s.count = (long long)nx; ex.s.d = x; ex.s.N = N; ex.s.Nc = Nc; ex.s.owner = a.owner; ex.s.z = w.X.d(); ex.s.dz = w.dX.d(); }
  if (!has_ub) { eu.s.count = (long long)nu; eu.s.d = u; eu.s.N = N; eu.s.Nc = Nc; eu.s.owner = a.owner; eu.s.is_u = 1; eu.s.z = w.U.d(); eu.s.dz = w.dU.d(); }
  ex.bounded = has_xb; eu.bounded = has_ub;
  ex.s.dz2 = w.dX2.d(); eu.s.dz2 = w.dU2.d();
  ex.pw = eu.pw = p->weights; ex.per = (long long)N * x; eu.per = (long long)N * u;
  ex.ref = p->X_ref; ex.prev = p->X_prev; ex.reg = p->reg_x; ex.gm = fast ? w.xm.d() : nullptr; ex.gd = fast ? w.xd.d() : nullptr;
  eu.ref = p->U_ref; eu.prev = p->U_prev; eu.reg = p->reg_u; eu.gm = fast ? w.um.d() : nullptr; eu.gd = fast ? w.ud.d() : nullptr;
  auto rollout = [&]() {
    if (fast) launch_rollout_fast(a, w.U.d(), w.X.d(), s);
    else launch_rollout(a, w.U.d(), w.X.d(), s);
  };
  bool remembered = false;
  if (warm) {
    HIP_CHECK(hipMemcpyAsync(w.U.p, w.warmU.p, nu * D8, hipMemcpyDeviceToDevice, s));
    rollout();
    if (has_xb) launch_violation(sx, w.part_max.d(), s);
    if (has_ub) launch_violation(su, w.part_max.d() + B, s);
    exchange(c, 1);
    read_scalars(c);
    if (*c->fail_host || !(c->sc_host->viol_max <= 0.0)) {
      if (verbose) printf("pmpc_hip: remembered iterate is outside the new boxes: cold start\n");
      return -1;
    }
  } else if (has_ub) {
    launch_ipm_clip(su, s);
    rollout();
  }
  a.Dx = has_xb ? sx.D : nullptr; a.wx = has_xb ? sx.w : nullptr;
  a.Du = has_ub ? su.D : nullptr; a.wu = has_ub ? su.w : nullptr;
  if (has_xb) launch_ipm_init_slack(sx, 1.0, s, warm ? 1e-9 : 1e-2);
  if (has_ub) launch_ipm_init_slack(su, 1.0, s, warm ? 1e-9 : 1e-2);
  if (warm) {
    if (has_xb) {
      HIP_CHECK(hipMemcpyAsync(sx.ll, w.warm_llx.p, nx * D8, hipMemcpyDeviceToDevice, s));
      HIP_CHECK(hipMemcpyAsync(sx.lu, w.warm_lux.p, nx * D8, hipMemcpyDeviceToDevice, s));
    }
    if (has_ub) {
      HIP_CHECK(hipMemcpyAsync(su.ll, w.warm_llu.p, nu * D8, hipMemcpyDeviceToDevice, s));
      HIP_CHECK(hipMemcpyAsync(su.lu, w.warm_luu.p, nu * D8, hipMemcpyDeviceToDevice, s));
    }
  }
  int status = 1;
  double mu_peak = 1.0;
  double polish_next = xbox_as ? 1e-3 * polish_mu : polish_mu;
  bool advanced = false;
  double late_mu = -1.0;
  for (int it = 1; it <= max_iter; it++) {
// ... 218 lines not shown
```

pmpc_amd/csrc/solver_scp.hip:

```cpp
#include "solver_internal.h"
#include "cost_lin.h"
#include "keepout.h"
#include "model_jit.h"
#include "cost_jit.h"
#include "cstr_jit.h"
#include "cstr_rows.h"

static std::atomic<unsigned long long> g_follow_ups[2];

static bool lin_compact_env() {
  static const bool on = !(getenv("PMPC_LIN_COMPACT") && atoi(getenv("PMPC_LIN_COMPACT")) == 0);
  return on;
}
static bool scp_aug_complete(const pmpc_scp_aug *g) {
  if (!g || !g->Q || !g->x0 || !g->lx || !g->X_out) return false;
  for (int k = 0; k < 2; k++)
    if (!g->f[k] || !g->fx[k] || !g->fu[k] || !g->X_prev[k] || !g->X_ref[k] || !g->xu[k]) return false;
  return true;
}

namespace pmpc_impl {

struct ScpLoop {
  struct Residual { const double *X, *Xp, *U, *Up; double *out; };

  pmpc_ctx *const c;
  const int model;
  const double *const params;
  const pmpc_problem *const p0;
  const int steps, first_cold;
  double *const res;
  pmpc_info *const infos;
  const pmpc_scp_cost *const cost;
  const pmpc_scp_cstr *const cstr;
  const pmpc_scp_aug *const aug;
  const int x, u, N, M;
  const bool with_cost;
  const bool custom_cost, cost_u;
  const bool with_cstr;
  const bool custom_cstr;
  const int K;
  const bool soc;
  const bool cone_obj;
  const int jac32;
  const bool compact_ok;
  double *const XA, *const UA, *const XB, *const UB;
  double *const F[2][3];

  double *Xr[2] = {nullptr, nullptr}, *Ur[2] = {nullptr, nullptr}, *cgrad = nullptr;
  unsigned *cost_bad = nullptr, *cstr_bad = nullptr;
  double *crows = nullptr;
  bool compact_set[2] = {false, false};
  int done = 0, cur = 0;
  double *Xp = nullptr, *Up = nullptr, *Xo = nullptr, *Uo = nullptr;
  bool res_dirty = false;

  ScpLoop(pmpc_ctx *c_, int model_, const double *params_, const pmpc_problem *p, double *f2, double *fx2, double *fu2, int steps_, int first_cold_,
          double *res_, pmpc_info *infos_, const pmpc_scp_cost *cost_, const pmpc_scp_cstr *cstr_, const pmpc_scp_aug *aug_)
      : c(c_), model(model_), params(params_), p0(p), steps(steps_), first_cold(first_cold_), res(res_), infos(infos_), cost(cost_), cstr(cstr_),
        aug(aug_), x((int)p->xdim), u((int)p->udim), N((int)p->N), M((int)p->M), with_cost(cost_ != nullptr && cost_->kind != 0),
        custom_cost(with_cost && cost_->kind == 2), cost_u(custom_cost && cost_->uses_u != 0),
        with_cstr(cstr_ != nullptr && cstr_->kind != 0), custom_cstr(with_cstr && cstr_->kind == 2), K(with_cstr ? cstr_->K : 0), soc(p->soc_u_interior != nullptr || p->cone_count > 0),
        cone_obj((p->flags & PMPC_CONE_OBJECTIVE) != 0), jac32((p->flags & PMPC_F32_MATRICES) ? 1 : 0),
        compact_ok(lin_compact_env() && !with_cstr && !cone_obj && !jac32 && !c_->multi() && p->Nc >= 0 && p->Nc <= 1 && jac_compact_dims(model_, x, u) &&
                   (p->flags & PMPC_SYMMETRIC_COST) && !(p->flags & (PMPC_HAS_SLEW | PMPC_HAS_SLEW0 | PMPC_FORCE_GENERIC | PMPC_COLD_START)) &&
                   ((p->flags & PMPC_HAS_UBOUNDS) || soc) && !(p->barrier_mu > 0.0) && c_->opt[OPT_AS_DEFECT] != 0.0 && c_->opt[OPT_AS_WARM] != 0.0 &&
                   c_->opt[OPT_POLISH_MU] > 0.0),
        XA(const_cast<double *>(p->X_prev)), UA(const_cast<double *>(p->U_prev)), XB(p->X_out), UB(p->U_out),
        F{{const_cast<double *>(p->f), const_cast<double *>(p->fx), const_cast<double *>(p->fu)}, {f2, fx2, fu2}} {}

  bool warm() const { return done > 0 || !first_cold; }

  bool refused() const {
    if (!model_known(c, model)) return true;
    if (model_custom(model)) {
      int mx = 0, mu = 0;
      if (jac32 || !custom_model_dims(model, &mx, &mu) || mx != x || mu != u) return true;
    }
    if (with_cost && !custom_cost && (jac32 || !obstacle_cost_valid(cost, x))) return true;
    if (custom_cost) {
      int cx_ = 0, cu_ = 0, uses = 0;
      if (jac32 || !custom_cost_known(c, cost->id) || !custom_cost_dims(cost->id, &cx_, &cu_, nullptr, &uses) || cx_ != x || cu_ != u ||
          (uses != 0) != cost_u || !cost->cparams || !p0->X_ref || (cost_u && !p0->U_ref))
        return true;
    }
    if (custom_cstr) {
      int gx = 0, gk = 0;
      if (!custom_cstr_known(c, cstr->id) || !custom_cstr_dims(cstr->id, &gx, &gk, nullptr) || gx != x || gk != K || !cstr->gparams) return true;
    }
    return with_cstr && ((!custom_cstr && !keepout_cstr_valid(cstr, x)) || !keepout_strip_dims_valid(p0->xdim, K, p0->udim) || !scp_aug_complete(aug) || soc ||
                         (p0->flags & (PMPC_HAS_SLEW | PMPC_HAS_SLEW0)) || jac32 || c->multi() || p0->smooth_cstr == 1);
  }

  void linearize(int set, const double *X, const double *U, const Residual *fused) {
    ProfScope ps(c, 6);
    double *const *f = F[set];
    compact_set[set] = compact_ok && (set != cur || warm());
    if (compact_set[set] && fused)
      launch_linearize_compact(model, N, M, p0->x0, X, U, params, f[0], f[1], fused->X, fused->Xp, fused->U, fused->Up, x, u, fused->out, c->stream);
    else if (compact_set[set])
      launch_linearize_compact(model, N, M, p0->x0, X, U, params, f[0], f[1], nullptr, nullptr, nullptr, nullptr, 0, 0, nullptr, c->stream);
    else if (fused)
      launch_linearize_with_residual(model, N, M, p0->x0, X, U, params, f[0], f[1], f[2], fused->X, fused->Xp, fused->U, fused->Up, x, u, fused->out,
                                     c->stream, jac32);
    else
      launch_linearize(model, N, M, p0->x0, X, U, params, f[0], f[1], f[2], c->stream, jac32);
    if (custom_cost) {
      const long long rows = (long long)M * N;
      double *cu = cost_u ? cgrad + rows * x : nullptr;
      custom_launch_cost_grad(cost->id, N, M, X, U, cost->cparams, cgrad, cu, nullptr, c->stream);
      launch_ref_shift(x, rows, p0->Q, cgrad, p0->X_ref, Xr[set], cost_bad, c->stream);
      if (cost_u) launch_ref_shift(u, rows, p0->R, cu, p0->U_ref, Ur[set], cost_bad, c->stream);
    } else if (with_cost) {
      launch_obstacle_ref_shift(*cost, x, N, M, X, p0->Q, p0->X_ref, Xr[set], cost_bad, c->stream);
    }
    const double *ref = with_cost ? Xr[set] : p0->X_ref;
    if (custom_cstr) {
      double *h = crows + (long long)M * N * K * x;
      custom_launch_cstr_rows(cstr->id, N, M, X, cstr->gparams, crows, h, nullptr, cstr_bad, c->stream);
      launch_rows_augment(K, x, u, N, M, crows, h, X, f[0], f[1], f[2], ref, aug->f[set], aug->fx[set], aug->fu[set], aug->X_prev[set], aug->X_ref[set],
                          aug->xu[set], c->stream);
    } else if (with_cstr)
      launch_keepout_augment(*cstr, x, u, N, M, X, f[0], f[1], f[2], ref, aug->f[set], aug->fx[set], aug->fu[set],
                             aug->X_prev[set], aug->X_ref[set], aug->xu[set], c->stream);
  }

  pmpc_problem sub_problem(int set, bool warm_start) const {
    pmpc_problem p = *p0;
    p.f = F[set][0]; p.fx = F[set][1]; p.fu = F[set][2];
    if (with_cost) p.X_ref = Xr[set];
    if (cost_u) p.U_ref = Ur[set];
    p.X_prev = Xp; p.U_prev = Up; p.X_out = Xo; p.U_out = Uo;
    p.flags = p0->flags | PMPC_STATIC_CONS_BOUNDS;
    if (warm_start) p.flags |= PMPC_PREV_IS_LAST_SOLUTION;
    else p.flags &= ~(unsigned)PMPC_PREV_IS_LAST_SOLUTION;
    if (with_cstr) {
      p.xdim = (size_t)(x + K);
      p.f = aug->f[set]; p.fx = aug->fx[set]; p.fu = aug->fu[set]; p.X_prev = aug->X_prev[set];
      p.X_ref = (with_cost || p0->X_ref) ? aug->X_ref[set] : nullptr;
      p.Q = aug->Q; p.x0 = aug->x0; p.lx = aug->lx; p.ux = aug->xu[set]; p.X_out = aug->X_out;
      p.flags = (p.flags | PMPC_HAS_XBOUNDS) & ~(unsigned)PMPC_PREV_IS_LAST_SOLUTION;
    }
    return p;
  }

  void follow_up(bool with_next) {
    const bool next = with_next && done + 1 < steps;
    const long long rows = (long long)M * (long long)N;
    if (with_cstr) {
      {
        ProfScope ps(c, 7);
        launch_keepout_strip_residual(aug->X_out, Xo, Xp, Uo, Up, rows, x, K, u, res + done, c->stream, res_dirty);
        res_dirty = true;
      }
      if (next) linearize(cur ^ 1, Xo, Uo, nullptr);
      return;
    }
    if (next && !res_dirty && !c->multi()) {
      const Residual r{Xo, Xp, Uo, Up, res + done};
      linearize(cur ^ 1, Xo, Uo, &r);
      res_dirty = true;
      return;
    }
    {
      ProfScope ps(c, 7);
      launch_scp_residual(Xo, Xp, Uo, Up, rows, x, u, res + done, c->stream, res_dirty);
      res_dirty = true;
    }
    if (c->multi()) allreduce(c, res + done, 1, ncclFloat64, ncclMax);
    if (next) linearize(cur ^ 1, Xo, Uo, nullptr);
  }

  int run() {
    HIP_CHECK(hipSetDevice(c->device));
    HIP_CHECK(hipMemsetAsync(res, 0, (size_t)steps * sizeof(double), c->stream));
    if (with_cost) {
      for (DevBuf &b : c->ws.cost_ref) b.ensure((size_t)p0->M * p0->N * p0->xdim * sizeof(double));
      Xr[0] = c->ws.cost_ref[0].d(); Xr[1] = c->ws.cost_ref[1].d();
      cost_bad = cost_bad_counter(c);
    }
    if (custom_cost) {
      const size_t rows = (size_t)p0->M * p0->N;
      c->ws.cost_grad.ensure(rows * (p0->xdim + (cost_u ? p0->udim : 0)) * sizeof(double));
      cgrad = c->ws.cost_grad.d();
      if (cost_u) {
        for (DevBuf &b : c->ws.cost_uref) b.ensure(rows * p0->udim * sizeof(double));
        Ur[0] = c->ws.cost_uref[0].d(); Ur[1] = c->ws.cost_uref[1].d();
      }
    }
    if (custom_cstr) {
      c->ws.cstr_rows.ensure((size_t)p0->M * p0->N * K * (p0->xdim + 1) * sizeof(double));
      crows = c->ws.cstr_rows.d();
      cstr_bad = cstr_bad_counter(c);
    }
    bool lin_ready = false;
    for (; done < steps; done++, cur ^= 1) {
      Xp = (done & 1) ? XB : XA; Up = (done & 1) ? UB : UA; Xo = (done & 1) ? XA : XB; Uo = (done & 1) ? UA : UB;
      if (!lin_ready) linearize(cur, Xp, Up, nullptr);
      const pmpc_problem p = sub_problem(cur, warm());
      res_dirty = false;
      ScpHookGuard hook{c};
      c->scp = pmpc_ctx::ScpHook{[this] { follow_up(true); }, false, false, compact_set[cur] ? F[cur][1] : nullptr, model};
      pmpc_info inf;
      const int st = cone_obj ? lcone_body(c, &p, p.barrier_mu > 0.0 ? 1.0 / p.barrier_mu : std::numeric_limits<double>::quiet_NaN(), &inf, 0)
                              : (soc ? pmpc_lsoc_solve_device(c, &p, &inf, 0) : pmpc_lqp_solve_device(c, &p, &inf, 0));
      if (infos) infos[done] = inf;
      if (st != 0) {
        if (with_cstr) launch_fill(Xo, std::numeric_limits<double>::quiet_NaN(), (long long)M * N * x, c->stream);
        break;
      }
      lin_ready = c->scp.fired && c->scp.ok;
      if (!lin_ready) follow_up(false);
      g_follow_ups[lin_ready ? 0 : 1]++;
    }
    HIP_CHECK(hipGetLastError());
    return done;
  }

  void poison() {
    if (infos && done < steps) { memset(&infos[done], 0, sizeof(pmpc_info)); infos[done].status = 2; }
    fail_after_error(c, nullptr, nullptr);
    try {
      const double nan = std::numeric_limits<double>::quiet_NaN();
      const long long ex = (long long)M * N * x, eu = (long long)M * N * u;
      for (double *b : {XA, XB}) if (b) launch_fill(b, nan, ex, c->stream);
      for (double *b : {UA, UB}) if (b) launch_fill(b, nan, eu, c->stream);
      if (with_cstr) launch_fill(aug->X_out, nan, (long long)M * N * (x + K), c->stream);
      HIP_WARN(hipStreamSynchronize(c->stream));
    } catch (...) {
    }
  }
};

}

extern "C" {

void pmpc_scp_loop_follow_ups(unsigned long long *out2, int reset) {
  for (int k = 0; k < 2; k++) {
    if (out2) out2[k] = g_follow_ups[k].load();
    if (reset) g_follow_ups[k].store(0);
  }
}
size_t pmpc_abi_scp_aug_size(void) { return sizeof(pmpc_scp_aug); }

int pmpc_scp_loop_device(pmpc_ctx *c, int model, const double *params, const pmpc_problem *p0, double *f2, double *fx2, double *fu2,
                         int steps, int first_cold, double *res, pmpc_info *infos, int *last_in_out) {
  return pmpc_scp_loop_device_cstr(c, model, params, p0, f2, fx2, fu2, steps, first_cold, res, infos, last_in_out, nullptr, nullptr, nullptr);
}
int pmpc_scp_loop_device_cost(pmpc_ctx *c, int model, const double *params, const pmpc_problem *p0, double *f2, double *fx2, double *fu2,
                              int steps, int first_cold, double *res, pmpc_info *infos, int *last_in_out, const pmpc_scp_cost *cost) {
  return pmpc_scp_loop_device_cstr(c, model, params, p0, f2, fx2, fu2, steps, first_cold, res, infos, last_in_out, cost, nullptr, nullptr);
}
int pmpc_scp_loop_device_cstr(pmpc_ctx *c, int model, const double *params, const pmpc_problem *p0, double *f2, double *fx2, double *fu2,
                              int steps, int first_cold, double *res, pmpc_info *infos, int *last_in_out, const pmpc_scp_cost *cost,
                              const pmpc_scp_cstr *cstr, const pmpc_scp_aug *aug) {
  ScpLoop loop(c, model, params, p0, f2, fx2, fu2, steps, first_cold, res, infos, cost, cstr, aug);
  if (loop.refused()) {
    if (infos && steps > 0) { memset(&infos[0], 0, sizeof(pmpc_info)); infos[0].status = 2; }
    if (last_in_out) *last_in_out = 0;
    return 0;
  }
  try {
    loop.run();
  } catch (const PmpcHipError &) {
    loop.poison();
  }
  if (last_in_out) *last_in_out = loop.done & 1;
  return loop.done;
}

}
```

Before: 3071 SCP iterations/s.

## Fold active-set control block into the follow-up linearize kernel launch

When the first active-set round is the last of its batch and the SCP follow-up linearisation fires, the one-block active-set control reduction now runs as block 0 of the linearise kernel instead of as its own launch. This removes one kernel launch and a serial dependency on the stream per SCP iteration. The control reduction is also rewritten to use wave shuffles plus a small per-wave array, so it works with any whole-wave block size rather than assuming 1024 threads. Launch and ride counters are added so the fusion can be checked. The risk is that the control decision now waits for, or shares the grid with, the linearise blocks, and ordering relative to later consumers of the control state changes.

```diff
diff --git a/include/pmpc_abi.h b/include/pmpc_abi.h
--- a/include/pmpc_abi.h
+++ b/include/pmpc_abi.h
@@ -227,6 +227,7 @@
 long long pmpc_cstr_bad_rows(pmpc_ctx *ctx, int reset);
 
 void pmpc_scp_loop_follow_ups(unsigned long long *out2, int reset);
+void pmpc_as_ctl_counts(unsigned long long *out2, int reset);
 
 void pmpc_profile_enable(pmpc_ctx *ctx, int level);
 void pmpc_profile_read(pmpc_ctx *ctx, double *ms4, long long *n4);
diff --git a/pmpc_amd/_lib.py b/pmpc_amd/_lib.py
--- a/pmpc_amd/_lib.py
+++ b/pmpc_amd/_lib.py
@@ -26,7 +26,7 @@
     "pmpc_scp_loop_device_cost", "pmpc_abi_scp_cost_size",
     "pmpc_rollout_device", "pmpc_shift_plan_device",
     "pmpc_keepout_augment_device", "pmpc_abi_scp_cstr_size",
-    "pmpc_keepout_strip_residual_device", "pmpc_scp_loop_device_cstr", "pmpc_abi_scp_aug_size", "pmpc_scp_loop_follow_ups",
+    "pmpc_keepout_strip_residual_device", "pmpc_scp_loop_device_cstr", "pmpc_abi_scp_aug_size", "pmpc_scp_loop_follow_ups", "pmpc_as_ctl_counts",
     "pmpc_shift_active_set_device", "pmpc_warm_shift_device", "pmpc_warm_set_read_device",
     "pmpc_model_compile", "pmpc_model_free_code", "pmpc_model_load", "pmpc_model_unload",
     "pmpc_cost_compile", "pmpc_cost_load", "pmpc_cost_unload", "pmpc_custom_cost_grad_device",
@@ -228,6 +228,9 @@
         if lib.pmpc_abi_scp_aug_size() != ctypes.sizeof(PmpcScpAug):
             raise ImportError(f"{LIB_PATH} and pmpc_amd/_lib.py disagree on pmpc_scp_aug: library {lib.pmpc_abi_scp_aug_size()} bytes, "
                               f"binding {ctypes.sizeof(PmpcScpAug)}: rebuild the library")
+    if hasattr(lib, "pmpc_as_ctl_counts"):
+        lib.pmpc_as_ctl_counts.argtypes = [ctypes.POINTER(ctypes.c_ulonglong), ctypes.c_int]
+        lib.pmpc_as_ctl_counts.restype = None
     if hasattr(lib, "pmpc_warm_shift_device"):
         lib.pmpc_shift_active_set_device.argtypes = [vp, sz, sz, sz, ll, sz] + [vp] * 7
         lib.pmpc_shift_active_set_device.restype = ctypes.c_int
@@ -360,6 +363,12 @@
     return int(out[0]), int(out[1])
 
 
+def as_ctl_counts(reset: bool = False):
+    out = (ctypes.c_ulonglong * 2)()
+    load().pmpc_as_ctl_counts(out, int(reset))
+    return int(out[0]), int(out[1])
+
+
 def as_sweep_knobs():
     out = (ctypes.c_int * 3)()
     load().pmpc_as_sweep_knobs(out)
diff --git a/pmpc_amd/csrc/as_ctl_dev.h b/pmpc_amd/csrc/as_ctl_dev.h
--- a/pmpc_amd/csrc/as_ctl_dev.h
+++ b/pmpc_amd/csrc/as_ctl_dev.h
@@ -6,8 +6,8 @@
 __device__ inline void as_ctl_block(AsCtl *ctl, const int *cnt_part, int M, const int *fail, int reduce, int decide, int last_of_batch,
                                                  AsCtl *mirror, unsigned long long *mirror_seq, unsigned long long seq, double *tail, const double *viol,
                                                  const int *open_part = nullptr) {
-  __shared__ int sh[4][1024];
-  __shared__ double shv[1024];
+  __shared__ int shw[4][16];
+  __shared__ double shvw[16];
   if (ctl->done) {
     if (threadIdx.x == 0 && decide && last_of_batch && mirror) {
       *mirror = *ctl;
@@ -19,27 +19,23 @@
   if (reduce) {
     int r = 0, d = 0, b = 0, op = 0;
     double vw = 0.0;
-    for (int i = threadIdx.x; i < M; i += 1024) {
+    for (int i = threadIdx.x; i < M; i += (int)blockDim.x) {
       r += cnt_part[3 * i]; d += cnt_part[3 * i + 1]; b |= cnt_part[3 * i + 2];
       if (viol) vw = fmax(vw, viol[i]);
       if (open_part) op += open_part[i];
     }
-    sh[0][threadIdx.x] = r; sh[1][threadIdx.x] = d; sh[2][threadIdx.x] = b; sh[3][threadIdx.x] = op; shv[threadIdx.x] = vw;
+    for (int o = 32; o > 0; o >>= 1) {
+      r += __shfl_xor(r, o, 64); d += __shfl_xor(d, o, 64); b |= __shfl_xor(b, o, 64); op += __shfl_xor(op, o, 64);
+      vw = fmax(vw, __shfl_xor(vw, o, 64));
+    }
+    const int wv = (int)threadIdx.x >> 6, nw = ((int)blockDim.x + 63) >> 6;
+    if ((threadIdx.x & 63) == 0) { shw[0][wv] = r; shw[1][wv] = d; shw[2][wv] = b; shw[3][wv] = op; shvw[wv] = vw; }
     __syncthreads();
-    for (int o = 512; o > 0; o >>= 1) {
-      if (threadIdx.x < o) {
-        sh[0][threadIdx.x] += sh[0][threadIdx.x + o];
-        sh[1][threadIdx.x] += sh[1][threadIdx.x + o];
-        sh[2][threadIdx.x] |= sh[2][threadIdx.x + o];
-        sh[3][threadIdx.x] += sh[3][threadIdx.x + o];
-        shv[threadIdx.x] = fmax(shv[threadIdx.x], shv[threadIdx.x + o]);
-      }
-      __syncthreads();
-    }
-    if (threadIdx.x == 0 && viol && ctl->round < 16) ctl->worst[ctl->round] = shv[0];
     if (threadIdx.x == 0) {
-      if (tail) { tail[0] = sh[0][0]; tail[1] = sh[1][0]; tail[2] = sh[2][0]; tail[3] = *fail; tail[4] = sh[3][0]; }
-      else { ctl->cnt[0] = sh[0][0]; ctl->cnt[1] = sh[1][0]; ctl->cnt[2] = sh[2][0]; ctl->cnt[3] = *fail; ctl->open = sh[3][0]; }
+      for (int k = 1; k < nw; k++) { r += shw[0][k]; d += shw[1][k]; b |= shw[2][k]; op += shw[3][k]; vw = fmax(vw, shvw[k]); }
+      if (viol && ctl->round < 16) ctl->worst[ctl->round] = vw;
+      if (tail) { tail[0] = r; tail[1] = d; tail[2] = b; tail[3] = *fail; tail[4] = op; }
+      else { ctl->cnt[0] = r; ctl->cnt[1] = d; ctl->cnt[2] = b; ctl->cnt[3] = *fail; ctl->open = op; }
     }
   }
   if (threadIdx.x == 0 && decide) {
diff --git a/pmpc_amd/csrc/dynamics.hip b/pmpc_amd/csrc/dynamics.hip
--- a/pmpc_amd/csrc/dynamics.hip
+++ b/pmpc_amd/csrc/dynamics.hip
@@ -1,6 +1,7 @@
 #include "pmpc_dev.h"
 #include "jac_compact.h"
 #include "model_jit.h"
+#include "as_ctl_dev.h"
 #include <cstring>
 #include <cstdlib>
 
@@ -218,10 +219,16 @@
 #ifndef PMPC_LIN_THREADS
 #define PMPC_LIN_THREADS 256
 #endif
+static_assert(PMPC_LIN_THREADS % 64 == 0 && PMPC_LIN_THREADS <= 1024, "as_ctl_block: whole waves, 16 at the most");
+__device__ __forceinline__ void ride_ctl_block(const AsCtlCall &ride) {
+  as_ctl_block(ride.ctl, ride.cnt_part, ride.M, ride.fail, 1, 1, 1, ride.mirror, ride.mirror_seq, ride.seq, nullptr, ride.viol, ride.open_part);
+}
 template <class Model, class JT>
 __global__ void __launch_bounds__(PMPC_LIN_THREADS) k_linearize(int N, long long tot, const double *x0, const double *X_prev, const double *U_prev,
-                                                  const double *params, double *f, JT *fx, JT *fu, ResArgs res) {
+                                                  const double *params, double *f, JT *fx, JT *fu, ResArgs res, AsCtlCall ride) {
   constexpr int X = Model::X, U = Model::U, UNITS = Model::UNITS;
+  const int front = ride.ctl ? 1 : 0;
+  if (front && blockIdx.x == 0) return ride_ctl_block(ride);
   {
     const int glin = (int)gridDim.x - res.nblk;
     if ((int)blockIdx.x >= glin) {
@@ -232,7 +239,7 @@
   constexpr int REC = X + X * X + X * U, LD = REC | 1;
   extern __shared__ double rec[];
   const int t = threadIdx.x;
-  const long long first = (long long)blockIdx.x * UNITS;
+  const long long first = (long long)((int)blockIdx.x - front) * UNITS;
   for (int e = t; e < UNITS * LD; e += PMPC_LIN_THREADS) rec[e] = 0.0;
   __syncthreads();
   if (t < UNITS && first + t < tot) {
@@ -248,23 +255,25 @@
 
 template <class Model>
 void launch_model(int N, int M, const double *x0, const double *X_prev, const double *U_prev, const double *params, double *f,
-                  double *fx, double *fu, const ResArgs &res, hipStream_t s, int jac32) {
+                  double *fx, double *fu, const ResArgs &res, const AsCtlCall &ride, hipStream_t s, int jac32) {
   const long long tot = (long long)M * N;
   constexpr int REC = Model::X + Model::X * Model::X + Model::X * Model::U, LD = REC | 1;
-  const unsigned grid = (unsigned)((tot + Model::UNITS - 1) / Model::UNITS);
+  const unsigned grid = (unsigned)((tot + Model::UNITS - 1) / Model::UNITS) + (ride.ctl ? 1u : 0u);
   if (jac32)
     hipLaunchKernelGGL((k_linearize<Model, float>), dim3(grid + (unsigned)res.nblk), dim3(PMPC_LIN_THREADS), Model::UNITS * LD * sizeof(double), s, N, tot, x0,
-                       X_prev, U_prev, params, f, (float *)fx, (float *)fu, res);
+                       X_prev, U_prev, params, f, (float *)fx, (float *)fu, res, ride);
   else
     hipLaunchKernelGGL((k_linearize<Model, double>), dim3(grid + (unsigned)res.nblk), dim3(PMPC_LIN_THREADS), Model::UNITS * LD * sizeof(double), s, N, tot, x0,
-                       X_prev, U_prev, params, f, fx, fu, res);
+                       X_prev, U_prev, params, f, fx, fu, res, ride);
 }
 constexpr int LIN_CUNITS = 64;
 template <class Model>
 __global__ void __launch_bounds__(PMPC_LIN_THREADS) k_linearize_compact(int N, long long tot, const double *x0, const double *X_prev, const double *U_prev,
-                                                                         const double *params, double *f, double *jc, ResArgs res) {
+                                                                         const double *params, double *f, double *jc, ResArgs res, AsCtlCall ride) {
   typedef jacc::Compact<typename Model::Spec> C;
   constexpr int X = Model::X, U = Model::U, UNITS = LIN_CUNITS, REC = C::REC, POOL = C::POOL;
+  const int front = ride.ctl ? 1 : 0;
+  if (front && blockIdx.x == 0) return ride_ctl_block(ride);
   {
     const int glin = (int)gridDim.x - res.nblk;
     if ((int)blockIdx.x >= glin) {
@@ -275,7 +284,7 @@
   constexpr int LD = (X + REC) | 1;
   extern __shared__ double rec[];
   const int t = threadIdx.x;
-  const long long first = (long long)blockIdx.x * UNITS;
+  const long long first = (long long)((int)blockIdx.x - front) * UNITS;
   if (t < UNITS && first + t < tot) {
     double J[X * X + X * U] = {};
     double *mine = rec + t * LD;
@@ -311,13 +320,13 @@
 
 template <class Model>
 void launch_model_compact(int N, int M, const double *x0, const double *X_prev, const double *U_prev, const double *params, double *f,
-                          double *jc, const ResArgs &res, hipStream_t s) {
+                          double *jc, const ResArgs &res, const AsCtlCall &ride, hipStream_t s) {
   typedef jacc::Compact<typename Model::Spec> C;
   const long long tot = (long long)M * N;
   constexpr int LD = (Model::X + C::REC) | 1;
-  const unsigned grid = (unsigned)((tot + LIN_CUNITS - 1) / LIN_CUNITS);
+  const unsigned grid = (unsigned)((tot + LIN_CUNITS - 1) / LIN_CUNITS) + (ride.ctl ? 1u : 0u);
   hipLaunchKernelGGL((k_linearize_compact<Model>), dim3(grid + (unsigned)res.nblk), dim3(PMPC_LIN_THREADS), LIN_CUNITS * LD * sizeof(double), s, N, tot,
-                     x0, X_prev, U_prev, params, f, jc, res);
+                     x0, X_prev, U_prev, params, f, jc, res, ride);
 }
 __global__ void __launch_bounds__(256) k_widen_f32(const float *src, double *dst, long long n) {
   for (long long k = (long long)blockIdx.x * 256 + threadIdx.x; k < n; k += (long long)gridDim.x * 256) dst[k] = (double)src[k];
@@ -435,11 +444,11 @@
   if (model_custom(model)) return custom_launch_linearize(model, N, M, x0, X_prev, U_prev, params, f, fx, fu, s);
   ResArgs none;
   memset(&none, 0, sizeof(none));
-  with_model(model, [&](auto m) { launch_model<decltype(m)>(N, M, x0, X_prev, U_prev, params, f, fx, fu, none, s, jac32); });
+  with_model(model, [&](auto m) { launch_model<decltype(m)>(N, M, x0, X_prev, U_prev, params, f, fx, fu, none, AsCtlCall{}, s, jac32); });
 }
 void launch_linearize_compact(int model, int N, int M, const double *x0, const double *X_prev, const double *U_prev, const double *params,
                               double *f, double *jc, const double *Xr, const double *Xrp, const double *Ur, const double *Urp, int x, int u,
-                              double *res_out, hipStream_t s) {
+                              double *res_out, hipStream_t s, AsCtlCall *ride) {
   ResArgs r;
   memset(&r, 0, sizeof(r));
   if (res_out) {
@@ -447,7 +456,9 @@
     r.nblk = (int)residual_blocks(r.rows);
     r.out_bits = (unsigned long long *)res_out;
   }
-  with_model(model, [&](auto m) { launch_model_compact<decltype(m)>(N, M, x0, X_prev, U_prev, params, f, jc, r, s); });
+  const AsCtlCall rc = ride ? *ride : AsCtlCall{};
+  with_model(model, [&](auto m) { launch_model_compact<decltype(m)>(N, M, x0, X_prev, U_prev, params, f, jc, r, rc, s); });
+  if (ride && ride->ctl) { count_as_ctl_ride(); ride->ctl = nullptr; }
 }
 void launch_rollout(int model, int N, int M, const double *x0, const double *U, const double *params, double *X, hipStream_t s) {
   if (model_custom(model)) return custom_launch_rollout(model, N, M, x0, U, params, X, s);
@@ -518,7 +529,7 @@
 
 void launch_linearize_with_residual(int model, int N, int M, const double *x0, const double *X_prev, const double *U_prev,
                                     const double *params, double *f, double *fx, double *fu, const double *Xr, const double *Xrp,
-                                    const double *Ur, const double *Urp, int x, int u, double *res_out, hipStream_t s, int jac32) {
+                                    const double *Ur, const double *Urp, int x, int u, double *res_out, hipStream_t s, int jac32, AsCtlCall *ride) {
   if (model_custom(model)) {
     custom_launch_linearize(model, N, M, x0, X_prev, U_prev, params, f, fx, fu, s);
     return launch_scp_residual(Xr, Xrp, Ur, Urp, (long long)M * N, x, u, res_out, s, false);
@@ -527,7 +538,9 @@
   r.X = Xr; r.Xp = Xrp; r.U = Ur; r.Up = Urp; r.rows = (long long)M * N; r.x = x; r.u = u;
   r.nblk = (int)residual_blocks(r.rows);
   r.out_bits = (unsigned long long *)res_out;
-  with_model(model, [&](auto m) { launch_model<decltype(m)>(N, M, x0, X_prev, U_prev, params, f, fx, fu, r, s, jac32); });
+  const AsCtlCall rc = ride ? *ride : AsCtlCall{};
+  with_model(model, [&](auto m) { launch_model<decltype(m)>(N, M, x0, X_prev, U_prev, params, f, fx, fu, r, rc, s, jac32); });
+  if (ride && ride->ctl) { count_as_ctl_ride(); ride->ctl = nullptr; }
 }
 
 namespace {
diff --git a/pmpc_amd/csrc/kernels_as.hip b/pmpc_amd/csrc/kernels_as.hip
--- a/pmpc_amd/csrc/kernels_as.hip
+++ b/pmpc_amd/csrc/kernels_as.hip
@@ -874,6 +874,7 @@
   return k;
 }
 std::atomic<unsigned long long> as_bwd_launches[AS_BWD_CODES], as_fwd_launches[AS_FWD_CODES];
+std::atomic<unsigned long long> as_ctl_launches, as_ctl_rides;
 
 template <int XD, int UD>
 void launch_bwd_as_t(const LQArgs &a, hipStream_t s) {
@@ -972,6 +973,14 @@
   }
   return codes;
 }
+void pmpc_as_ctl_counts(unsigned long long *out2, int reset) {
+  std::atomic<unsigned long long> *t[2] = {&as_ctl_launches, &as_ctl_rides};
+  for (int k = 0; k < 2; k++) {
+    const unsigned long long v = reset ? t[k]->exchange(0, std::memory_order_relaxed) : t[k]->load(std::memory_order_relaxed);
+    if (out2) out2[k] = v;
+  }
+}
+void count_as_ctl_ride() { as_ctl_rides.fetch_add(1, std::memory_order_relaxed); }
 void pmpc_as_sweep_knobs(int *out) {
   const AsSweepKnobs &k = as_sweep_knobs();
   out[0] = k.deep2_maxm; out[1] = k.deep_maxm; out[2] = k.fwd_pf2_maxm;
@@ -990,6 +999,7 @@
 }
 void launch_as_ctl(AsCtl *ctl, const int *cnt_part, int M, const int *fail, int reduce, int decide, int last_of_batch, AsCtl *mirror,
                    unsigned long long *mirror_seq, unsigned long long seq, hipStream_t s, double *tail, const double *viol, const int *open_part) {
+  as_ctl_launches.fetch_add(1, std::memory_order_relaxed);
   hipLaunchKernelGGL(k_as_ctl, dim3(1), dim3(1024), 0, s, ctl, cnt_part, M, fail, reduce, decide, last_of_batch, mirror, mirror_seq, seq, tail, viol,
                      open_part);
 }
diff --git a/pmpc_amd/csrc/pmpc_dev.h b/pmpc_amd/csrc/pmpc_dev.h
--- a/pmpc_amd/csrc/pmpc_dev.h
+++ b/pmpc_amd/csrc/pmpc_dev.h
@@ -187,6 +187,7 @@
 void launch_fwd_as(const LQArgs &a, hipStream_t s);
 void launch_as_perm(const int *settled, int M, int *perm, const int *done, hipStream_t s);
 void launch_as_begin(AsCtl *ctl, int *fail, int max_rounds, double dual_scale, hipStream_t s, int stall_limit = 2);
+void count_as_ctl_ride();
 void launch_as_ctl(AsCtl *ctl, const int *cnt_part, int M, const int *fail, int reduce, int decide, int last_of_batch, AsCtl *mirror,
                    unsigned long long *mirror_seq, unsigned long long seq, hipStream_t s, double *tail = nullptr, const double *viol = nullptr,
                    const int *open_part = nullptr);
@@ -310,7 +311,7 @@
                       const double *params, double *f, double *fx, double *fu, hipStream_t s, int jac32 = 0);
 void launch_linearize_compact(int model, int N, int M, const double *x0, const double *X_prev, const double *U_prev, const double *params,
                               double *f, double *jc, const double *Xr, const double *Xrp, const double *Ur, const double *Urp, int x, int u,
-                              double *res_out, hipStream_t s);
+                              double *res_out, hipStream_t s, AsCtlCall *ride = nullptr);
 void launch_rollout(int model, int N, int M, const double *x0, const double *U, const double *params, double *X, hipStream_t s);
 void launch_shift_plan(int model, int N, int M, int sh, const double *X, const double *U, const double *params, const double *U_tail, double *Xn,
                        double *Un, double *um1n, hipStream_t s);
@@ -323,7 +324,8 @@
 int jac_live_mask(int model, unsigned char *fx_mask, unsigned char *fu_mask);
 void launch_linearize_with_residual(int model, int N, int M, const double *x0, const double *X_prev, const double *U_prev,
                                     const double *params, double *f, double *fx, double *fu, const double *Xr, const double *Xrp,
-                                    const double *Ur, const double *Urp, int x, int u, double *res_out, hipStream_t s, int jac32 = 0);
+                                    const double *Ur, const double *Urp, int x, int u, double *res_out, hipStream_t s, int jac32 = 0,
+                                    AsCtlCall *ride = nullptr);
 void launch_widen_f32(const float *src, double *dst, long long n, hipStream_t s);
 bool f32_as_dims_supported(int x, int u);
 void launch_scp_residual(const double *X, const double *Xp, const double *U, const double *Up, long long rows, int x, int u,
diff --git a/pmpc_amd/csrc/solver_internal.h b/pmpc_amd/csrc/solver_internal.h
--- a/pmpc_amd/csrc/solver_internal.h
+++ b/pmpc_amd/csrc/solver_internal.h
@@ -153,6 +153,8 @@
     bool fired = false, ok = false;
     const double *compact_fx = nullptr;
     int compact_model = 0;
+    AsCtlCall ride{};
+    bool can_ride = false;
   } scp;
 };
 
diff --git a/pmpc_amd/csrc/solver_qp.hip b/pmpc_amd/csrc/solver_qp.hip
--- a/pmpc_amd/csrc/solver_qp.hip
+++ b/pmpc_amd/csrc/solver_qp.hip
@@ -714,6 +714,7 @@
   const bool fuse_env = c->opt[OPT_AS_FUSE_CTL] != 0.0 && c->opt[OPT_AS_WAVE_CONS] != 0.0;
   const bool fuse_ctl = fuse_env && !c->multi() && Nc == 1;
   const int *open_part = (cone || xbox) ? (const int *)w.as_open.p : nullptr;
+  static const bool ride_ctl = !(getenv("PMPC_SCP_RIDE_CTL") && atoi(getenv("PMPC_SCP_RIDE_CTL")) == 0);
   const int perm_min_m = (int)c->opt[OPT_AS_PERM_MIN_M];
   round = 0;
   int depth = mode == 0 ? std::max(1, std::min(w.as_pred_rounds, max_rounds)) : std::min(3, max_rounds);
@@ -778,6 +779,9 @@
       } else if (!last && fuse_ctl) {
         c->as_pend = AsCtlCall{ctl, (const int *)w.as_cntp.p, M, (const int *)w.fail.p, &c->mirror_dev->ctl, &c->mirror_dev->as_seq, c->as_seq,
                                b.as_viol, open_part, nullptr, nullptr};
+      } else if (last && round == 0 && c->scp.post_batch && c->scp.can_ride && ride_ctl) {
+        c->scp.ride = AsCtlCall{ctl, (const int *)w.as_cntp.p, M, (const int *)w.fail.p, &c->mirror_dev->ctl, &c->mirror_dev->as_seq, c->as_seq,
+                                b.as_viol, open_part, nullptr, nullptr};
       } else {
         launch_as_ctl(ctl, (const int *)w.as_cntp.p, M, (const int *)w.fail.p, 1, 1, last ? 1 : 0, &c->mirror_dev->ctl, &c->mirror_dev->as_seq, c->as_seq, s,
                       nullptr, b.as_viol, open_part);
@@ -789,6 +793,12 @@
       c->scp.fired = true;
       n_batches_at_hook = 0;
       hook();
+      if (c->scp.ride.ctl) {
+        ProfScope ps(c, 5);
+        const AsCtlCall r = c->scp.ride;
+        c->scp.ride = AsCtlCall{};
+        launch_as_ctl(r.ctl, r.cnt_part, r.M, r.fail, 1, 1, 1, r.mirror, r.mirror_seq, r.seq, s, nullptr, r.viol, r.open_part);
+      }
     }
     n_batches_at_hook++;
     {
diff --git a/pmpc_amd/csrc/solver_scp.hip b/pmpc_amd/csrc/solver_scp.hip
--- a/pmpc_amd/csrc/solver_scp.hip
+++ b/pmpc_amd/csrc/solver_scp.hip
@@ -97,12 +97,13 @@
     double *const *f = F[set];
     compact_set[set] = compact_ok && (set != cur || warm());
     if (compact_set[set] && fused)
-      launch_linearize_compact(model, N, M, p0->x0, X, U, params, f[0], f[1], fused->X, fused->Xp, fused->U, fused->Up, x, u, fused->out, c->stream);
+      launch_linearize_compact(model, N, M, p0->x0, X, U, params, f[0], f[1], fused->X, fused->Xp, fused->U, fused->Up, x, u, fused->out, c->stream,
+                               &c->scp.ride);
     else if (compact_set[set])
       launch_linearize_compact(model, N, M, p0->x0, X, U, params, f[0], f[1], nullptr, nullptr, nullptr, nullptr, 0, 0, nullptr, c->stream);
     else if (fused)
       launch_linearize_with_residual(model, N, M, p0->x0, X, U, params, f[0], f[1], f[2], fused->X, fused->Xp, fused->U, fused->Up, x, u, fused->out,
-                                     c->stream, jac32);
+                                     c->stream, jac32, &c->scp.ride);
     else
       launch_linearize(model, N, M, p0->x0, X, U, params, f[0], f[1], f[2], c->stream, jac32);
     if (custom_cost) {
@@ -201,6 +202,7 @@
       res_dirty = false;
       ScpHookGuard hook{c};
       c->scp = pmpc_ctx::ScpHook{[this] { follow_up(true); }, false, false, compact_set[cur] ? F[cur][1] : nullptr, model};
+      c->scp.can_ride = !with_cstr && !model_custom(model) && !c->multi() && done + 1 < steps;
       pmpc_info inf;
       const int st = cone_obj ? lcone_body(c, &p, p.barrier_mu > 0.0 ? 1.0 / p.barrier_mu : std::numeric_limits<double>::quiet_NaN(), &inf, 0)
                               : (soc ? pmpc_lsoc_solve_device(c, &p, &inf, 0) : pmpc_lqp_solve_device(c, &p, &inf, 0));
```

Result: faster. 3135 SCP iterations/s (median of 6 runs) (+2.1%).
